# mims-harvard/G-Meta

Measured on AMD Instinct MI355X. Metric: meta-tasks/sec (inner-loop fwd+bwd) at task_num=32, higher is better.
Workload: dtype f32

## Files before the change

g-meta_amd/_lib.py:

```python
import ctypes as C
import os

HERE = os.path.dirname(os.path.abspath(__file__))
LIB_PATH = os.environ.get('GMETA_HIP_LIB') or os.path.join(HERE, 'libgmeta_hip.so')

GM_MAX_GCN = 4
(F_SUB_OFF, F_SET_SUB_OFF, F_PARENT, F_GRAPH, F_INDPTR, F_INDICES, F_INDPTR_T, F_INDICES_T, F_CENTRE, F_NORM,
 F_FEAT_ROW, F_NORM_SRC, F_NORM_CENTRE, F_EDGE_W, F_EDGE_W_T, F_HOP, F_NORM_E1, F_EDGE_CENTRE_T, F_OBS_CENTRE, F_OBS_E1) = range(20)
LINK_SYMMETRIC = 2
LINK_MASK_TARGET = 4
NEG_MODES = {'uniform': 0, 'two_hop': 1}
PAIR_MASK_TARGET = 1
PROP_SELF_LOOPS = 1
PROP_OPS = {'hadamard': 0, 'abs_diff': 1}
DIST_UNREACHED = 255


class Seed(C.Structure):
    _fields_ = [('graph', C.c_int32), ('i', C.c_int32), ('j', C.c_int32)]


class Model(C.Structure):
    _fields_ = [('n_gcn', C.c_int32), ('dims', C.c_int32 * (GM_MAX_GCN + 1)), ('n_out', C.c_int32), ('link_pred', C.c_int32)]


class HParams(C.Structure):
    _fields_ = [('update_lr', C.c_float), ('update_step', C.c_int32), ('k_spt', C.c_int32), ('need_meta_grad', C.c_int32),
                ('hoist_z1', C.c_int32), ('serialize', C.c_int32), ('sparse_bwd', C.c_int32), ('cone', C.c_int32)]


vp, i32, i64, u64 = C.c_void_p, C.c_int32, C.c_int64, C.c_uint64
PROTOTYPES = {
    'gm_last_error': (C.c_char_p, []),
    'gm_version': (C.c_int, []),
    'gm_store_create': (C.c_int, [i32, vp, vp, vp, vp, i32, vp]),
    'gm_store_create_weighted': (C.c_int, [i32, vp, vp, vp, vp, vp, i32, vp]),
    'gm_store_weighted': (i32, [vp]),
    'gm_batch_weighted': (i32, [vp]),
    'gm_store_destroy': (None, [vp]),
    'gm_store_negative_pairs': (i32, [vp, i32, i64, u64, i32, vp, i64, vp, vp, vp]),
    'gm_store_has_edges': (i32, [vp, i32, vp, i64, vp, vp]),
    'gm_store_pair_scores': (i32, [vp, i32, vp, i64, i32, vp, vp]),
    'gm_store_pair_walks': (i32, [vp, i32, vp, i64, i32, vp, vp]),
    'gm_store_rooted_pagerank': (i32, [vp, i32, vp, i64, C.c_float, i32, vp, vp]),
    'gm_store_pair_pagerank': (i32, [vp, i32, vp, i64, i32, C.c_float, i32, vp, vp]),
    'gm_store_pagerank_candidates': (i32, [vp, i32, vp, i64, i32, C.c_float, i32, vp, vp, vp, vp]),
    'gm_store_node_distances': (i32, [vp, i32, vp, i64, i32, vp, vp]),
    'gm_store_pair_distance': (i32, [vp, i32, vp, i64, i32, i32, vp, vp]),
    'gm_store_pair_distance_profile': (i32, [vp, i32, vp, i64, i32, i32, vp, vp]),
    'gm_store_sketch_build': (i32, [vp, i32, i32, i32, i32, u64, vp, vp]),
    'gm_sketch_dims': (i32, [vp, vp, vp, vp, vp, vp]),
    'gm_sketch_registers': (i32, [vp, i32, vp, i64, vp, vp, vp]),
    'gm_sketch_pair_counts': (i32, [vp, vp, i64, vp, vp, vp]),
    'gm_sketch_destroy': (None, [vp]),
    'gm_store_propagate_build': (i32, [vp, i32, i32, i32, vp, vp]),
    'gm_prop_dims': (i32, [vp, vp, vp, vp, vp, vp]),
    'gm_prop_rows': (i32, [vp, i32, vp, i64, vp, vp]),
    'gm_prop_pair_features': (i32, [vp, vp, i64, i32, vp, vp]),
    'gm_prop_destroy': (None, [vp]),
    'gm_store_neighbour_degrees': (i32, [vp, i32, vp, vp]),
    'gm_store_pair_candidates': (i32, [vp, i32, vp, i64, i32, i32, vp, vp, vp, vp]),
    'gm_extract': (C.c_int, [vp, vp, i32, vp, i32, i32, i32, u64, i32, vp, vp]),
    'gm_extract_pair': (C.c_int, [vp, vp, i32, vp, i32, vp, i32, vp, i32, i32, i32, u64, i32, vp, vp, vp]),
    'gm_batch_from_nodes': (C.c_int, [vp, vp, i32, vp, i32, vp, vp, i32, vp, vp]),
    'gm_set_hop_labels': (None, [i32]),
    'gm_get_hop_labels': (i32, []),
    'gm_batch_hop_labels': (i32, [vp]),
    'gm_batch_mask_target': (i32, [vp]),
    'gm_batch_concat': (C.c_int, [vp, i32, vp, vp]),
    'gm_batch_destroy': (None, [vp]),
    'gm_batch_prepare_cone': (C.c_int, [vp, i32, vp]),
    'gm_batch_prepare_cone_pair': (C.c_int, [vp, vp, i32, vp]),
    'gm_batch_cone_dims': (C.c_int, [vp, i32, vp, vp, vp]),
    'gm_batch_cone_read': (C.c_int, [vp, i32, i32, i32, vp, i64]),
    'gm_batch_dims': (C.c_int, [vp, vp, vp, vp, vp, vp]),
    'gm_batch_read': (C.c_int, [vp, i32, vp, i64]),
    'gm_batch_device_ptr': (C.c_int, [vp, i32, vp]),
    'gm_batch_source_rows': (C.c_int, [vp, vp]),
    'gm_batch_e1_source_rows': (C.c_int, [vp, vp]),
    'gm_gather_features': (C.c_int, [vp, vp, vp]),
    'gm_aggregate': (C.c_int, [vp, i32, i32, vp, i32, vp, vp, vp, vp]),
    'gm_aggregate_bytes': (i64, [vp, i32]),
    'gm_model_param_count': (i64, [vp]),
    'gm_gcn_ws_bytes': (i64, [vp, vp]),
    'gm_gcn_forward': (C.c_int, [vp, vp, vp, i64, vp, vp, vp, vp, i64, vp]),
    'gm_gcn_backward': (C.c_int, [vp, vp, vp, i64, vp, vp, vp, vp, i64, vp, i64, vp]),
    'gm_dense_update': (C.c_int, [vp, vp, i32, vp, i64, i32, vp, i32, vp]),
    'gm_dense_gemm': (C.c_int, [vp, vp, i64, i32, vp, i64, i32, i32, vp, i64, vp, vp, vp, i64, i32, vp, vp, vp, vp, vp, i32, vp, vp]),
    'gm_dense_fused_gemm': (C.c_int, [vp, i32, vp, i64, i32, vp, i64, vp, i64, vp, i64, i32, vp, i64, vp, vp, vp, i64, i32, vp, vp, vp, i32, vp, vp]),
    'gm_dense_wgrad_fused': (C.c_int, [vp, i32, vp, i64, i32, vp, i64, vp, i64, i32, vp, vp, vp, i64, vp, i64, i32, vp]),
    'gm_dense_aggregate': (C.c_int, [vp, i32, i32, vp, i64, i32, i32, vp, vp, i32, vp, i64, i32, vp, vp, vp, i32, vp, i64, i32, i32, i32, i32, i32, vp, vp, vp]),
    'gm_dense_agg_info': (C.c_int, [vp, i32, vp]),
    'gm_dense_fuse_counts': (C.c_int, [vp, vp]),
    'gm_dense_agg_table': (C.c_int, [vp, i32, i32, vp, i64, vp]),
    'gm_dense_dz_centre': (C.c_int, [vp, vp, i32, vp, i64, i32, vp, vp]),
    'gm_dense_wgrad_centre': (C.c_int, [vp, vp, i32, vp, i32, vp, i64, vp, i64, vp]),
    'gm_dense_agg_centre_t': (C.c_int, [vp, vp, i32, vp, vp, i32, vp]),
    'gm_dense_wgrad_e1': (C.c_int, [vp, vp, i32, vp, i32, vp, i64, vp, i64, vp]),
    'gm_dense_wgrad': (C.c_int, [vp, vp, i64, i32, vp, i64, i32, vp, vp, i64, vp, i64, vp, i64, i32, vp, vp, i64, C.c_float, vp, vp, vp, vp]),
    'gm_proto_loss_spt': (C.c_int, [vp, vp, i32, vp, i32, vp, vp, vp, vp, vp]),
    'gm_proto_loss_qry': (C.c_int, [vp, vp, i32, vp, vp, i32, vp, vp, vp, vp, vp]),
    'gm_dense_head_loss': (C.c_int, [vp, vp, i32, i32, i32, i32, vp, i64, i64, i64, vp, vp, i32, i32, vp, i32, vp, vp, vp, vp, vp, vp, vp, vp, i32, vp, i64, vp, vp,
                                     vp, vp, i64, C.c_float, vp, i32, vp, vp]),
    'gm_set_ragged_classes': (None, [i32]),
    'gm_get_ragged_classes': (i32, []),
    'gm_set_readout': (None, [i32]),
    'gm_get_readout': (i32, []),
    'gm_meta_ws_bytes': (i64, [vp, vp, vp, vp]),
    'gm_meta_out_floats': (i64, [vp, vp, vp]),
    'gm_meta_step': (C.c_int, [vp, vp, vp, vp, vp, vp, vp, vp, i64, vp, i64, vp]),
    'gm_adapt_ws_bytes': (i64, [vp, vp, vp]),
    'gm_meta_adapt': (C.c_int, [vp, vp, vp, vp, vp, vp, i64, vp, i32, vp, i64, vp]),
    'gm_predict_ws_bytes': (i64, [vp, vp, vp]),
    'gm_proto_predict': (C.c_int, [vp, vp, vp, vp, i64, vp, vp, i32, vp, vp, vp, vp, i64, vp]),
    'gm_meta_finish': (C.c_int, [vp, i64, i32, vp, vp, vp]),
    'gm_meta_finish_adam': (C.c_int, [vp, i64, i32, vp, vp, vp, vp, vp, i32, C.c_float, C.c_float, C.c_float, C.c_float, vp, vp, vp]),
    'gm_set_gemm_mode': (None, [i32]),
    'gm_get_gemm_mode': (i32, []),
    'gm_get_split_pieces': (i32, []),
    'gm_set_split_pieces': (None, [i32]),
    'gm_set_tuning': (C.c_int, [C.c_char_p, i32]),
    'gm_get_tuning': (i32, [C.c_char_p]),
    'gm_tuning_epoch': (i32, []),
    'gm_set_fuse_agg': (None, [i32]),
    'gm_get_fuse_agg': (i32, []),
    'gm_profile_enable': (None, [i32]),
    'gm_profile_aggregate': (C.c_int, [vp, vp, vp]),
    'gm_profile_read': (C.c_int, [i32, vp, vp, vp]),
    'gm_profile_read_launches': (C.c_int, [i32, vp, vp, i32]),
}
PROBE_PROTOTYPES = {
    'gm_debug_stamp': (C.c_int, [vp, vp]),
    'gm_stream_debug': (C.c_int, [i32, vp, i32]),
    'gm_head_loss_debug': (C.c_int, [i32, vp]),
}

_lib = None


def lib():
    global _lib
    if _lib is None:
        if not os.path.exists(LIB_PATH):
            raise RuntimeError('gmeta_amd: %s is missing -- run `python -c "import __graft_entry__ as g; g.build()"` '
                               '(hipcc --offload-arch=gfx950).  There is no CPU fallback.' % LIB_PATH)
        l = C.CDLL(LIB_PATH)
        for name, (res, args) in PROTOTYPES.items():
            fn = getattr(l, name)
            fn.restype, fn.argtypes = res, args
        for name, (res, args) in PROBE_PROTOTYPES.items():
            if hasattr(l, name):
                fn = getattr(l, name)
                fn.restype, fn.argtypes = res, args
        _lib = l
    return _lib


def check(rc, what=''):
    if rc != 0:
        msg = lib().gm_last_error().decode('utf-8', 'replace')
        exc = ValueError if rc == -1 else RuntimeError
        raise exc('%s failed (code %d): %s' % (what or 'libgmeta_hip', rc, msg))


def require_gpu():
    import torch
    if not torch.cuda.is_available():
        raise RuntimeError('gmeta_amd needs an AMD GPU (gfx950); torch.cuda.is_available() is False and there is no CPU fallback')


def stream_ptr():
    import torch
    return C.c_void_p(torch.cuda.current_stream().cuda_stream)


def ptr(t):
    if t is None:
        return C.c_void_p(0)
    if hasattr(t, 'data_ptr'):
        return C.c_void_p(t.data_ptr())
    return C.c_void_p(t.ctypes.data)


READOUT_CENTRE, READOUT_MEAN = 0, 1
READOUTS = {'centre': READOUT_CENTRE, 'mean': READOUT_MEAN}


def config_readout(config):
    ent = [(k, p) for k, (n, p) in enumerate(config) if n == 'Readout']
    if not ent:
        return 'centre'
    if len(ent) > 1:
        raise ValueError("config holds %d 'Readout' entries; at most one" % len(ent))
    k, p = ent[0]
    if not isinstance(p, (list, tuple)) or len(p) != 1 or p[0] not in READOUTS:
        raise ValueError("config entry ('Readout', %r): expected ['centre'] or ['mean']" % (p,))
    if any(n == 'LinkPred' for n, _ in config) and config[-1][0] != 'LinkPred':
        raise ValueError("the ('Readout', ...) entry must come before the trailing ('LinkPred', [True]) entry")
    return p[0]


class readout_switch:

    def __init__(self, readout):
        self.mode = READOUTS[readout] if isinstance(readout, str) else int(readout)

    def __enter__(self):
        l = lib()
        self.was = int(l.gm_get_readout())
        if self.was != self.mode:
            l.gm_set_readout(self.mode)
        return self

    def __exit__(self, *exc):
        if self.was != self.mode:
            lib().gm_set_readout(self.was)
        return False


def make_model(config):
    unknown = sorted({str(n) for n, _ in config if n not in ('GraphConv', 'Linear', 'LinkPred', 'Readout', 'Attention')})
    if unknown:
        raise ValueError('unknown config entries: %s' % ', '.join(unknown))
    config_readout(config)
    gcn = [p for n, p in config if n == 'GraphConv']
    lin = [p for n, p in config if n == 'Linear']
    if any(n == 'Attention' for n, _ in config):
        raise NotImplementedError("the 'Attention' branch of learner.py:98-131 is dead code in the reference (uses an undefined name)")
    if not gcn or len(lin) != 1 or len(gcn) > GM_MAX_GCN:
        raise ValueError('config must hold 1..%d GraphConv entries and one Linear entry' % GM_MAX_GCN)
# ... 12 lines not shown
```

g-meta_amd/csrc/agg.hip:

```cpp
#include <algorithm>
#include <stdlib.h>
#include <mutex>
#include "gm_internal.h"
#include "agg_hub.h"

#define AGG_BLOCK 256

struct AggK {
    const int32_t* indptr; const int32_t* indices; const float* x; const int32_t* x_row; int64_t ldx;
    const float* s_in; const float* s_out; const float* mask_h; const float* bias; int64_t bias_stride;
    const int32_t* set_row_off; int n_sets; int relu; float* out; int64_t rows; int width; int nblocks;
    const uint8_t* mask_b; uint8_t* relu_bits;
    const int32_t* heavy; int n_heavy, heavy_deg;
    const int32_t* sched; int sched_len;
    int nt;
    int win;
    const int32_t* hub; float* hub_scratch; int hub_part, hub_ld;
    const float* e_w; const int32_t* x_idx;
    int skip_lo, skip_hi;
    const int32_t* rowlist; int64_t n_list;
    int keep_signed;
};
__host__ __device__ __forceinline__ int agg_xcd_first(const int nb, const int x) {
    const int q = nb / GM_NXCD, r = nb % GM_NXCD;
    return x < r ? x * (q + 1) : r * (q + 1) + (x - r) * q;
}
__device__ __forceinline__ int agg_logical_block(const int nb, const int b) { return agg_xcd_first(nb, b % GM_NXCD) + b / GM_NXCD; }

__device__ __forceinline__ float agg_out_scale(const AggK& a, const float raw, bool& keep) {
    keep = !(a.keep_signed && (__float_as_uint(raw) >> 31));
    return a.keep_signed ? fabsf(raw) : raw;
}
__device__ __forceinline__ bool agg_unobservable(const AggK& a, const float raw) {
    return a.keep_signed && !a.relu_bits && (__float_as_uint(raw) >> 31);
}
__device__ __forceinline__ int agg_bias_set(const AggK& a, const int64_t row) {
    if (!a.bias || !a.bias_stride) return 0;
    int lo = 0, hi = a.n_sets;
    while (hi - lo > 1) { const int mid = (lo + hi) >> 1; if (a.set_row_off[mid] <= row) lo = mid; else hi = mid; }
    return lo;
}

__device__ __forceinline__ void agg_edge(const AggK& a, const int e, int& u, float& w) {
    if (a.e_w && (a.x_idx || !a.x_row)) {
        w = a.e_w[e]; u = a.x_idx ? a.x_idx[e] : a.indices[e];
    } else {
        u = a.indices[e]; w = a.s_in ? a.s_in[u] : 1.f;
        if (a.x_idx) u = a.x_idx[e]; else if (a.x_row) u = a.x_row[u];
    }
}
template <int VEC> struct VecT;
template <> struct VecT<4> { using T = float4; };
template <> struct VecT<1> { using T = float; };

__device__ __forceinline__ void vfma(float4& a, const float4& v, float s) { a.x += v.x * s; a.y += v.y * s; a.z += v.z * s; a.w += v.w * s; }
__device__ __forceinline__ void vfma(float& a, const float& v, float s) { a += v * s; }
__device__ __forceinline__ void vzero(float4& a) { a = make_float4(0.f, 0.f, 0.f, 0.f); }
__device__ __forceinline__ void vzero(float& a) { a = 0.f; }
__device__ __forceinline__ float vget(const float4& a, int k) { return k == 0 ? a.x : k == 1 ? a.y : k == 2 ? a.z : a.w; }
__device__ __forceinline__ float vget(const float& a, int) { return a; }
__device__ __forceinline__ void vset(float4& a, int k, float v) { if (k == 0) a.x = v; else if (k == 1) a.y = v; else if (k == 2) a.z = v; else a.w = v; }
__device__ __forceinline__ void vset(float& a, int, float v) { a = v; }

template <int VEC, int LPR>
__global__ __launch_bounds__(AGG_BLOCK) void k_agg(AggK a) {
    using V = typename VecT<VEC>::T;
    constexpr int RPW = GM_WAVE / LPR;
    constexpr int RPB = RPW * (AGG_BLOCK / GM_WAVE);
    const int lb = agg_logical_block(a.nblocks, blockIdx.x);
    const int lane = threadIdx.x & 63, wave = threadIdx.x >> 6;
    const int sub = lane / LPR, l = lane % LPR;
    const int64_t row = (int64_t)lb * RPB + wave * RPW + sub;
    if (row >= a.rows) return;
    const int e0 = a.indptr[row], e1 = a.indptr[row + 1];
    bool keep;
    const float raw = a.s_out ? a.s_out[row] : 1.f;
    if (agg_unobservable(a, raw)) return;
    const float so = agg_out_scale(a, raw, keep);
    const int set = agg_bias_set(a, row);
    for (int c0 = l * VEC; c0 < a.width; c0 += LPR * VEC) {
        V acc0, acc1; vzero(acc0); vzero(acc1);
        int e = e0;
        for (; e + 4 <= e1; e += 4) {
            int u0, u1, u2, u3; float w0, w1, w2, w3;
            agg_edge(a, e, u0, w0); agg_edge(a, e + 1, u1, w1); agg_edge(a, e + 2, u2, w2); agg_edge(a, e + 3, u3, w3);
            const V v0 = *reinterpret_cast<const V*>(a.x + (int64_t)u0 * a.ldx + c0);
            const V v1 = *reinterpret_cast<const V*>(a.x + (int64_t)u1 * a.ldx + c0);
            const V v2 = *reinterpret_cast<const V*>(a.x + (int64_t)u2 * a.ldx + c0);
            const V v3 = *reinterpret_cast<const V*>(a.x + (int64_t)u3 * a.ldx + c0);
            vfma(acc0, v0, w0); vfma(acc1, v1, w1); vfma(acc0, v2, w2); vfma(acc1, v3, w3);
        }
        for (; e < e1; ++e) {
            int u; float w;
            agg_edge(a, e, u, w);
            vfma(acc0, *reinterpret_cast<const V*>(a.x + (int64_t)u * a.ldx + c0), w);
        }
        V res;
#pragma unroll
        for (int k = 0; k < VEC; ++k) {
            float v = (vget(acc0, k) + vget(acc1, k)) * so;
            if (a.bias) v += a.bias[(int64_t)set * a.bias_stride + c0 + k];
            if (a.relu) v = v < 0.f ? 0.f : v;
            if (a.mask_b) v = ((a.mask_b[(row * a.width + c0) >> 2] >> k) & 1u) ? v : 0.f;
            else if (a.mask_h) v = a.mask_h[row * a.width + c0 + k] > 0.f ? v : 0.f;
// ... 56 lines not shown
            __builtin_nontemporal_store(vv, reinterpret_cast<f4v*>(dst));
        } else *dst = v;
    }
}

#define AGG_HEAVY_BLOCK 1024
template <int LPR, int NCH, int NTHREADS>
__device__ __forceinline__ void agg_heavy_row(const AggK& a, const int g, float* part) {
    constexpr int NG = NTHREADS / LPR;
    constexpr int PS = 16;
    const int tid = threadIdx.x, gi = tid / LPR, l = tid % LPR, lane = tid & 63;
    const int gbase = (lane / LPR) * LPR;
    int h = g, p = 0, P = 1;
    if (a.hub) { h = a.hub[a.n_heavy + 1 + g]; p = g - a.hub[h]; P = a.hub[h + 1] - a.hub[h]; }
    const int row = a.heavy[h];
    const float so = a.s_out ? a.s_out[row] : 1.f;
    if (agg_unobservable(a, so)) return;
    int e0 = a.indptr[row], e1 = a.indptr[row + 1];
    if (P > 1) { e0 += p * a.hub_part; if (p < P - 1) e1 = e0 + a.hub_part; }
    const float* xl = a.x + l * 4;
    float4 acc[NCH];
#pragma unroll
    for (int c = 0; c < NCH; ++c) acc[c] = make_float4(0.f, 0.f, 0.f, 0.f);
    for (int eb = e0 + gi * PS; eb < e1; eb += NG * PS) agg_gather_batch<LPR, NCH, PS, 8>(a, xl, eb, e1, l, gbase, acc);
#pragma unroll
    for (int c = 0; c < NCH; ++c) *reinterpret_cast<float4*>(&part[(gi * NCH + c) * LPR * 4 + l * 4]) = acc[c];
    __syncthreads();
    float4 s4[NCH];
    if (gi == 0) {
#pragma unroll
        for (int c = 0; c < NCH; ++c) {
            s4[c] = make_float4(0.f, 0.f, 0.f, 0.f);
            for (int k = 0; k < NG; ++k) { const float4 t = *reinterpret_cast<const float4*>(&part[(k * NCH + c) * LPR * 4 + l * 4]); s4[c].x += t.x; s4[c].y += t.y; s4[c].z += t.z; s4[c].w += t.w; }
        }
    }
    if (P > 1) {
        if (gi == 0) {
#pragma unroll
            for (int c = 0; c < NCH; ++c) agg_hub_publish(a.hub_scratch + (int64_t)g * a.hub_ld + l * 4 + c * LPR * 4, s4[c]);
        }
        agg_hub_drain();
        __syncthreads();
        int* ctr = const_cast<int*>(a.hub) + a.n_heavy + 1 + a.hub[a.n_heavy] + h;
        int* flag = reinterpret_cast<int*>(part);
        if (tid == 0) *flag = agg_hub_arrive(ctr, P);
        __syncthreads();
        if (!*flag || gi != 0) return;
        const float* sc = a.hub_scratch + (int64_t)a.hub[h] * a.hub_ld + l * 4;
#pragma unroll
        for (int c = 0; c < NCH; ++c) {
            s4[c] = make_float4(0.f, 0.f, 0.f, 0.f);
            for (int k = 0; k < P; ++k) {
                const float4 t = *reinterpret_cast<const float4*>(sc + (int64_t)k * a.hub_ld + c * LPR * 4);
                s4[c].x += t.x; s4[c].y += t.y; s4[c].z += t.z; s4[c].w += t.w;
            }
        }
    }
    if (gi == 0) agg_store_row<LPR, NCH>(a, row, so, l, s4, false);
}
template <int LPR, int NCH>
__global__ __launch_bounds__(AGG_HEAVY_BLOCK) void k_agg_heavy(AggK a) {
    __shared__ __attribute__((aligned(16))) float part[(AGG_HEAVY_BLOCK / LPR) * LPR * 4 * NCH];
    agg_heavy_row<LPR, NCH, AGG_HEAVY_BLOCK>(a, blockIdx.x, part);
}

template <int LPR, int NCH>
__global__ __launch_bounds__(AGG_BLOCK) void k_agg_win(AggK a) {
    constexpr int G = GM_WAVE / LPR;
    constexpr int UNR = 2;
    int lb = agg_logical_block(a.nblocks, blockIdx.x);
    if (a.sched) {
        const int e = a.sched[(blockIdx.x % GM_NXCD) * a.sched_len + blockIdx.x / GM_NXCD];
        if (e == -1) return;
        if (e < -1) {
            __shared__ __attribute__((aligned(16))) float part[AGG_BLOCK * 4 * NCH];
            agg_heavy_row<LPR, NCH, AGG_BLOCK>(a, -e - 2, part);
            return;
        }
        lb = e;
    }
    const int lane = threadIdx.x & 63, wave = threadIdx.x >> 6;
    const int g = lane / LPR, l = lane % LPR;
    const int64_t R0 = ((int64_t)lb * (AGG_BLOCK / GM_WAVE) + wave) * a.win;
    const int64_t nrows_w = a.rowlist ? a.n_list : a.rows;
    if (R0 >= nrows_w) return;
    const bool mine = lane < a.win && R0 + lane < nrows_w;
    const int64_t myrow = a.rowlist ? (mine ? (int64_t)a.rowlist[R0 + lane] : 0) : R0 + lane;
    const int myrow32 = (int)myrow;
    int p0 = 0, dg = 0, u0 = 0, u1 = 0; float w0 = 0.f, w1 = 0.f, so = 1.f;
    if (mine) {
        p0 = a.indptr[myrow]; dg = a.indptr[myrow + 1] - p0;
        if (a.s_out) so = a.s_out[myrow];
        if (dg >= a.skip_lo && dg <= a.skip_hi) dg = -2;
        if (agg_unobservable(a, so)) dg = -2;
        if (dg >= 1) agg_edge(a, p0, u0, w0);
        if (dg >= 2) agg_edge(a, p0 + 1, u1, w1);
    }
    const int nwin = (int)min((int64_t)a.win, nrows_w - R0);
    const float* xl = a.x + l * 4;
    const unsigned long long live = __ballot(mine && dg >= 0);
    for (int t0 = 0; t0 < nwin; t0 += G * UNR) {
        if (!((live >> t0) & ((1ull << (G * UNR)) - 1))) continue;
        float4 acc[UNR][NCH];
        int rdg[UNR], rp0[UNR], rrow[UNR]; float rso[UNR];
#pragma unroll
        for (int k = 0; k < UNR; ++k) {
            const int rr = t0 + k * G + g;
            const int src = rr < GM_WAVE ? rr : 0;
            rdg[k] = rr < nwin ? __shfl(dg, src, 64) : -1;
            rrow[k] = __shfl(myrow32, src, 64);
            if (a.n_heavy && rdg[k] > a.heavy_deg) rdg[k] = -1;
            rp0[k] = __shfl(p0, src, 64); rso[k] = __shfl(so, src, 64);
            const int a0 = __shfl(u0, src, 64), a1 = __shfl(u1, src, 64);
            const float f0 = __shfl(w0, src, 64), f1 = __shfl(w1, src, 64);
#pragma unroll
            for (int c = 0; c < NCH; ++c) acc[k][c] = make_float4(0.f, 0.f, 0.f, 0.f);
            if (rdg[k] >= 1) {
#pragma unroll
                for (int c = 0; c < NCH; ++c) vfma(acc[k][c], *reinterpret_cast<const float4*>(xl + (int64_t)a0 * a.ldx + c * LPR * 4), f0);
            }
            if (rdg[k] >= 2) {
#pragma unroll
                for (int c = 0; c < NCH; ++c) vfma(acc[k][c], *reinterpret_cast<const float4*>(xl + (int64_t)a1 * a.ldx + c * LPR * 4), f1);
            }
        }
#pragma unroll
        for (int k = 0; k < UNR; ++k) {
            if (rdg[k] < 0) continue;
            const int rr_ = t0 + k * G + g;
            const int64_t row = a.rowlist ? (int64_t)rrow[k] : R0 + rr_;
            const int eend = rp0[k] + rdg[k];
            for (int eb = rp0[k] + 2; eb < eend; eb += LPR) agg_gather_batch<LPR, NCH, LPR, 4>(a, xl, eb, eend, l, g * LPR, acc[k]);
            agg_store_row<LPR, NCH>(a, row, rso[k], l, acc[k], a.nt);
        }
    }
}

int gm_agg_window(int64_t rows, int64_t edges) {
    const bool dense = edges > 8 * rows;
    const int min_waves = dense ? 16384 : 32768;
    const int min_win = dense ? 4 : 2;
    int win = 64;
    while (win > min_win && rows / win < min_waves) win >>= 1;
    return win;
}

int gm_agg_schedule_flat(gm_batch* b, int64_t rows, int win, const int32_t* pos, int n_heavy, const std::vector<int32_t>& tab, int32_t** d_sched, int32_t* len_out,
                         hipStream_t s, gm_stager* sg) {
    const bool split = !tab.empty();
    const int RPB = win * (AGG_BLOCK / GM_WAVE);
    const int nwb = std::max(1, (int)((rows + RPB - 1) / RPB));
    auto x_start = [&](int x) { return agg_xcd_first(nwb, x); };
    auto n_entries = [&](int k) { return split ? tab[k + 1] - tab[k] : 1; };
    int extra[GM_NXCD] = {}; int first[GM_NXCD + 1];
    {
        int hk = 0;
        for (int x = 0; x < GM_NXCD; ++x) {
            const int end = x_start(x + 1);
            first[x] = hk;
            while (hk < n_heavy && pos[hk] / RPB < end) {
                GM_REQUIRE(hk == 0 || pos[hk] >= pos[hk - 1], GM_EINVAL, "aggregate schedule: hub-row list is not ascending");
                extra[x] += n_entries(hk); ++hk;
            }
        }
        first[GM_NXCD] = hk;
        GM_REQUIRE(hk == n_heavy, GM_EINVAL, "aggregate schedule: hub-row list is not ascending / out of range");
    }
    size_t len = 0;
    for (int x = 0; x < GM_NXCD; ++x) len = std::max(len, (size_t)(x_start(x + 1) - x_start(x) + extra[x]));
    std::vector<int32_t> flat(GM_NXCD * len);
    for (int x = 0; x < GM_NXCD; ++x) {
        int32_t* o = flat.data() + x * len; int32_t* const o_end = o + len;
        int wb = x_start(x); const int end = x_start(x + 1);
        for (int hk = first[x]; hk < first[x + 1]; ++hk) {
            const int hb = pos[hk] / RPB;
            while (wb <= hb) *o++ = wb++;
            if (split) for (int g = tab[hk]; g < tab[hk + 1]; ++g) *o++ = -g - 2;
            else *o++ = -hk - 2;
        }
        while (wb < end) *o++ = wb++;
        while (o < o_end) *o++ = -1;
    }
    GM_TRY(gm_balloc(b, d_sched, flat.size(), s));
    GM_TRY(sg->upload(*d_sched, flat));
    *len_out = (int32_t)len;
    return GM_OK;
}

int gm_agg_schedule(gm_batch* b, int64_t rows, int win, const int32_t* heavy_host, const int32_t* heavy_deg_host, int n_heavy, gm_agg_sched* out, hipStream_t s, gm_stager* sg) {
    *out = gm_agg_sched{};
    if (n_heavy <= 0 || rows <= 0) return GM_OK;
    int hub_part = 0;
    std::vector<int32_t> tab;
    if (heavy_deg_host) {
        int maxdeg = 0;
        for (int k = 0; k < n_heavy; ++k) maxdeg = std::max(maxdeg, heavy_deg_host[k]);
        hub_part = std::max(128, ((maxdeg + 31) / 32 + 15) / 16 * 16);
        tab.assign(n_heavy + 1, 0);
        for (int k = 0; k < n_heavy; ++k) tab[k + 1] = tab[k] + std::max(1, (heavy_deg_host[k] + hub_part / 2) / hub_part);
        const int parts = tab[n_heavy];
        if (parts == n_heavy) { hub_part = 0; tab.clear(); }
        else {
            tab.resize(n_heavy + 1 + parts + n_heavy, 0);
            for (int k = 0; k < n_heavy; ++k) for (int g = tab[k]; g < tab[k + 1]; ++g) tab[n_heavy + 1 + g] = k;
        }
    }
    GM_TRY(gm_agg_schedule_flat(b, rows, win, heavy_host, n_heavy, tab, &out->d_sched, &out->len, s, sg));
    if (hub_part) {
        GM_TRY(gm_balloc(b, &out->d_hub, tab.size(), s));
        GM_TRY(sg->upload(out->d_hub, tab));
        GM_TRY(gm_balloc(b, &out->d_hub_scratch, (size_t)tab[n_heavy] * GM_AGG_HUB_LD, s));
        out->hub_part = hub_part; out->hub_words = (int32_t)tab.size(); out->parts = tab[n_heavy];
    }
    out->tab = tab;
    return GM_OK;
}

template <int LPR, int NCH>
static void launch_win(const AggK& a0, hipStream_t s, int* launched) {
    AggK a = a0;
    a.win = (a.sched || a.rowlist) ? a0.win : gm_agg_window(a.rows, 0);
    const int RPB = a.win * (AGG_BLOCK / GM_WAVE);
    a.nblocks = (int)(((a.rowlist ? a.n_list : a.rows) + RPB - 1) / RPB);
    int grid = a.nblocks;
    if (a.sched) grid = GM_NXCD * a.sched_len;
    else if (a.n_heavy > 0) hipLaunchKernelGGL((k_agg_heavy<LPR, NCH>), dim3(a.n_heavy), dim3(AGG_HEAVY_BLOCK), 0, s, a);
    hipLaunchKernelGGL((k_agg_win<LPR, NCH>), dim3(grid), dim3(AGG_BLOCK), 0, s, a);
    if (launched) *launched = GM_AGG_ID_WIN(LPR, NCH) + (a.sched ? GM_AGG_ID_WIN_SCHED + (a.hub ? GM_AGG_ID_WIN_SPLIT : 0) : a.n_heavy > 0 ? GM_AGG_ID_WIN_HEAVY : 0) +
                                (a.rowlist ? GM_AGG_ID_WIN_LIST : 0);
}

template <int VEC, int LPR>
static void launch_one(const AggK& a0, hipStream_t s, int* launched) {
    AggK a = a0;
    constexpr int RPB = (GM_WAVE / LPR) * (AGG_BLOCK / GM_WAVE);
    a.nblocks = (int)((a.rows + RPB - 1) / RPB);
    hipLaunchKernelGGL((k_agg<VEC, LPR>), dim3(a.nblocks), dim3(AGG_BLOCK), 0, s, a);
    if (launched) *launched = GM_AGG_ID_ONE(VEC, LPR);
}
template <int VEC>
static void launch_generic(const AggK& a, const int lanes, hipStream_t s, int* launched) {
    if (lanes > 32) launch_one<VEC, 64>(a, s, launched);
    else if (lanes > 16) launch_one<VEC, 32>(a, s, launched);
    else if (lanes > 8) launch_one<VEC, 16>(a, s, launched);
    else if (lanes > 4) launch_one<VEC, 8>(a, s, launched);
    else if (lanes > 2) launch_one<VEC, 4>(a, s, launched);
    else launch_one<VEC, 2>(a, s, launched);
}

static int agg_nt(int64_t rows, int width) { return rows * (int64_t)width * 4 >= ((int64_t)128 << 20) ? 1 : 0; }

int gm_launch_aggregate(const gm_agg_args& g, hipStream_t s) {
    if (g.rows <= 0) return GM_OK;
    AggK a{};
    a.indptr = g.indptr; a.indices = g.indices; a.x = g.x; a.x_row = g.x_row; a.ldx = g.ldx;
    a.s_in = g.s_in; a.s_out = g.s_out; a.mask_h = g.mask_h; a.bias = g.bias; a.bias_stride = g.bias_stride;
    a.set_row_off = g.set_row_off; a.n_sets = g.n_sets; a.relu = g.relu; a.out = g.out; a.rows = g.rows; a.width = g.width;
    a.mask_b = g.mask_b; a.relu_bits = g.relu_bits;
    a.heavy = g.heavy; a.n_heavy = g.n_heavy; a.heavy_deg = g.heavy_deg;
    a.sched = g.sched; a.sched_len = g.sched_len;
    a.nt = agg_nt(g.rows, g.width);
    a.win = g.rowlist ? g.list_win : g.sched ? g.sched_win : 64;
    a.hub = g.sched ? g.hub : nullptr; a.hub_scratch = g.sched ? g.hub_scratch : nullptr; a.hub_part = g.hub_part; a.hub_ld = GM_AGG_HUB_LD;
    a.e_w = g.e_w; a.x_idx = g.x_idx;
    a.skip_lo = g.skip_on ? g.skip_lo : 1; a.skip_hi = g.skip_on ? g.skip_hi : 0;
    a.rowlist = g.rowlist; a.n_list = g.n_list;
    a.keep_signed = (g.keep_signed && g.s_out) ? 1 : 0;
    const bool vec4 = (g.width % 4 == 0) && (g.ldx % 4 == 0) && (((uintptr_t)g.x & 15) == 0) && (((uintptr_t)g.out & 15) == 0);
    const bool bias_ok = !g.bias || ((((uintptr_t)g.bias & 15) == 0) && (g.bias_stride % 4 == 0));
    const bool mask_ok = !g.mask_h || (((uintptr_t)g.mask_h & 15) == 0);
    GM_REQUIRE(!(g.mask_b || g.relu_bits) || vec4, GM_EINVAL, "aggregate: packed relu masks need width %% 4 == 0 and 16-byte aligned operands");
    const bool win = vec4 && bias_ok && mask_ok && (g.width == 64 || g.width == 128 || g.width == 256 || g.width == 512);
    GM_REQUIRE(!g.rowlist || win, GM_EINVAL, "aggregate: a row list needs the window kernel");
    if (!win) { a.heavy = nullptr; a.n_heavy = 0; a.sched = nullptr; a.hub = nullptr; }
    if (win && gm_knob().agg_stream && gm_stream_ok(g)) return gm_launch_stream(g, a.nt, s);
    if (win) {
        if (g.width == 64) launch_win<16, 1>(a, s, g.launched);
        else if (g.width == 128) launch_win<32, 1>(a, s, g.launched);
        else if (g.width == 256) launch_win<64, 1>(a, s, g.launched);
        else launch_win<64, 2>(a, s, g.launched);
    } else if (vec4) launch_generic<4>(a, g.width / 4, s, g.launched);
    else launch_generic<1>(a, g.width, s, g.launched);
    GM_HIP(hipGetLastError());
    return GM_OK;
}

int gm_agg_stream_args(gm_agg_args& a, const gm_batch* b, int o, bool gather, hipStream_t s) {
    if (!gm_knob().agg_stream || a.s_out || a.bias || a.mask_h || a.mask_b || a.relu || a.relu_bits || a.rowlist || a.skip_on) return GM_OK;
    gm_batch::stream_pending& sp = b->spend[o];
    {
        static std::mutex mu;
        std::lock_guard<std::mutex> lk(mu);
        if (sp.pending) {
            gm_batch* mb = const_cast<gm_batch*>(b);
            gm_stager sg(s);
            GM_TRY(gm_stream_tables(mb, o, sp.hubs.data(), sp.deg.data(), (int)sp.hubs.size(), sp.n_parts, sp.has_tab ? &sp.tab : nullptr, s, &sg));
            sp.pending = false;
            sp.hubs = std::vector<int32_t>(); sp.deg = std::vector<int32_t>(); sp.tab = std::vector<int32_t>();
            gm_batch_mark_use(b, s);
        }
    }
    if (!b->d_sptr[o] || !b->d_sseg[o] || (gather && (o != 0 || !b->d_su_feat))) return GM_OK;
    a.stream = b; a.stream_o = o; a.stream_feat = gather ? 1 : 0;
    a.stream_xrows = gather ? b->feat_rows : b->rows;
    return GM_OK;
}

extern "C" int64_t gm_aggregate_bytes(const gm_batch_t* b, int32_t width) {
    if (!b) return -1;
    return 4 * (b->rows + 1) + 4 * b->edges + 4 * b->rows + 8 * b->rows * (int64_t)width;
}

extern "C" int gm_aggregate(const gm_batch_t* b, int32_t transposed, int32_t gather, const float* x, int32_t width,
                            const float* s_in, const float* s_out, float* out, void* stream) {
    GM_REQUIRE(b && out && width >= 1, GM_EINVAL, "aggregate: bad arguments");
    GM_REQUIRE(gather || x, GM_EINVAL, "aggregate: x is NULL and gather == 0");
    GM_REQUIRE(!gather || width == b->feat_dim, GM_EINVAL, "aggregate: gather needs width == feat_dim");
    gm_agg_args a{};
    a.indptr = transposed ? b->d_indptr_t : b->d_indptr;
    a.indices = transposed ? b->d_indices_t : b->d_indices;
    a.x = gather ? b->feat : x;
    a.x_row = gather ? b->d_feat_row : nullptr;
    if (gather && !transposed) a.x_idx = b->d_efeat;
    if (s_in && s_in == b->d_norm) a.e_w = b->d_enorm[transposed ? 1 : 0];
    if (b->weighted) {
        GM_REQUIRE(!s_in || s_in == b->d_norm, GM_EINVAL, "aggregate: on a weighted batch s_in must be NULL or the batch's own GM_F_NORM (the per-source gather has no edge-weight slot)");
        GM_REQUIRE(!(gather && transposed), GM_EINVAL, "aggregate: gather with transposed is not available on a weighted batch (no per-edge feature rows for the by-source CSR)");
        if (!s_in) a.e_w = b->d_ew[transposed ? 1 : 0];
    }
    a.ldx = gather ? b->feat_ld : width; a.s_in = s_in; a.s_out = s_out; a.out = out; a.rows = b->rows; a.width = width;
    a.heavy = b->d_heavy[transposed ? 1 : 0]; a.n_heavy = b->n_heavy[transposed ? 1 : 0]; a.heavy_deg = b->heavy_deg;
    a.sched = b->d_sched[transposed ? 1 : 0]; a.sched_len = b->sched_len[transposed ? 1 : 0]; a.sched_win = b->sched_win; GM_TRY(gm_agg_hub(a, b, transposed ? 1 : 0, (hipStream_t)stream));
    if (a.e_w && a.e_w == b->d_enorm[transposed ? 1 : 0]) GM_TRY(gm_agg_stream_args(a, b, transposed ? 1 : 0, gather != 0, (hipStream_t)stream));
    gm_prof_agg_begin((hipStream_t)stream, gm_aggregate_bytes(b, width));
    int rc = gm_launch_aggregate(a, (hipStream_t)stream);
    gm_prof_agg_end((hipStream_t)stream);
    gm_batch_mark_use(b, (hipStream_t)stream);
    return rc;
}
```

g-meta_amd/csrc/common.hip:

```cpp
#include <stdarg.h>
#include <stdlib.h>
#include <atomic>
#include <chrono>
#include <map>
#include <mutex>
#include <set>
#include <utility>
#include "gm_internal.h"

static thread_local char g_err[512] = "";

void gm_set_error(const char* fmt, ...) {
    va_list ap;
    va_start(ap, fmt);
    vsnprintf(g_err, sizeof(g_err), fmt, ap);
    va_end(ap);
}

extern "C" const char* gm_last_error(void) { return g_err; }
extern "C" int gm_version(void) { return 100; }

static void pool_keep_memory() {
    static thread_local int done_for = -1;
    int dev = 0;
// ... 230 lines not shown
    ProfCat& c = g_prof[cat];
    if (c.used + 2 > c.ev.size()) {
        hipEvent_t a, b;
        if (hipEventCreate(&a) != hipSuccess || hipEventCreate(&b) != hipSuccess) return;
        c.ev.push_back(a); c.ev.push_back(b);
    }
    (void)hipEventRecord(c.ev[c.used], s);
    c.work += work; c.launches += 1; c.open = true;
    if (c.works.size() < c.used / 2 + 1) c.works.resize(c.used / 2 + 1);
    c.works[c.used / 2] = work;
}
bool gm_prof_enabled() { return g_prof_on != 0; }
void gm_prof_reset_cat(int cat) { ProfCat& c = g_prof[cat]; c.used = 0; c.work = 0; c.launches = 0; c.open = false; }
void gm_prof_note(int cat, int64_t work) { if (g_prof_on) g_prof[cat].work += work; }
void gm_prof_end(int cat, hipStream_t s) {
    ProfCat& c = g_prof[cat];
    if (!g_prof_on || !c.open) return;
    (void)hipEventRecord(c.ev[c.used + 1], s);
    c.used += 2; c.open = false;
}

extern "C" int gm_profile_read(int32_t category, double* total_ms, int64_t* launches, int64_t* work) {
    GM_REQUIRE(category >= 0 && category < GM_PROF_CATS, GM_EINVAL, "profile_read: unknown category %d", category);
    ProfCat& c = g_prof[category];
    double tot = 0;
    for (size_t k = 0; k + 1 < c.used + 1 && k < c.used; k += 2) {
        GM_HIP(hipEventSynchronize(c.ev[k + 1]));
        float ms = 0;
        GM_HIP(hipEventElapsedTime(&ms, c.ev[k], c.ev[k + 1]));
        tot += ms;
    }
    if (total_ms) *total_ms = tot;
    if (launches) *launches = c.launches;
    if (work) *work = c.work;
    return GM_OK;
}
extern "C" int gm_profile_read_launches(int32_t category, double* ms, int64_t* work, int32_t cap) {
    GM_REQUIRE(category >= 0 && category < GM_PROF_CATS && ms && work && cap >= 0, GM_EINVAL, "profile_read_launches: bad arguments");
    ProfCat& c = g_prof[category];
    int n = 0;
    for (size_t k = 0; k + 1 < c.used + 1 && k < c.used && n < cap; k += 2, ++n) {
        GM_HIP(hipEventSynchronize(c.ev[k + 1]));
        float t = 0;
        GM_HIP(hipEventElapsedTime(&t, c.ev[k], c.ev[k + 1]));
        ms[n] = t; work[n] = k / 2 < c.works.size() ? c.works[k / 2] : 0;
    }
    return n;
}
extern "C" int gm_profile_aggregate(double* total_ms, int64_t* launches, int64_t* algorithmic_bytes) {
    return gm_profile_read(GM_PROF_AGG, total_ms, launches, algorithmic_bytes);
}

#ifdef GM_PROBES
__global__ void k_debug_stamp(unsigned long long* out) { *out = wall_clock64(); }
extern "C" int gm_debug_stamp(void* out, void* stream) {
    GM_REQUIRE(out, GM_EINVAL, "debug_stamp: NULL argument");
    hipLaunchKernelGGL(k_debug_stamp, dim3(1), dim3(1), 0, (hipStream_t)stream, (unsigned long long*)out);
    GM_HIP(hipGetLastError());
    return GM_OK;
}
#endif

static gm_knobs g_knobs;
static std::once_flag g_knobs_once;
const gm_knobs& gm_knob() {
    gm_knobs& k = g_knobs;
    std::call_once(g_knobs_once, [] {
        gm_knobs& k = g_knobs;
        auto env = [](const char* name, int dflt) { const char* e = getenv(name); return e ? atoi(e) : dflt; };
        k.timing = env("GM_TIMING", 0);
        const char* gm = getenv("GM_GEMM_MODE");
        k.gemm_mode = (gm && (!strcmp(gm, "split") || !strcmp(gm, "1"))) ? 1 : (gm && (!strcmp(gm, "f32") || !strcmp(gm, "0"))) ? 0 : -1;
        k.gemm_split_min_tiles = env("GM_GEMM_SPLIT_MIN_TILES", -1);
        k.centre_store = env("GM_CENTRE_STORE", 2);
        k.dead_rows = env("GM_DEAD_ROWS", 4);
        k.fuse_agg = env("GM_FUSE_AGG", 1);
        k.fuse_diff = env("GM_FUSE_DIFF", 2);
        k.extract_pref16 = env("GM_EXTRACT_PREF16", 1);
        k.head_stage = env("GM_HEAD_STAGE", 1);
        k.head_threads = env("GM_HEAD_THREADS", 0);
        k.query_streams = env("GM_QUERY_STREAMS", 0);
        k.agg_mid_list = env("GM_AGG_MID_LIST", 1);
        k.agg_mid_win = env("GM_AGG_MID_WIN", 0);
        k.split_pieces = env("GM_SPLIT_PIECES", 3);
        k.split16_min_rows = env("GM_SPLIT16_MIN_ROWS", 65536);
        k.wgrad_split_min_chunks = env("GM_WGRAD_SPLIT_MIN_CHUNKS", -1);
        k.agg_stream = env("GM_AGG_STREAM", 1);
        k.agg_stream_min_rows = env("GM_AGG_STREAM_MIN_ROWS", 100000);
        k.neg_round = env("GM_NEG_ROUND", 0);
        k.pair_lanes = env("GM_PAIR_LANES", 0);
        k.cand_round = env("GM_CAND_ROUND", 0);
        k.cand_bitmap = env("GM_CAND_BITMAP", 0);
        k.walk_chunk = env("GM_WALK_CHUNK", 0);
        k.walk_lanes = env("GM_WALK_LANES", 0);
        k.ppr_chunk = env("GM_PPR_CHUNK", 0);
        k.ppr_cols = env("GM_PPR_COLS", 0);
        k.dist_chunk = env("GM_DIST_CHUNK", 0);
        k.dist_cols = env("GM_DIST_COLS", 0);
        k.dist_plane_kib = env("GM_DIST_PLANE_KIB", 0);
        k.sketch_chunk = env("GM_SKETCH_CHUNK", 0);
        k.sketch_mib = env("GM_SKETCH_MIB", 0);
        k.prop_chunk = env("GM_PROP_CHUNK", 0);
        k.prop_mib = env("GM_PROP_MIB", 0);
    });
    return k;
}

static std::atomic<int> g_tuning_epoch{0};
extern "C" int32_t gm_tuning_epoch(void) { return g_tuning_epoch.load(std::memory_order_relaxed); }
static int gm_knobs::* gm_find_knob(const char* name) {
    (void)gm_knob();
    static const struct { const char* name; int gm_knobs::*field; } tab[] = {
        {"GM_GEMM_SPLIT_MIN_TILES", &gm_knobs::gemm_split_min_tiles}, {"GM_CENTRE_STORE", &gm_knobs::centre_store}, {"GM_DEAD_ROWS", &gm_knobs::dead_rows},
        {"GM_HEAD_STAGE", &gm_knobs::head_stage}, {"GM_HEAD_THREADS", &gm_knobs::head_threads}, {"GM_QUERY_STREAMS", &gm_knobs::query_streams}, {"GM_AGG_MID_LIST", &gm_knobs::agg_mid_list}, {"GM_AGG_MID_WIN", &gm_knobs::agg_mid_win}, {"GM_AGG_STREAM", &gm_knobs::agg_stream}, {"GM_AGG_STREAM_MIN_ROWS", &gm_knobs::agg_stream_min_rows},
        {"GM_SPLIT16_MIN_ROWS", &gm_knobs::split16_min_rows}, {"GM_WGRAD_SPLIT_MIN_CHUNKS", &gm_knobs::wgrad_split_min_chunks}, {"GM_TIMING", &gm_knobs::timing},
        {"GM_FUSE_DIFF", &gm_knobs::fuse_diff}, {"GM_EXTRACT_PREF16", &gm_knobs::extract_pref16},
        {"neg_round", &gm_knobs::neg_round}, {"GM_NEG_ROUND", &gm_knobs::neg_round},
        {"pair_lanes", &gm_knobs::pair_lanes}, {"GM_PAIR_LANES", &gm_knobs::pair_lanes},
        {"cand_round", &gm_knobs::cand_round}, {"GM_CAND_ROUND", &gm_knobs::cand_round},
        {"cand_bitmap", &gm_knobs::cand_bitmap}, {"GM_CAND_BITMAP", &gm_knobs::cand_bitmap},
        {"walk_chunk", &gm_knobs::walk_chunk}, {"GM_WALK_CHUNK", &gm_knobs::walk_chunk},
        {"walk_lanes", &gm_knobs::walk_lanes}, {"GM_WALK_LANES", &gm_knobs::walk_lanes},
        {"ppr_chunk", &gm_knobs::ppr_chunk}, {"GM_PPR_CHUNK", &gm_knobs::ppr_chunk},
        {"ppr_cols", &gm_knobs::ppr_cols}, {"GM_PPR_COLS", &gm_knobs::ppr_cols},
        {"dist_chunk", &gm_knobs::dist_chunk}, {"GM_DIST_CHUNK", &gm_knobs::dist_chunk},
        {"dist_cols", &gm_knobs::dist_cols}, {"GM_DIST_COLS", &gm_knobs::dist_cols},
        {"dist_plane_kib", &gm_knobs::dist_plane_kib}, {"GM_DIST_PLANE_KIB", &gm_knobs::dist_plane_kib},
        {"sketch_chunk", &gm_knobs::sketch_chunk}, {"GM_SKETCH_CHUNK", &gm_knobs::sketch_chunk},
        {"sketch_mib", &gm_knobs::sketch_mib}, {"GM_SKETCH_MIB", &gm_knobs::sketch_mib},
        {"prop_chunk", &gm_knobs::prop_chunk}, {"GM_PROP_CHUNK", &gm_knobs::prop_chunk},
        {"prop_mib", &gm_knobs::prop_mib}, {"GM_PROP_MIB", &gm_knobs::prop_mib},
    };
    for (const auto& e : tab)
        if (!strcmp(name, e.name)) return e.field;
    return nullptr;
}
extern "C" int gm_set_tuning(const char* name, int32_t value) {
    GM_REQUIRE(name, GM_EINVAL, "set_tuning: NULL name");
    int gm_knobs::* f = gm_find_knob(name);
    GM_REQUIRE(f, GM_EINVAL, "set_tuning: unknown or start-up-only knob %s", name);
    g_knobs.*f = value; g_tuning_epoch.fetch_add(1, std::memory_order_relaxed);
    return GM_OK;
}
extern "C" int32_t gm_get_tuning(const char* name) {
    int gm_knobs::* f = name ? gm_find_knob(name) : nullptr;
    return f ? g_knobs.*f : 0;
}

int gm_heavy_deg() { return 64; }
int gm_heavy_deg_for(int64_t rows, int64_t edges) {
    return edges <= 8 * rows ? 32 : 64;
}

static std::mutex g_dev_mu;

int gm_num_cus() {
    static std::map<int, int> cus;
    int dev = 0;
    if (hipGetDevice(&dev) != hipSuccess) { (void)hipGetLastError(); return 256; }
    std::lock_guard<std::mutex> lk(g_dev_mu);
    auto it = cus.find(dev);
    if (it != cus.end()) return it->second;
    int n = 0;
    if (hipDeviceGetAttribute(&n, hipDeviceAttributeMultiprocessorCount, dev) != hipSuccess || n <= 0) { (void)hipGetLastError(); n = 256; }
    cus[dev] = n;
    return n;
}

int gm_func_full_lds(const void* fn) {
    static std::set<std::pair<int, const void*>> done;
    int dev = 0;
    GM_HIP(hipGetDevice(&dev));
    std::lock_guard<std::mutex> lk(g_dev_mu);
    if (done.count({dev, fn})) return GM_OK;
    GM_HIP(hipFuncSetAttribute(fn, hipFuncAttributeMaxDynamicSharedMemorySize, 160 * 1024));
    done.insert({dev, fn});
    return GM_OK;
}
```

g-meta_amd/csrc/dense_exports.hip:

```cpp
#include <algorithm>
#include "gm_internal.h"

static int set_row_amax(const gm_batch* b, const float* x, int64_t ldx, int cols, unsigned* slots, hipStream_t st) {
    int rc = GM_OK;
    for (int t0 = 0; rc == GM_OK && t0 < b->sets; t0 += 8) {
        const int segs = std::min(8, b->sets - t0);
        int64_t xo[8], xn[8];
        for (int i = 0; i < segs; ++i) {
            const int64_t r0 = b->h_set_row_off[t0 + i], nr = b->h_set_row_off[t0 + i + 1] - r0;
            xo[i] = r0 * ldx; xn[i] = nr > 0 ? (nr - 1) * ldx + cols : 0;
        }
        rc = gm_amax_segs(x, xo, xn, segs, slots + (int64_t)t0 * GM_BOUND_PAD, GM_BOUND_PAD, st);
    }
    return rc;
}

extern "C" int gm_dense_update(const gm_batch_t* b, const float* x, int32_t K, const float* W, int64_t w_stride, int32_t N, float* out, int32_t mode,
                               void* stream) {
    GM_REQUIRE(b && x && W && out && K >= 1 && N >= 1, GM_EINVAL, "dense_update: bad arguments");
    hipStream_t st = (hipStream_t)stream;
    gm_gemm_args g{};
    g.A = x; g.lda = K; g.B = W; g.b_stride = w_stride; g.C = out; g.ldc = N; g.K = K; g.N = N;
    g.tiles = b->d_tiles; g.n_tiles = b->n_tiles; g.rows = b->rows;
    uint16_t* planes = nullptr; unsigned* slots = nullptr;
// ... 220 lines not shown
    GM_REQUIRE(table == 1 || (gx && ldgx >= K), GM_EINVAL, "dense_wgrad_fused: table 0 needs gx and ldgx >= K");
    GM_REQUIRE(table == 0 || (b->feat && (K == b->feat_dim || K == b->feat_ld)), GM_EINVAL, "dense_wgrad_fused: table 1 needs K == feat_dim (%d)", b->feat_dim);
    const int sets = b->sets;
    const int64_t KN = (int64_t)K * N;
    GM_REQUIRE(sets == 1 || (dw_stride >= KN && db_stride >= N), GM_EINVAL, "dense_wgrad_fused: per-set outputs overlap");
    hipStream_t st = (hipStream_t)stream;
    gm_wgrad_args w{};
    w.A = A; w.lda = lda; w.K = K; w.G = g; w.ldg = ldg; w.N = N; w.a_scale = s; w.g_keep = g_keep;
    w.chunks = b->d_chunks; w.n_chunks = b->n_chunks; w.set_chunk_off = b->d_set_chunk_off; w.sets = sets; w.rows = b->rows;
    w.dW = dW; w.dw_stride = dw_stride; w.db = db; w.db_stride = db_stride;
    w.fuse2 = table == 1 ? b->d_fuse2_feat : b->d_fuse2;
    w.gx = table == 1 ? b->feat : gx; w.ldgx = table == 1 ? b->feat_ld : ldgx;
    w.pick = mode == 0 ? GM_WGRAD_PICK_EXACT : GM_WGRAD_PICK_SPLIT;
    unsigned* slots = nullptr;
    int rc = gm_alloc(&w.partial, (size_t)std::max(1, b->n_chunks) * (size_t)(KN + N), st);
    if (rc == GM_OK && mode == 2) {
        rc = gm_alloc(&slots, (size_t)(2 * sets + 1) * GM_BOUND_PAD, st);
        if (rc == GM_OK && hipMemsetAsync(slots, 0, sizeof(unsigned) * (2 * sets + 1) * GM_BOUND_PAD, st) != hipSuccess) { gm_set_error("dense_wgrad_fused: memset failed"); rc = GM_EHIP; }
        w.np = 2;
        w.a_bound = gm_no_bound(); w.a_bound.amax = slots; w.a_bound.stride = GM_BOUND_PAD;
        w.g_bound = gm_no_bound(); w.g_bound.amax = slots + (int64_t)sets * GM_BOUND_PAD; w.g_bound.stride = GM_BOUND_PAD;
    }
    if (rc == GM_OK) rc = gm_launch_wgrad(w, st);
    if (w.partial) gm_dev_free(w.partial, st);
    if (slots) gm_dev_free(slots, st);
    gm_batch_mark_use(b, st);
    return rc;
}

extern "C" int gm_dense_aggregate(const gm_batch_t* b, int32_t transposed, int32_t x_src, const float* x, int64_t ldx, int32_t width, int32_t scale_src,
                                  const float* s_in, const float* s_out, int32_t keep_signed, const float* bias, int64_t bias_stride, int32_t relu,
                                  uint8_t* relu_bits, const float* mask_h, const uint8_t* mask_b, int32_t hubs, const int32_t* rowlist, int64_t n_list,
                                  int32_t list_win, int32_t list_sched, int32_t skip_lo, int32_t skip_hi, int32_t stream_ok, float* out, int32_t* launched,
                                  void* stream) {
    GM_REQUIRE(b && out && width >= 1 && x_src >= 0 && x_src <= 3 && scale_src >= 0 && scale_src <= 2 && hubs >= 0 && hubs <= 2, GM_EINVAL, "dense_aggregate: bad arguments");
    GM_REQUIRE(!(mask_h && mask_b), GM_EINVAL, "dense_aggregate: mask_h together with mask_b");
    GM_REQUIRE(!(rowlist && stream_ok), GM_EINVAL, "dense_aggregate: a row list together with the stream kernel");
    GM_REQUIRE(!stream_ok || hubs == 2, GM_EINVAL, "dense_aggregate: the stream kernel takes the batch's hub tables (hubs == 2)");
    const int o = transposed ? 1 : 0;
    const bool gather = x_src == 1 || x_src == 2;
    GM_REQUIRE(gather || (x && ldx >= width), GM_EINVAL, "dense_aggregate: a caller matrix needs x and ldx >= width");
    GM_REQUIRE(!gather || width == b->feat_dim, GM_EINVAL, "dense_aggregate: a gather needs width == feat_dim (%d)", b->feat_dim);
    GM_REQUIRE(x_src != 2 || (!transposed && b->d_efeat), GM_EINVAL, "dense_aggregate: the per-edge feature rows belong to the by-destination CSR");
    GM_REQUIRE(x_src != 3 || (transposed && b->d_ect), GM_EINVAL, "dense_aggregate: the centre-edge table belongs to the by-source CSR of a batch that carries one");
    GM_REQUIRE((scale_src == 1) == (s_in != nullptr), GM_EINVAL, "dense_aggregate: s_in goes with scale_src == 1 and only with it");
    GM_REQUIRE(scale_src != 2 || b->d_enorm[o], GM_EINVAL, "dense_aggregate: the batch has no per-edge norm table");
    GM_REQUIRE(!bias || !bias_stride || b->d_set_row_off, GM_EINVAL, "dense_aggregate: per-set bias without set row offsets");
    GM_REQUIRE(!keep_signed || s_out, GM_EINVAL, "dense_aggregate: keep_signed needs s_out");
    GM_REQUIRE(!relu_bits || relu, GM_EINVAL, "dense_aggregate: relu_bits are written with relu");
    hipStream_t st = (hipStream_t)stream;
    gm_agg_args a{};
    a.indptr = transposed ? b->d_indptr_t : b->d_indptr;
    a.indices = transposed ? b->d_indices_t : b->d_indices;
    a.rows = b->rows; a.width = width; a.out = out; a.launched = launched;
    if (gather) { a.x = b->feat; a.ldx = b->feat_ld; a.x_row = b->d_feat_row; if (x_src == 2) a.x_idx = b->d_efeat; }
    else { a.x = x; a.ldx = ldx; if (x_src == 3) a.x_idx = b->d_ect; }
    if (b->weighted) {
        GM_REQUIRE(scale_src != 1, GM_EINVAL, "dense_aggregate: on a weighted batch the source scale is none or the batch's own table (the per-source gather has no edge-weight slot)");
        GM_REQUIRE(x_src != 1, GM_EINVAL, "dense_aggregate: on a weighted batch the feature gather goes through the per-edge row table (x_src 2; the per-source gather has no edge-weight slot)");
        if (scale_src == 0) a.e_w = b->d_ew[o];
    }
    if (scale_src == 1) a.s_in = s_in;
    if (scale_src == 2) { a.s_in = b->d_norm; a.e_w = b->d_enorm[o]; }
    a.s_out = s_out; a.keep_signed = keep_signed ? 1 : 0;
    a.bias = bias; a.bias_stride = bias_stride; a.set_row_off = b->d_set_row_off; a.n_sets = b->sets;
    a.relu = relu ? 1 : 0; a.relu_bits = relu_bits; a.mask_h = mask_h; a.mask_b = mask_b;
    if (hubs) { a.heavy = b->d_heavy[o]; a.n_heavy = b->n_heavy[o]; a.heavy_deg = b->heavy_deg; }
    if (hubs == 2) { a.sched = b->d_sched[o]; a.sched_len = b->sched_len[o]; a.sched_win = b->sched_win; GM_TRY(gm_agg_hub(a, b, o, st)); }
    if (skip_lo <= skip_hi) { a.skip_on = 1; a.skip_lo = skip_lo; a.skip_hi = skip_hi; }
    if (rowlist) {
        GM_REQUIRE(n_list >= 1 && n_list <= b->rows && list_win >= 2 && list_win <= 64 && (list_win & (list_win - 1)) == 0, GM_EINVAL,
                   "dense_aggregate: a row list needs 1 .. rows entries and a window of 2, 4, .. 64 rows");
        std::vector<int32_t> h((size_t)n_list);
        GM_HIP(hipMemcpyAsync(h.data(), rowlist, sizeof(int32_t) * (size_t)n_list, hipMemcpyDeviceToHost, st));
        GM_HIP(hipStreamSynchronize(st));
        for (int64_t k = 0; k < n_list; ++k)
            GM_REQUIRE(h[k] >= 0 && h[k] < b->rows && (k == 0 || h[k] > h[k - 1]), GM_EINVAL, "dense_aggregate: the row list is not ascending / out of range at entry %lld", (long long)k);
        a.rowlist = rowlist; a.n_list = n_list; a.list_win = list_win;
        if (list_sched) {
            GM_REQUIRE(hubs == 2 && !transposed && b->d_sched_mid && n_list == b->n_mid && list_win == b->mid_win, GM_EINVAL,
                       "dense_aggregate: the list schedule goes with the batch's own list (%d rows, windows of %d) and its hub tables", b->n_mid, b->mid_win);
            a.sched = b->d_sched_mid; a.sched_len = b->sched_len_mid; a.sched_win = b->mid_win;
        } else { a.sched = nullptr; a.sched_len = 0; }
    } else GM_REQUIRE(!list_sched, GM_EINVAL, "dense_aggregate: a list schedule without a row list");
    if (stream_ok && a.e_w && a.e_w == b->d_enorm[o]) GM_TRY(gm_agg_stream_args(a, b, o, gather, st));
    const int rc = gm_launch_aggregate(a, st);
    gm_batch_mark_use(b, st);
    return rc;
}

extern "C" int gm_dense_agg_info(const gm_batch_t* b, int32_t transposed, int64_t* info) {
    GM_REQUIRE(b && info, GM_EINVAL, "dense_agg_info: bad arguments");
    const int o = transposed ? 1 : 0;
    const int64_t v[16] = {b->heavy_deg, b->n_heavy[o], b->sched_win, b->hub_part[o], b->hub_parts[o], b->d_sched[o] ? 1 : 0, b->d_mid ? b->n_mid : 0, b->mid_win,
                           b->d_sched_mid ? 1 : 0, b->d_sseg[o] ? b->stream_nseg[o] : 0, b->stream_nwg[o], b->stream_hubwg[o], b->weighted ? 1 : 0, b->feat_dim, b->feat_ld, 0};
    std::copy(v, v + 16, info);
    return GM_OK;
}
extern "C" int gm_dense_fuse_counts(const gm_batch_t* b, int64_t* counts) {
    GM_REQUIRE(b && counts, GM_EINVAL, "dense_fuse_counts: bad arguments");
    counts[0] = b->unfused_rows; counts[1] = b->unfused_edges;
    return GM_OK;
}
extern "C" int gm_dense_agg_table(const gm_batch_t* b, int32_t which, int32_t transposed, void* dst, int64_t n, void* stream) {
    GM_REQUIRE(b && dst && n >= 0 && which >= 0 && which <= 9, GM_EINVAL, "dense_agg_table: bad arguments");
    const int o = transposed ? 1 : 0;
    const void* src = which == 0 ? (const void*)b->d_enorm[o] : which == 1 ? (const void*)b->d_efeat : which == 2 ? (const void*)b->d_mid : which == 3 ? (const void*)b->d_heavy[o]
                    : which == 4 ? (const void*)b->d_fuse2 : which == 5 ? (const void*)b->d_fuse2_feat : which == 6 ? (const void*)b->d_dq_tab
                    : which == 7 ? (const void*)b->d_fwd_tab[0] : which == 8 ? (const void*)b->d_fwd_tab[1] : (const void*)b->d_fwd_tab_feat;
    const int64_t have = which <= 1 ? b->edges : which == 2 ? b->n_mid : which == 3 ? b->n_heavy[o] : b->rows;
    GM_REQUIRE(src && n <= have, GM_EINVAL, "dense_agg_table: table %d holds %lld entries", which, (long long)(src ? have : 0));
    if (n) GM_HIP(hipMemcpyAsync(dst, src, (which >= 4 ? 16 : 4) * (size_t)n, hipMemcpyDeviceToDevice, (hipStream_t)stream));
    gm_batch_mark_use(b, (hipStream_t)stream);
    return GM_OK;
}
```

g-meta_amd/csrc/extract.hip:

```cpp
#include <algorithm>
#include <initializer_list>
#include <stdlib.h>
#include <string.h>
#include <memory>
#include <mutex>
#include <type_traits>
#include "gm_internal.h"
#include "gm_devutil.h"

#define EX_BLOCK 512
#define EX_WAVES (EX_BLOCK / GM_WAVE)

__device__ __forceinline__ int lane_id() { return __builtin_amdgcn_mbcnt_hi(~0u, __builtin_amdgcn_mbcnt_lo(~0u, 0u)); }
__device__ __forceinline__ int wave_sum(int v) {
#pragma unroll
    for (int o = 32; o > 0; o >>= 1) v += __shfl_xor(v, o, 64);
    return v;
}
template <bool G> __device__ __forceinline__ bool bit_test(const uint32_t* bm, int v) { return (wld<G>(&bm[v >> 5]) >> (v & 31)) & 1u; }
__device__ __forceinline__ void bit_set(uint32_t* bm, int v) { atomicOr(&bm[v >> 5], 1u << (v & 31)); }
template <bool G, typename PT> __device__ __forceinline__ int pref_ld(const PT* p) {
    if constexpr (sizeof(PT) == 4) return (int)wld<G>(reinterpret_cast<const uint32_t*>(p)); else return (int)*p;
}
template <bool G, typename PT> __device__ __forceinline__ int bit_rank(const uint32_t* bm, const PT* pref, int v) {
// ... 504 lines not shown
template <typename... WArgs>
__global__ void k_row_tables(const int32_t* indptr, const int32_t* indices, const int32_t* indptr_t, int64_t rows, const float* norm, const int32_t* feat_row,
                             int4* f2, int4* f2_feat, unsigned long long* counts, int32_t* heavy0, int32_t* heavy1, int32_t* hcnt, int cap, int thr, float* norm_c,
                             int2* first0, int2* first1, int n_first, float* norm_src, int4* dq_tab, WArgs... w_args) {
    constexpr bool WT = sizeof...(WArgs) != 0;
    unsigned long long nr = 0, ne = 0, ns = 0;
    for (int64_t r = blockIdx.x * (int64_t)blockDim.x + threadIdx.x; r < rows; r += (int64_t)gridDim.x * blockDim.x) {
        const int p = indptr[r], d = indptr[r + 1] - p, dt = indptr_t[r + 1] - indptr_t[r];
        {
            const unsigned long long m0 = __ballot(d > thr), m1 = __ballot(dt > thr), below = (1ull << (threadIdx.x & 63)) - 1ull;
            if (m0) {
                const int lead = __ffsll((long long)m0) - 1;
                int base = ((int)(threadIdx.x & 63) == lead) ? atomicAdd(hcnt, __popcll(m0)) : 0;
                base = __shfl(base, lead, 64);
                if (d > thr) { const int k = base + __popcll(m0 & below); if (k < cap) { heavy0[k] = (int32_t)r; heavy0[cap + k] = d; } if (k < n_first) first0[k] = make_int2((int)r, d); }
            }
            if (m1) {
                const int lead = __ffsll((long long)m1) - 1;
                int base = ((int)(threadIdx.x & 63) == lead) ? atomicAdd(hcnt + 1, __popcll(m1)) : 0;
                base = __shfl(base, lead, 64);
                if (dt > thr) { const int k = base + __popcll(m1 & below); if (k < cap) { heavy1[k] = (int32_t)r; heavy1[cap + k] = dt; } if (k < n_first) first1[k] = make_int2((int)r, dt); }
            }
        }
        const float nrm = norm[r];
        norm_c[r] = __uint_as_float(__float_as_uint(nrm) | 0x80000000u);
        norm_src[r] = dt > 0 ? nrm : __uint_as_float(__float_as_uint(nrm) | 0x80000000u);
        if (dt > 0) ++ns;
        dq_tab[r] = make_int4(GM_FUSE_ZERO, GM_FUSE_ZERO, 0, 0);
        const int self = (int)r | GM_FUSE_SELF;
        int4 t = make_int4(self, self, __float_as_int(1.f), 0), tf = t;
        if (d == 0) { t = make_int4(GM_FUSE_ZERO, GM_FUSE_ZERO, __float_as_int(1.f), 0); tf = t; }
        else if (d <= GM_FUSE_MAXDEG) {
            const int u0 = indices[p], u1 = d >= 2 ? indices[p + 1] : u0;
            int w0, w1;
            if constexpr (WT) { const float* ew = (w_args, ...).ew; w0 = __float_as_int(ew[p] * norm[u0]); w1 = d >= 2 ? __float_as_int(ew[p + 1] * norm[u1]) : 0; }
            else { w0 = __float_as_int(norm[u0]); w1 = d >= 2 ? __float_as_int(norm[u1]) : 0; }
            t = make_int4(u0, u1, w0, w1); tf = make_int4(feat_row[u0], feat_row[u1], w0, w1);
        }
        if (d > GM_FUSE_MAXDEG) { ++nr; ne += (unsigned long long)d; }
        f2[r] = t; f2_feat[r] = tf;
    }
    __shared__ unsigned long long part[3][4];
#pragma unroll
    for (int off = 32; off >= 1; off >>= 1) { nr += __shfl_down(nr, off, 64); ne += __shfl_down(ne, off, 64); ns += __shfl_down(ns, off, 64); }
    if ((threadIdx.x & 63) == 0) { part[0][threadIdx.x >> 6] = nr; part[1][threadIdx.x >> 6] = ne; part[2][threadIdx.x >> 6] = ns; }
    __syncthreads();
    if (threadIdx.x == 0) {
        counts[3 * blockIdx.x] = part[0][0] + part[0][1] + part[0][2] + part[0][3];
        counts[3 * blockIdx.x + 1] = part[1][0] + part[1][1] + part[1][2] + part[1][3];
        counts[3 * blockIdx.x + 2] = part[2][0] + part[2][1] + part[2][2] + part[2][3];
    }
}
__global__ void k_mark_sources(const int32_t* indptr, const int32_t* indices, int64_t rows, int maxdeg, uint32_t* bits) {
    for (int64_t r = blockIdx.x * (int64_t)blockDim.x + threadIdx.x; r < rows; r += (int64_t)gridDim.x * blockDim.x) {
        const int p = indptr[r], d = indptr[r + 1] - p;
        if (d > maxdeg) for (int e = p; e < p + d; ++e) { const int u = indices[e]; atomicOr(&bits[u >> 5], 1u << (u & 31)); }
    }
}
__global__ void k_count_bits(const uint32_t* bits, int64_t words, unsigned long long* out) {
    unsigned long long c = 0;
    for (int64_t w = blockIdx.x * (int64_t)blockDim.x + threadIdx.x; w < words; w += (int64_t)gridDim.x * blockDim.x) c += __popc(bits[w]);
#pragma unroll
    for (int off = 32; off >= 1; off >>= 1) c += __shfl_down(c, off, 64);
    if ((threadIdx.x & 63) == 0 && c) atomicAdd(out, c);
}
int64_t gm_batch_unfused_sources(const gm_batch* b, hipStream_t s) {
    if (b->unfused_src >= 0) return b->unfused_src;
    const int64_t fallback = std::min<int64_t>(b->unfused_edges, b->rows);
    if (b->rows <= 0 || b->unfused_edges <= 0) return b->unfused_src = 0;
    const int64_t words = (b->rows + 31) / 32;
    uint32_t* bits = nullptr; unsigned long long* cnt = nullptr; unsigned long long h = 0;
    if (gm_alloc(&bits, (size_t)words, s) != GM_OK || gm_alloc(&cnt, 1, s) != GM_OK) { gm_dev_free(bits, s); return fallback; }
    bool ok = hipMemsetAsync(bits, 0, 4 * (size_t)words, s) == hipSuccess && hipMemsetAsync(cnt, 0, 8, s) == hipSuccess;
    if (ok) {
        hipLaunchKernelGGL(k_mark_sources, dim3((int)std::min<int64_t>(2048, (b->rows + 255) / 256)), dim3(256), 0, s, b->d_indptr, b->d_indices, (int64_t)b->rows, GM_FUSE_MAXDEG, bits);
        hipLaunchKernelGGL(k_count_bits, dim3((int)std::min<int64_t>(512, (words + 255) / 256)), dim3(256), 0, s, bits, words, cnt);
        ok = hipMemcpyAsync(&h, cnt, 8, hipMemcpyDeviceToHost, s) == hipSuccess && hipStreamSynchronize(s) == hipSuccess;
    }
    if (!ok) (void)hipGetLastError();
    gm_dev_free(bits, s); gm_dev_free(cnt, s);
    return ok ? (b->unfused_src = (int64_t)h) : fallback;
}
#define MID_BLOCK 1024
__device__ __forceinline__ bool mid_row(const int32_t* indptr, int64_t r, int64_t rows, int lo, int hi) {
    if (r >= rows) return false;
    const int d = indptr[r + 1] - indptr[r];
    return d >= lo && d <= hi;
}
__global__ __launch_bounds__(MID_BLOCK) void k_mid_count(const int32_t* indptr, int64_t rows, int lo, int hi, int32_t* bcnt) {
    __shared__ int wsum[MID_BLOCK / 64];
    const int64_t r = (int64_t)blockIdx.x * MID_BLOCK + threadIdx.x;
    const unsigned long long m = __ballot(mid_row(indptr, r, rows, lo, hi));
    if ((threadIdx.x & 63) == 0) wsum[threadIdx.x >> 6] = __popcll(m);
    __syncthreads();
    if (threadIdx.x == 0) { int t = 0; for (int k = 0; k < MID_BLOCK / 64; ++k) t += wsum[k]; bcnt[blockIdx.x] = t; }
}
__global__ __launch_bounds__(1024) void k_mid_scan(int32_t* bcnt, int nb) {
    __shared__ int part[1024];
    const int per = (nb + 1023) / 1024, a = threadIdx.x * per, b = min(nb, a + per);
    int t = 0;
    for (int k = a; k < b; ++k) t += bcnt[k];
    part[threadIdx.x] = t;
    __syncthreads();
    if (threadIdx.x == 0) { int run = 0; for (int k = 0; k < 1024; ++k) { const int v = part[k]; part[k] = run; run += v; } }
    __syncthreads();
    int run = part[threadIdx.x];
    for (int k = a; k < b; ++k) { const int v = bcnt[k]; bcnt[k] = run; run += v; }
}
__global__ __launch_bounds__(MID_BLOCK) void k_mid_scatter(const int32_t* indptr, int64_t rows, int lo, int hi, const int32_t* boff, int32_t* list, int cap) {
    __shared__ int wsum[MID_BLOCK / 64];
    const int64_t r = (int64_t)blockIdx.x * MID_BLOCK + threadIdx.x;
    const bool f = mid_row(indptr, r, rows, lo, hi);
    const unsigned long long m = __ballot(f);
    const int lane = threadIdx.x & 63, wv = threadIdx.x >> 6;
    if (lane == 0) wsum[wv] = __popcll(m);
    __syncthreads();
    int base = boff[blockIdx.x];
    for (int k = 0; k < wv; ++k) base += wsum[k];
    const int at = base + __popcll(m & ((1ull << lane) - 1ull));
    if (f && at < cap) list[at] = (int32_t)r;
}
__global__ void k_centre_rows(const int32_t* sub_off, const int32_t* centre, int nc, int n_c, const int32_t* indptr, const float* norm,
                              int32_t* crow, float* cnorm, int32_t* cdeg, float* norm_c, int32_t* centre_copy, int4* dq_tab) {
    const int k = blockIdx.x * blockDim.x + threadIdx.x;
    if (k >= n_c) return;
    const int row = sub_off[k / nc] + centre[k];
    centre_copy[k] = centre[k];
    crow[k] = row; cnorm[k] = norm[row]; cdeg[k] = indptr[row + 1] - indptr[row];
    if (norm_c) norm_c[row] = __uint_as_float(__float_as_uint(norm[row]) & 0x7fffffffu);
    if (dq_tab) dq_tab[row] = make_int4(row | GM_FUSE_SELF, GM_FUSE_ZERO, __float_as_int(1.f), 0);
}
struct CentreW { const float* ew; float* e_coef; };
template <typename... WArgs>
__global__ void k_centre_edges(const int32_t* crow, const int32_t* eoff, int n_c, const int32_t* indptr, const int32_t* indices,
                               const float* norm, int32_t* e_row, int32_t* e_par, float* e_norm, WArgs... w_args) {
    const int k = blockIdx.x;
    if (k >= n_c) return;
    const int p0 = indptr[crow[k]], n = eoff[k + 1] - eoff[k], o = eoff[k];
    for (int j = threadIdx.x; j < n; j += blockDim.x) {
        const int u = indices[p0 + j]; e_row[o + j] = u; e_par[o + j] = k; e_norm[o + j] = norm[u];
        if constexpr (sizeof...(WArgs) != 0) { const CentreW& cw = (w_args, ...); cw.e_coef[o + j] = cw.ew[p0 + j] * norm[u]; }
    }
}
__global__ void k_e1_tables(const int32_t* indices_t, int64_t edges, const float* norm, const float* norm_c, int64_t rows, int32_t* ect, float* norm_e1, int32_t* n_rows) {
    const int64_t n = edges > rows ? edges : rows;
    if (blockIdx.x == 0 && threadIdx.x == 0) *n_rows = 0;
    for (int64_t k = blockIdx.x * (int64_t)blockDim.x + threadIdx.x; k < n; k += (int64_t)gridDim.x * blockDim.x) {
        if (k < rows) norm_e1[k] = __uint_as_float(__float_as_uint(norm[k]) | 0x80000000u);
        if (k < edges) { const int v = indices_t[k]; ect[k] = (__float_as_uint(norm_c[v]) >> 31) ? (int32_t)(rows + (k & (GM_ZERO_ROWS - 1))) : v; }
    }
}
__global__ void k_e1_rows(const int32_t* e_row, int n_e1, float* norm_e1, int32_t* n_rows) {
    const int k = blockIdx.x * blockDim.x + threadIdx.x;
    if (k >= n_e1) return;
    const unsigned old = atomicAnd(reinterpret_cast<unsigned*>(norm_e1) + e_row[k], 0x7fffffffu);
    if (old >> 31) atomicAdd(n_rows, 1);
}
int64_t gm_batch_e1_rows(const gm_batch* b, hipStream_t s) {
    if (b->n_e1_rows >= 0) return b->n_e1_rows;
    const int64_t fallback = std::min<int64_t>(b->n_e1, b->rows);
    if (!b->d_n_e1_rows) return fallback;
    int32_t h = 0;
    if (hipMemcpyAsync(&h, b->d_n_e1_rows, 4, hipMemcpyDeviceToHost, s) != hipSuccess || hipStreamSynchronize(s) != hipSuccess) { (void)hipGetLastError(); return fallback; }
    return b->n_e1_rows = h;
}
__global__ void k_e1_kept_edges(const int32_t* indptr_t, const float* norm_e1, int64_t rows, unsigned long long* out) {
    unsigned long long c = 0;
    for (int64_t r = blockIdx.x * (int64_t)blockDim.x + threadIdx.x; r < rows; r += (int64_t)gridDim.x * blockDim.x)
        if (!(__float_as_uint(norm_e1[r]) >> 31)) c += (unsigned long long)(indptr_t[r + 1] - indptr_t[r]);
#pragma unroll
    for (int off = 32; off >= 1; off >>= 1) c += __shfl_down(c, off, 64);
    if ((threadIdx.x & 63) == 0 && c) atomicAdd(out, c);
}
int64_t gm_batch_e1_edges(const gm_batch* b, hipStream_t s) {
    if (b->n_e1_edges >= 0) return b->n_e1_edges;
    const int64_t fallback = b->edges;
    if (!b->d_norm_e1 || !b->d_indptr_t || b->rows <= 0) return fallback;
    unsigned long long* cnt = nullptr; unsigned long long h = 0;
    if (gm_alloc(&cnt, 1, s) != GM_OK) return fallback;
    bool ok = hipMemsetAsync(cnt, 0, 8, s) == hipSuccess;
    if (ok) {
        hipLaunchKernelGGL(k_e1_kept_edges, dim3((int)std::min<int64_t>(512, (b->rows + 255) / 256)), dim3(256), 0, s, b->d_indptr_t, b->d_norm_e1, (int64_t)b->rows, cnt);
        ok = hipMemcpyAsync(&h, cnt, 8, hipMemcpyDeviceToHost, s) == hipSuccess && hipStreamSynchronize(s) == hipSuccess;
    }
    if (!ok) (void)hipGetLastError();
    gm_dev_free(cnt, s);
    return ok ? (b->n_e1_edges = (int64_t)h) : fallback;
}
__global__ void k_fwd_tables(const int4* f2, const int4* f2_feat, const float* norm_c, const float* norm_e1, int64_t rows, int4* tab_c, int4* tab_e1, int4* tab_e1_feat,
                             float* obs_c, float* obs_e1) {
    auto pick = [](const bool on, const int4 t) { return make_int4(on ? t.x : GM_FUSE_ZERO, on ? t.y : GM_FUSE_ZERO, on ? t.z : 0, on ? t.w : 0); };
    for (int64_t r = blockIdx.x * (int64_t)blockDim.x + threadIdx.x; r < rows; r += (int64_t)gridDim.x * blockDim.x) {
        const bool c = !(__float_as_uint(norm_c[r]) >> 31), e = !(__float_as_uint(norm_e1[r]) >> 31);
        const int4 t = f2[r], tf = f2_feat[r];
        tab_c[r] = pick(c, t); tab_e1[r] = pick(e, t); tab_e1_feat[r] = pick(e, tf);
// ... 177 lines not shown
};
struct TabPart { int32_t** d; const std::vector<int32_t>* v; };
static int upload_tables(gm_batch* b, gm_stager& sg, hipStream_t s, std::initializer_list<TabPart> parts) {
    auto pad = [](size_t n) { return (std::max<size_t>(n, 1) + 63) / 64 * 64; };
    size_t tot = 0;
    for (const TabPart& p : parts) tot += pad(p.v->size());
    int32_t* base = nullptr;
    GM_TRY(gm_balloc(b, &base, tot, s));
    std::vector<int32_t> h(tot, 0);
    size_t o = 0;
    for (const TabPart& p : parts) { std::copy(p.v->begin(), p.v->end(), h.begin() + o); *p.d = base + o; o += pad(p.v->size()); }
    return sg.upload(base, h);
}
static std::vector<int32_t> set_spans(const std::vector<int32_t>& off, int step, std::vector<int32_t>* set_first = nullptr) {
    std::vector<int32_t> v;
    if (set_first) set_first->assign(1, 0);
    for (int t = 0; t + 1 < (int)off.size(); ++t) {
        for (int r = off[t]; r < off[t + 1]; r += step) { v.push_back(t); v.push_back(r); v.push_back(std::min(step, off[t + 1] - r)); }
        if (set_first) set_first->push_back((int32_t)(v.size() / 3));
    }
    return v;
}
static int finalize_launch(gm_batch* b, hipStream_t s, gm_stager& sg, FinalizeCtx& fc) {
    gm_phase_timer tm("finalize-launch");
    std::vector<int32_t> sub_set(b->subs), set_chunk_off;
    for (int t = 0; t < b->sets; ++t)
        for (int k = b->h_set_sub_off[t]; k < b->h_set_sub_off[t + 1]; ++k) sub_set[k] = t;
    const std::vector<int32_t> tiles = set_spans(b->h_set_row_off, GM_GEMM_BM), chunks = set_spans(b->h_set_row_off, gm_wgrad_chunk_rows(b->h_set_row_off), &set_chunk_off);
    b->n_tiles = (int32_t)(tiles.size() / 3); b->n_chunks = (int32_t)(chunks.size() / 3);
    GM_TRY(upload_tables(b, sg, s, {{&b->d_sub_set, &sub_set}, {&b->d_tiles, &tiles}, {&b->d_chunks, &chunks}, {&b->d_set_chunk_off, &set_chunk_off}}));
    tm.lap("tables");
    if (b->hop_D > 0) GM_TRY(label_batch(b, s)); else b->d_store_row = b->d_feat_row;
    b->heavy_deg = gm_heavy_deg_for(b->rows, b->edges);
    const int cap = fc.cap = (int)(b->edges / b->heavy_deg + 1);
    const int nc = b->centres; b->n_c = b->subs * nc;
    FinalScratch& lay = fc.lay;
    lay.plan(b->rows, b->n_c, cap);
    GM_TRY(gm_alloc(&fc.scratch, lay.ints, s));
    fc.s = s;
    int32_t* const scr = fc.scratch;
    GM_HIP(hipMemsetAsync(scr, 0, 32, s));
    for (int o = 0; o < 2; ++o) GM_TRY(gm_balloc(b, &b->d_heavy[o], 2 * (size_t)cap, s));
    if (b->edges > 0) {
        GM_TRY(gm_balloc(b, &b->d_enorm[0], (size_t)b->edges, s)); GM_TRY(gm_balloc(b, &b->d_enorm[1], (size_t)b->edges, s)); GM_TRY(gm_balloc(b, &b->d_efeat, (size_t)b->edges, s));
        auto edge_tables = [&](auto kern, auto... w) {
            hipLaunchKernelGGL(kern, dim3(grid_for(b->edges, 4096)), dim3(256), 0, s, b->d_indices, b->d_indices_t, (int64_t)b->edges, b->d_norm, b->d_feat_row, b->d_enorm[0], b->d_enorm[1], b->d_efeat, w...);
        };
        if (b->weighted) edge_tables(k_edge_tables<EdgeW>, EdgeW{b->d_ew[0], b->d_ew[1]}); else edge_tables(k_edge_tables<>);
    }
    GM_TRY(gm_balloc(b, &b->d_norm_c, b->rows, s)); GM_TRY(gm_balloc(b, &b->d_norm_src, b->rows, s));
    if (b->rows > 0) {
        int4 *f0 = nullptr, *ff = nullptr, *fd = nullptr;
        GM_TRY(gm_balloc(b, &f0, (size_t)b->rows, s)); GM_TRY(gm_balloc(b, &ff, (size_t)b->rows, s)); GM_TRY(gm_balloc(b, &fd, (size_t)b->rows, s));
        b->d_fuse2 = f0; b->d_fuse2_feat = ff; b->d_dq_tab = fd;
        auto row_tables = [&](auto kern, auto... w) {
            hipLaunchKernelGGL(kern, dim3(lay.rt_blocks), dim3(256), 0, s, b->d_indptr, b->d_indices, b->d_indptr_t, (int64_t)b->rows, b->d_norm, b->d_feat_row, f0, ff,
                               (unsigned long long*)(scr + lay.o_part), b->d_heavy[0], b->d_heavy[1], scr + lay.o_cnt, cap, b->heavy_deg, b->d_norm_c, (int2*)lay.pairs(scr, 0),
                               (int2*)lay.pairs(scr, 1), lay.first, b->d_norm_src, fd, w...);
        };
        if (b->weighted) row_tables(k_row_tables<RowW>, RowW{b->d_ew[0]}); else row_tables(k_row_tables<>);
    }
    GM_TRY(gm_balloc(b, &b->d_crow, b->n_c, s)); GM_TRY(gm_balloc(b, &b->d_cnorm, b->n_c, s));
    hipLaunchKernelGGL(k_centre_rows, dim3((b->n_c + 255) / 256), dim3(256), 0, s, b->d_sub_off, b->d_centre, nc, b->n_c, b->d_indptr, b->d_norm, b->d_crow, b->d_cnorm, scr + lay.o_cdeg, b->d_norm_c, scr + lay.o_centre, (int4*)b->d_dq_tab);
    GM_HIP(hipGetLastError());
    fc.h_scr = sg.download((const int32_t*)scr, lay.ints);
    GM_REQUIRE(fc.h_scr, GM_ENOMEM, "finalize: pinned staging failed");
    tm.lap("launches");
    return GM_OK;
}
static int finalize_finish(gm_batch* b, hipStream_t s, gm_stager& sg, FinalizeCtx& fc) {
    gm_phase_timer tm("finalize-finish");
    const FinalScratch& lay = fc.lay;
    const int cap = fc.cap, first = lay.first, nc = b->centres;
    const int32_t* h_cnt = fc.h_scr + lay.o_cnt; const int32_t* h_cdeg = fc.h_scr + lay.o_cdeg; const int32_t* h_centre = fc.h_scr + lay.o_centre;
    gm_dev_free(fc.scratch, s); fc.scratch = nullptr;
    if (b->rows > 0) {
        const unsigned long long* h_counts = (const unsigned long long*)(fc.h_scr + lay.o_part);
        unsigned long long nr = 0, ne = 0, ns = 0;
        for (int k = 0; k < lay.rt_blocks; ++k) { nr += h_counts[3 * k]; ne += h_counts[3 * k + 1]; ns += h_counts[3 * k + 2]; }
        b->unfused_rows = (int64_t)nr; b->unfused_edges = (int64_t)ne; b->n_src = (int64_t)ns;
    }
    b->h_centre.assign(h_centre, h_centre + b->n_c);
    b->sched_win = gm_agg_window(b->rows, b->edges);
    std::vector<int32_t> heavy0, tab0;
    for (int o = 0; o < 2; ++o) {
        b->n_heavy[o] = std::min(h_cnt[o], cap);
        if (b->n_heavy[o] > 0) {
            const size_t nh = b->n_heavy[o];
            std::vector<int32_t> h(nh), hd(nh);
            if ((int)nh <= first) { const int32_t* pr = lay.pairs(fc.h_scr, o); for (size_t k = 0; k < nh; ++k) { h[k] = pr[2 * k]; hd[k] = pr[2 * k + 1]; } }
            else {
                const int32_t* a = sg.download(b->d_heavy[o], nh); const int32_t* d = sg.download(b->d_heavy[o] + cap, nh);
                GM_REQUIRE(a && d, GM_ENOMEM, "finalize: pinned staging failed");
                GM_HIP(hipStreamSynchronize(s));
                std::copy(a, a + nh, h.begin()); std::copy(d, d + nh, hd.begin());
            }
            sort_rows_with_degrees(h, hd, b->rows);
            if (nh > 1) GM_TRY(sg.upload(b->d_heavy[o], h));
            tm.lap("hub-sort");
            gm_agg_sched sc;
            GM_TRY(gm_agg_schedule(b, b->rows, b->sched_win, h.data(), hd.data(), b->n_heavy[o], &sc, s, &sg));
            tm.lap("schedule");
            if (o == 0) { heavy0 = h; tab0 = sc.tab; }
            {
                gm_batch::stream_pending& sp = b->spend[o];
                sp.pending = true; sp.has_tab = sc.d_hub != nullptr; sp.n_parts = sc.d_hub ? sc.parts : (int)nh;
                sp.hubs = h; sp.deg = hd; if (sp.has_tab) sp.tab = sc.tab;
            }
            b->d_sched[o] = sc.d_sched; b->sched_len[o] = sc.len; b->d_hub[o] = sc.d_hub; b->d_hub_scratch[o] = sc.d_hub_scratch; b->hub_part[o] = sc.hub_part; b->hub_words[o] = sc.hub_words; b->hub_parts[o] = sc.parts;
        } else b->spend[o].pending = true;
    }
    if (b->d_fuse2 && gm_knob().agg_mid_list) {
        const int64_t n_mid = b->unfused_rows - (int64_t)b->n_heavy[0];
        if (n_mid > 0 && n_mid < b->rows && h_cnt[0] <= cap) {
            const int nb = (int)((b->rows + MID_BLOCK - 1) / MID_BLOCK);
            int32_t* d_bcnt = nullptr;
            GM_TRY(gm_alloc(&d_bcnt, (size_t)nb, s));
            GM_TRY(gm_balloc(b, &b->d_mid, (size_t)n_mid, s));
            hipLaunchKernelGGL(k_mid_count, dim3(nb), dim3(MID_BLOCK), 0, s, b->d_indptr, (int64_t)b->rows, GM_FUSE_MAXDEG + 1, b->heavy_deg, d_bcnt);
            hipLaunchKernelGGL(k_mid_scan, dim3(1), dim3(1024), 0, s, d_bcnt, nb);
            hipLaunchKernelGGL(k_mid_scatter, dim3(nb), dim3(MID_BLOCK), 0, s, b->d_indptr, (int64_t)b->rows, GM_FUSE_MAXDEG + 1, b->heavy_deg, d_bcnt, b->d_mid, (int)n_mid);
            GM_HIP(hipGetLastError());
            gm_dev_free(d_bcnt, s);
            b->n_mid = (int32_t)n_mid;
            int win = 64;
            while (win > 2 && n_mid / win < 16384) win >>= 1;
            if (gm_knob().agg_mid_win > 0) win = gm_knob().agg_mid_win;
            b->mid_win = win;
            if (b->n_heavy[0] > 0 && b->d_sched[0]) {
                std::vector<int32_t> pos(heavy0.size());
                for (size_t k = 0; k < heavy0.size(); ++k) pos[k] = (int32_t)std::min<int64_t>(n_mid - 1, (int64_t)heavy0[k] * n_mid / b->rows);
                GM_TRY(gm_agg_schedule_flat(b, n_mid, win, pos.data(), (int)heavy0.size(), tab0, &b->d_sched_mid, &b->sched_len_mid, s, &sg));
            }
        }
    }
    tm.lap("mid-list");
    std::vector<int32_t> eoff(b->n_c + 1, 0);
    for (int k = 0; k < b->n_c; ++k) eoff[k + 1] = eoff[k] + h_cdeg[k];
    b->n_e1 = eoff[b->n_c];
    int32_t* d_eoff = nullptr;
    GM_TRY(gm_alloc(&d_eoff, eoff.size(), s));
    GM_TRY(sg.upload(d_eoff, eoff));
    GM_TRY(gm_balloc(b, &b->d_e1_row, b->n_e1, s)); GM_TRY(gm_balloc(b, &b->d_e1_par, b->n_e1, s)); GM_TRY(gm_balloc(b, &b->d_e1_norm, b->n_e1, s));
    if (b->weighted) GM_TRY(gm_balloc(b, &b->d_e1_coef, b->n_e1, s));
    auto centre_edges = [&](auto kern, auto... w) {
        hipLaunchKernelGGL(kern, dim3(b->n_c), dim3(64), 0, s, b->d_crow, d_eoff, b->n_c, b->d_indptr, b->d_indices, b->d_norm, b->d_e1_row, b->d_e1_par, b->d_e1_norm, w...);
    };
    if (b->weighted) centre_edges(k_centre_edges<CentreW>, CentreW{b->d_ew[0], b->d_e1_coef}); else centre_edges(k_centre_edges<>);
    GM_HIP(hipGetLastError());
    if (b->rows > 0 && b->d_norm_c) {
        GM_TRY(gm_balloc(b, &b->d_ect, (size_t)b->edges, s)); GM_TRY(gm_balloc(b, &b->d_norm_e1, (size_t)b->rows, s)); GM_TRY(gm_balloc(b, &b->d_n_e1_rows, 1, s));
        hipLaunchKernelGGL(k_e1_tables, dim3(grid_for(std::max<int64_t>(b->edges, b->rows), 4096)), dim3(256), 0, s, b->d_indices_t, (int64_t)b->edges, b->d_norm, b->d_norm_c, (int64_t)b->rows, b->d_ect, b->d_norm_e1, b->d_n_e1_rows);
        if (b->n_e1 > 0) hipLaunchKernelGGL(k_e1_rows, dim3((b->n_e1 + 255) / 256), dim3(256), 0, s, b->d_e1_row, b->n_e1, b->d_norm_e1, b->d_n_e1_rows);
        GM_HIP(hipGetLastError());
        if (b->d_fuse2 && b->d_fuse2_feat) {
            int4 *tc = nullptr, *te = nullptr, *tf = nullptr;
            GM_TRY(gm_balloc(b, &tc, (size_t)b->rows, s)); GM_TRY(gm_balloc(b, &te, (size_t)b->rows, s)); GM_TRY(gm_balloc(b, &tf, (size_t)b->rows, s));
            GM_TRY(gm_balloc(b, &b->d_obs[0], (size_t)b->rows, s)); GM_TRY(gm_balloc(b, &b->d_obs[1], (size_t)b->rows, s));
            hipLaunchKernelGGL(k_fwd_tables, dim3(grid_for(b->rows, 4096)), dim3(256), 0, s, (const int4*)b->d_fuse2, (const int4*)b->d_fuse2_feat, b->d_norm_c, b->d_norm_e1, (int64_t)b->rows,
                               tc, te, tf, b->d_obs[0], b->d_obs[1]);
            GM_HIP(hipGetLastError());
            b->d_fwd_tab[0] = tc; b->d_fwd_tab[1] = te; b->d_fwd_tab_feat = tf;
        }
    }
    std::vector<int32_t> ccoff, ecoff, c_set_off(b->sets + 1), e_set_off(b->sets + 1);
    for (int t = 0; t <= b->sets; ++t) { c_set_off[t] = b->h_set_sub_off[t] * nc; e_set_off[t] = eoff[b->h_set_sub_off[t] * nc]; }
    const std::vector<int32_t> ct = set_spans(c_set_off, GM_GEMM_BM), cc = set_spans(c_set_off, gm_wgrad_chunk_rows(c_set_off), &ccoff), ec = set_spans(e_set_off, gm_wgrad_chunk_rows(e_set_off), &ecoff);
    b->n_c_tiles = (int32_t)(ct.size() / 3); b->n_c_chunks = (int32_t)(cc.size() / 3); b->n_e1_chunks = (int32_t)(ec.size() / 3);
    GM_TRY(upload_tables(b, sg, s, {{&b->d_c_tiles, &ct}, {&b->d_c_chunks, &cc}, {&b->d_c_set_chunk_off, &ccoff}, {&b->d_e1_chunks, &ec}, {&b->d_e1_set_chunk_off, &ecoff}}));
    gm_dev_free(d_eoff, s);
    return GM_OK;
}
static int gm_batch_finalize(gm_batch* const* bs, int n, hipStream_t s, gm_stager& sg, gm_phase_timer* tm = nullptr) {
    FinalizeCtx fc[2];
    for (int p = 0; p < n; ++p) GM_TRY(finalize_launch(bs[p], s, sg, fc[p]));
    GM_HIP(hipStreamSynchronize(s));
    if (tm) tm->lap("finalize-wait");
    for (int p = 0; p < n; ++p) GM_TRY(finalize_finish(bs[p], s, sg, fc[p]));
    return GM_OK;
}

static int batch_alloc(gm_batch* b, hipStream_t s) {
    GM_TRY(gm_balloc(b, &b->d_sub_off, b->subs + 1, s)); GM_TRY(gm_balloc(b, &b->d_set_sub_off, b->sets + 1, s));
    GM_TRY(gm_balloc(b, &b->d_set_row_off, b->sets + 1, s)); GM_TRY(gm_balloc(b, &b->d_graph, b->subs, s));
    GM_TRY(gm_balloc(b, &b->d_parent, b->rows, s)); GM_TRY(gm_balloc(b, &b->d_feat_row, b->rows, s));
    GM_TRY(gm_balloc(b, &b->d_indptr, b->rows + 1, s)); GM_TRY(gm_balloc(b, &b->d_indices, b->edges, s));
    GM_TRY(gm_balloc(b, &b->d_indptr_t, b->rows + 1, s)); GM_TRY(gm_balloc(b, &b->d_indices_t, b->edges, s));
    GM_TRY(gm_balloc(b, &b->d_centre, (size_t)b->subs * b->centres, s)); GM_TRY(gm_balloc(b, &b->d_norm, b->rows, s));
    if (b->weighted) { GM_TRY(gm_balloc(b, &b->d_ew[0], b->edges, s)); GM_TRY(gm_balloc(b, &b->d_ew[1], b->edges, s)); }
    return GM_OK;
}

static int upload_small(gm_batch* b, gm_stager& sg) {
    GM_TRY(sg.upload(b->d_sub_off, b->h_sub_off)); GM_TRY(sg.upload(b->d_set_sub_off, b->h_set_sub_off));
    GM_TRY(sg.upload(b->d_set_row_off, b->h_set_row_off)); GM_TRY(sg.upload(b->d_graph, b->h_graph));
    return GM_OK;
}
struct BatchDrop { void operator()(gm_batch* b) const { gm_batch_destroy(b); } };
typedef std::unique_ptr<gm_batch, BatchDrop> BatchPtr;

struct ExPart { const int32_t* set_offsets; int32_t n_sets; int32_t n_seeds; };
struct ExPlan { bool gpath, p16, needx, sym; int Wmax; size_t Wp; int64_t cap; size_t lds_a, lds_b; };
static ExPlan ex_plan(const gm_store* store, int64_t cap, bool given, int link, int h) {
    ExPlan pl;
    pl.cap = cap; pl.sym = link == GM_LINK_SYMMETRIC;
    pl.Wmax = (int)((store->max_nodes + 31) >> 5);
    const size_t W = (size_t)pl.Wmax;
    pl.gpath = sizeof(uint32_t) * (2 * W + EX_BLOCK + 256 + 16) > 160 * 1024;
    pl.p16 = !pl.gpath && cap < 65536 && gm_knob().extract_pref16;
    pl.needx = !given && link != 1 && h >= 3;
    pl.Wp = pl.p16 ? (W + 1) / 2 : W;
    pl.lds_a = sizeof(uint32_t) * ((pl.gpath ? 0 : W + ((pl.p16 && !pl.needx) ? pl.Wp : W)) + EX_BLOCK + 256 + 16);
    pl.lds_b = sizeof(uint32_t) * ((pl.gpath ? 0 : W + pl.Wp) + EX_BLOCK + 16);
    return pl;
}
struct ExKernels { decltype(&k_nodes<false>) nodes; decltype(&k_fill<false>) fill; decltype(&k_fill<false, false, false, FillW>) fill_w; };
template <bool MASK> static ExKernels ex_kernels_of(const ExPlan& pl) {
    ExKernels k = {};
    if (!pl.gpath) {
        if (pl.sym) { if (!pl.p16) k.nodes = k_nodes<false, false, true, true, MASK>; else if (pl.needx) k.nodes = k_nodes<false, true, true, true, MASK>; else k.nodes = k_nodes<false, true, false, true, MASK>; }
        else if (!pl.p16) k.nodes = k_nodes<false, false, true, false, MASK>;
        else if constexpr (MASK) k.nodes = k_nodes<false, true, false, false, true>;
        else if (pl.needx) k.nodes = k_nodes<false, true, true>; else k.nodes = k_nodes<false, true, false>;
        if (!pl.p16) k.fill = k_fill<false, false, MASK>; else k.fill = k_fill<false, true, MASK>;
        if (!pl.p16) k.fill_w = k_fill<false, false, MASK, FillW>; else k.fill_w = k_fill<false, true, MASK, FillW>;
    } else {
        if (pl.sym) k.nodes = k_nodes<true, false, true, true, MASK>; else k.nodes = k_nodes<true, false, true, false, MASK>;
        k.fill_w = k_fill<true, false, MASK, FillW>; k.fill = k_fill<true, false, MASK>;
    }
    return k;
}
static ExKernels ex_kernels(const ExPlan& pl, bool mask) { return mask ? ex_kernels_of<true>(pl) : ex_kernels_of<false>(pl); }
struct ExBuild {
    const gm_store* store; const gm_seed_t* seeds; int n_parts; const ExPart* parts; int32_t n_seeds, split;
    int32_t h, sample_nodes, link; uint64_t rng_seed;
    bool mask = false;
    const int32_t* nodes_flat; const int64_t* nodes_off;
    hipStream_t st; ExPlan pl; ExKernels kern; ExStore S;
    gm_stager sg;
    BatchPtr bs[2];
    gm_seed_t* d_seeds = nullptr; int32_t *d_nodes = nullptr, *d_degi = nullptr, *d_dego = nullptr, *d_nsub = nullptr, *d_esub = nullptr;
    int32_t* d_given = nullptr; int64_t* d_given_off = nullptr; uint32_t* d_gbits = nullptr;
    int32_t* d_eoff = nullptr; const int32_t* d_order = nullptr;
    const int32_t* nsub = nullptr; const int32_t* esub = nullptr; FillOut fo[2] = {};
    explicit ExBuild(hipStream_t s) : st(s), sg(s) {}
    ~ExBuild() { for (void* p : {(void*)d_gbits, (void*)d_seeds, (void*)d_nodes, (void*)d_degi, (void*)d_dego, (void*)d_nsub, (void*)d_esub, (void*)d_given, (void*)d_given_off, (void*)d_eoff}) gm_dev_free(p, st); }
};
// ... 264 lines not shown
```

g-meta_amd/csrc/gm_internal.h:

```cpp
#pragma once
#include <hip/hip_runtime.h>
#include "gm_bound.h"
#include <stdint.h>
#include <stdio.h>
#include <mutex>
#include <stdlib.h>
#include <string.h>
#include <vector>
#include <algorithm>
#include "../../include/gmeta_hip.h"

#define GM_WAVE 64
#define GM_NXCD 8

void gm_set_error(const char* fmt, ...);

#define GM_HIP(call)                                                                              \
    do {                                                                                          \
        hipError_t e__ = (call);                                                                  \
        if (e__ != hipSuccess) {                                                                  \
            gm_set_error("%s failed: %s (%s:%d)", #call, hipGetErrorString(e__), __FILE__, __LINE__); \
            return GM_EHIP;                                                                       \
        }                                                                                         \
    } while (0)
// ... 51 lines not shown
    float* d_ew = nullptr; float* d_enorm = nullptr; float* d_ew_t = nullptr; float* d_enorm_t = nullptr; int32_t* d_efeat = nullptr;
    int32_t* d_heavy[2] = {nullptr, nullptr}; int32_t n_heavy[2] = {0, 0};
};
struct gm_cone {
    int L = 0; bool ok = false; int heavy_deg = 64;
    gm_cone_level lv[GM_MAX_GCN + 1];
    void* slab = nullptr;
};
struct gm_batch;
int gm_batch_cone(const gm_batch* b, int L, hipStream_t s, const gm_cone** out);
void gm_cone_free(gm_cone* c, hipStream_t s);

struct gm_batch {
    const gm_store* store = nullptr;
    int64_t rows = 0, edges = 0;
    int32_t subs = 0, sets = 0, centres = 1;
    std::vector<int32_t> h_sub_off, h_set_sub_off, h_set_row_off, h_graph;
    int32_t* d_sub_off = nullptr;
    int32_t* d_set_sub_off = nullptr;
    int32_t* d_set_row_off = nullptr;
    int32_t* d_graph = nullptr;
    int32_t* d_parent = nullptr;
    int32_t* d_feat_row = nullptr;
    const float* feat = nullptr; int64_t feat_ld = 0, feat_rows = 0; int32_t feat_dim = 0;
    int32_t hop_D = 0;
    int8_t* d_hop = nullptr;
    int32_t* d_store_row = nullptr;
    int32_t* d_indptr = nullptr;
    int32_t* d_indices = nullptr;
    int32_t* d_indptr_t = nullptr;
    int32_t* d_indices_t = nullptr;
    int32_t* d_centre = nullptr;
    std::vector<int32_t> h_centre;
    float* d_norm = nullptr;
    bool weighted = false;
    bool mask_target = false;
    float* d_ew[2] = {nullptr, nullptr};
    int32_t* d_sub_set = nullptr;
    int32_t* d_tiles = nullptr;
    int32_t n_tiles = 0;
    int32_t* d_chunks = nullptr;
    int32_t n_chunks = 0;
    int32_t* d_set_chunk_off = nullptr;
    int32_t* d_heavy[2] = {nullptr, nullptr};
    int32_t n_heavy[2] = {0, 0};
    int32_t heavy_deg = 64;
    int32_t* d_sched[2] = {nullptr, nullptr};
    int32_t sched_len[2] = {0, 0};
    int32_t sched_win = 0;
    int32_t* d_hub[2] = {nullptr, nullptr}; float* d_hub_scratch[2] = {nullptr, nullptr}; int32_t hub_part[2] = {0, 0};
    int32_t hub_words[2] = {0, 0}, hub_parts[2] = {0, 0};
    mutable int32_t* d_hub2[2] = {nullptr, nullptr}; mutable float* d_hub_scratch2[2] = {nullptr, nullptr};
    mutable hipStream_t hub_stream[4] = {nullptr, nullptr, nullptr, nullptr}; mutable bool hub_used[4] = {false, false, false, false}; mutable hipEvent_t hub_ev[4] = {nullptr, nullptr, nullptr, nullptr};
    float* d_enorm[2] = {nullptr, nullptr}; int32_t* d_efeat = nullptr;
    float* d_gain = nullptr;
    void* d_fuse2 = nullptr; void* d_fuse2_feat = nullptr;
    int64_t unfused_rows = 0, unfused_edges = 0;
    int32_t* d_mid = nullptr; int32_t n_mid = 0, mid_win = 0;
    int32_t* d_sptr[2] = {nullptr, nullptr}; int32_t* d_su[2] = {nullptr, nullptr}; int32_t* d_su_feat = nullptr; float* d_sw[2] = {nullptr, nullptr};
    int32_t* d_scum[2] = {nullptr, nullptr}; int2* d_sseg[2] = {nullptr, nullptr}; int32_t* d_sxord[2] = {nullptr, nullptr};
    int32_t stream_nseg[2] = {0, 0}, stream_nwg[2] = {0, 0}, stream_hubwg[2] = {0, 0}, stream_nparts[2] = {0, 0}, stream_enorm[2] = {0, 0};
    struct stream_pending { bool pending = false; bool has_tab = false; int n_parts = 0; std::vector<int32_t> hubs, deg, tab; };
    mutable stream_pending spend[2];
    int32_t* d_sched_mid = nullptr; int32_t sched_len_mid = 0;
    mutable int64_t unfused_src = -1;
    int32_t n_c = 0;
    int32_t* d_crow = nullptr;
    float* d_cnorm = nullptr;
    float* d_norm_c = nullptr;
    float* d_norm_src = nullptr;
    int64_t n_src = 0;
    void* d_dq_tab = nullptr;
    int32_t n_e1 = 0;
    int32_t* d_e1_row = nullptr;
    int32_t* d_e1_par = nullptr;
    int32_t* d_ect = nullptr;
    float* d_norm_e1 = nullptr;
    int32_t* d_n_e1_rows = nullptr;
    mutable int64_t n_e1_rows = -1;
    mutable int64_t n_e1_edges = -1;
    void* d_fwd_tab[2] = {nullptr, nullptr};
    void* d_fwd_tab_feat = nullptr;
    float* d_obs[2] = {nullptr, nullptr};
    mutable int64_t fwd_cnt[2][3] = {{-1, -1, -1}, {-1, -1, -1}};
    float* d_e1_norm = nullptr;
    float* d_e1_coef = nullptr;
    int32_t* d_c_tiles = nullptr; int32_t n_c_tiles = 0;
    int32_t* d_c_chunks = nullptr; int32_t* d_c_set_chunk_off = nullptr; int32_t n_c_chunks = 0;
    int32_t* d_e1_chunks = nullptr; int32_t* d_e1_set_chunk_off = nullptr; int32_t n_e1_chunks = 0;
    mutable int32_t* d_ro_chunks = nullptr; mutable int32_t* d_ro_multi = nullptr; mutable int32_t n_ro_chunks = 0, n_ro_multi = 0;
    mutable hipStream_t ro_stream = nullptr; mutable hipEvent_t ro_ev = nullptr;
    mutable gm_cone* cone[GM_MAX_GCN + 1] = {};
    hipStream_t stream = nullptr;
    struct slab { char* base; size_t cap, used; };
    std::vector<slab> slabs;
    std::mutex slab_mu;
    mutable hipEvent_t used_ev = nullptr;
};
int gm_batch_gains(const gm_batch* b, hipStream_t s);
int gm_balloc_bytes(gm_batch* b, void** p, size_t bytes, hipStream_t s);
template <class T> static inline int gm_balloc(gm_batch* b, T** p, size_t n, hipStream_t s) { return gm_balloc_bytes(b, (void**)p, (n ? n : 1) * sizeof(T), s); }
void gm_batch_mark_use(const gm_batch* b, hipStream_t st);
int gm_batch_wait_build(const gm_batch* b, hipStream_t s);
static inline int gm_hop_feat_dim(const gm_store* st, int centres, int D) { return st->feat_dim + centres * (D + 2); }

struct gm_knobs {
    int timing;
    int extract_pref16;
    int gemm_mode;
    int gemm_split_min_tiles;
    int centre_store, dead_rows;
    int fuse_agg, head_stage;
    int fuse_diff;
    int agg_mid_win;
    int agg_mid_list;
    int query_streams;
    int head_threads;
    int split16_min_rows;
    int split_pieces;
    int wgrad_split_min_chunks;
    int agg_stream;
    int agg_stream_min_rows;
    int neg_round;
    int pair_lanes;
    int cand_round;
    int walk_chunk;
    int walk_lanes;
    int ppr_chunk;
    int ppr_cols;
    int dist_chunk;
    int dist_cols;
    int dist_plane_kib;
    int cand_bitmap;
    int sketch_chunk;
    int sketch_mib;
    int prop_chunk;
    int prop_mib;
};
const gm_knobs& gm_knob();

int gm_nbr_index(const gm_store* s);
void gm_nbr_release(const gm_store* s);
int gm_pair_lanes(const gm_store* s, int32_t g, const char* what, int* lpp);
int gm_pair_scores_launch(const gm_store* s, int32_t g, int lpp, const int32_t* d_pairs, int64_t n, int mask, float* d_out, hipStream_t st);

#define GM_CAND_THREADS 256
#define GM_CAND_WAVES (GM_CAND_THREADS / GM_WAVE)
#define GM_CAND_MAX_K 1024

__device__ __forceinline__ unsigned long long gm_cand_key(uint32_t score_bits, int32_t w) {
    return ((unsigned long long)score_bits << 32) | (unsigned long long)(0xFFFFFFFFu - (uint32_t)w);
}

__device__ __forceinline__ int gm_cand_scan(int v, int* part, int* total) {
    const int lane = (int)threadIdx.x & (GM_WAVE - 1), wave = (int)threadIdx.x / GM_WAVE;
    int inc = v;
#pragma unroll
    for (int o = 1; o < GM_WAVE; o <<= 1) { const int t = __shfl_up(inc, o, GM_WAVE); if (lane >= o) inc += t; }
    __syncthreads();
    if (lane == GM_WAVE - 1) part[wave] = inc;
    __syncthreads();
    int base = 0, tot = 0;
#pragma unroll
    for (int w = 0; w < GM_CAND_WAVES; ++w) { const int p = part[w]; tot += p; if (w < wave) base += p; }
    *total = tot;
    return base + inc;
}

__device__ __forceinline__ void gm_cand_sort_write(unsigned long long* sk, int cnt, int k, int64_t o, int32_t* __restrict__ out_nodes, float* __restrict__ out_scores) {
    const int tid = (int)threadIdx.x;
    int S = 1;
    while (S < cnt) S <<= 1;
    for (int i = cnt + tid; i < S; i += GM_CAND_THREADS) sk[i] = 0ull;
    __syncthreads();
    for (int size = 2; size <= S; size <<= 1) {
        for (int stride = size >> 1; stride > 0; stride >>= 1) {
            for (int t = tid; t < (S >> 1); t += GM_CAND_THREADS) {
                const int i = ((t & ~(stride - 1)) << 1) | (t & (stride - 1)), j = i + stride;
                const unsigned long long x = sk[i], y = sk[j];
                const bool desc = (i & size) == 0;
                if (desc ? x < y : x > y) { sk[i] = y; sk[j] = x; }
            }
            __syncthreads();
        }
    }
    for (int j = tid; j < k; j += GM_CAND_THREADS) {
        const unsigned long long key = j < cnt ? sk[j] : 0ull;
        out_nodes[o + j] = j < cnt ? (int32_t)(0xFFFFFFFFu - (uint32_t)key) : -1;
        out_scores[o + j] = j < cnt ? __uint_as_float((uint32_t)(key >> 32)) : 0.f;
    }
}

static inline int gm_store_call_check(const char* what, const gm_store* s, int32_t g, const char* cnt_name = nullptr, int64_t n = 0, int32_t flags = 0) {
    GM_REQUIRE(s, GM_EINVAL, "%s: store is NULL", what);
    GM_REQUIRE(g >= 0 && g < s->n_graphs, GM_EINVAL, "%s: graph %d of a store with %d graph(s)", what, g, s->n_graphs);
    if (!cnt_name) return GM_OK;
    GM_REQUIRE(n >= 0 && n <= (int64_t)INT32_MAX, GM_EINVAL, "%s: %s = %lld", what, cnt_name, (long long)n);
// ... 42 lines not shown
        return h;
    }
};

struct gm_scratch {
    hipStream_t st;
    std::vector<void*> p;
    explicit gm_scratch(hipStream_t s) : st(s) {}
    ~gm_scratch() { for (void* q : p) gm_dev_free(q, st); }
    gm_scratch(const gm_scratch&) = delete;
    gm_scratch& operator=(const gm_scratch&) = delete;
    template <class T> int take(T** d, size_t n) {
        GM_TRY(gm_alloc(d, n, st));
        p.push_back((void*)*d);
        return GM_OK;
    }
    template <class T> int put(T** d, const std::vector<T>& v, gm_stager& sg) {
        GM_TRY(take(d, v.size()));
        return sg.upload(*d, v);
    }
};

struct gm_nbr_graph;
struct gm_pprc {
    int32_t k = 0, wgs_max = 0; hipStream_t st = nullptr;
    void* cols = nullptr;
    int32_t *hist = nullptr, *cnt = nullptr, *total = nullptr, *ties = nullptr;
    unsigned long long* surv = nullptr;
};
int gm_pprc_prepare(gm_pprc* w, gm_scratch& sc, int32_t Bmax, int32_t k, hipStream_t st);
int gm_pprc_round(const gm_pprc& w, const gm_nbr_graph& G, float* P, int32_t Br, const int32_t* d_src, const int32_t* d_row, const int32_t* d_col, int64_t c0, int64_t rows,
                  int32_t* d_out_nodes, float* d_out_scores, int32_t* d_out_total, gm_phase_timer* tm);

int gm_prof_transpose(hipStream_t st, const uint64_t* next, int32_t W, int64_t N, const int32_t* flag, uint64_t* plane);
int gm_prof_count(hipStream_t st, const uint64_t* T, int32_t D, int64_t B, int64_t N, const int32_t* cu, const int32_t* cv, const int64_t* dst, int64_t cnt, int32_t* out);

struct gm_layout {
    int n_gcn;
    int dims[GM_MAX_GCN + 1];
    int n_out, link, hc;
    int readout;
    int64_t w_off[GM_MAX_GCN], b_off[GM_MAX_GCN], wl_off, bl_off, P;
};
int gm_make_layout(const gm_model_t* m, gm_layout* L);
static inline int gm_check_feat_dim(const gm_batch* b, int dims0, const char* what) {
    if (dims0 == b->feat_dim || dims0 == b->feat_ld) return GM_OK;
    if (b->hop_D) gm_set_error("%s: dims[0]=%d but the batch has %d features (%d of the store + %d hop-label columns, gm_set_hop_labels(%d))", what, dims0, b->feat_dim,
                               b->store->feat_dim, b->feat_dim - b->store->feat_dim, b->hop_D);
    else gm_set_error("%s: dims[0]=%d but the store has %d features", what, dims0, b->feat_dim);
    return GM_EINVAL;
}
static inline int gm_pad_feat(int F) { return F <= 32 ? 32 : (F + 63) / 64 * 64; }

struct gm_agg_args {
    const int32_t* indptr;
    const int32_t* indices;
    const float* x;
    const int32_t* x_row;
    const float* e_w;
    const int32_t* x_idx;
    int skip_on, skip_lo, skip_hi;
    int64_t ldx;
    const float* s_in;
    const float* s_out;
    int keep_signed;
    const float* mask_h;
    const uint8_t* mask_b;
    uint8_t* relu_bits;
    const float* bias;
    int64_t bias_stride;
    const int32_t* set_row_off;
    int n_sets;
    int relu;
    float* out;
    int64_t rows;
    int width;
    const int32_t* heavy;
    int n_heavy;
    int heavy_deg;
    const int32_t* sched;
    int sched_len, sched_win;
    const int32_t* hub; float* hub_scratch; int hub_part;
    const int32_t* rowlist; int64_t n_list; int list_win;
    const gm_batch* stream; int stream_o; int stream_feat; int64_t stream_xrows;
    int* launched;
};
#define GM_AGG_ID_LPR(LPR) ((LPR) == 64 ? 6 : (LPR) == 32 ? 5 : (LPR) == 16 ? 4 : (LPR) == 8 ? 3 : (LPR) == 4 ? 2 : 1)
#define GM_AGG_ID_ONE(VEC, LPR) (100 + ((VEC) == 4 ? 10 : 0) + GM_AGG_ID_LPR(LPR))
#define GM_AGG_ID_WIN(LPR, NCH) (200 + 16 * ((NCH) == 2 ? 3 : GM_AGG_ID_LPR(LPR) - 4))
#define GM_AGG_ID_WIN_SCHED 1
#define GM_AGG_ID_WIN_SPLIT 2
#define GM_AGG_ID_WIN_HEAVY 4
#define GM_AGG_ID_WIN_LIST 8
#define GM_AGG_ID_STREAM(LPR, SPLIT) (300 + 2 * (GM_AGG_ID_LPR(LPR) - 4) + ((SPLIT) ? 1 : 0))
int gm_agg_stream_args(gm_agg_args& a, const gm_batch* b, int o, bool gather, hipStream_t s);
bool gm_stream_ok(const gm_agg_args& g);
bool gm_stream_batch_ok(const gm_batch* b, int o);
int gm_launch_stream(const gm_agg_args& g, int nt, hipStream_t s);
int gm_stream_tables(gm_batch* b, int o, const int32_t* hubs_host, const int32_t* deg_host, int n_hubs, int n_parts, const std::vector<int32_t>* part_tab, hipStream_t s,
                     gm_stager* sg);
#define GM_FUSE_SELF 0x40000000
#define GM_FUSE_ZERO 0x20000000
const float* gm_zero_row(hipStream_t s);
#ifndef GM_ZERO_ROWS
#define GM_ZERO_ROWS 1
#endif
#define GM_FUSE_MAXDEG 2
#define GM_AGG_HUB_LD 512
struct gm_agg_sched { int32_t* d_sched = nullptr; int32_t len = 0; int32_t* d_hub = nullptr; float* d_hub_scratch = nullptr; int32_t hub_part = 0; int32_t hub_words = 0, parts = 0;
                      std::vector<int32_t> tab; };
int gm_batch_hub_order(const gm_batch* b, int o, hipStream_t s, int set = 0);
int gm_batch_hub_alt(const gm_batch* b, hipStream_t s);
template <class A> inline int gm_agg_hub(A& a, const gm_batch* b, int o, hipStream_t s, int set = 0) {
    const bool alt = set == 1 && b->d_hub2[o];
    a.hub = alt ? b->d_hub2[o] : b->d_hub[o]; a.hub_scratch = alt ? b->d_hub_scratch2[o] : b->d_hub_scratch[o]; a.hub_part = b->hub_part[o];
    return a.hub ? gm_batch_hub_order(b, o, s, alt ? 1 : 0) : GM_OK;
}
int gm_agg_window(int64_t rows, int64_t edges);
struct gm_stager;
int gm_agg_schedule_flat(gm_batch* b, int64_t rows, int win, const int32_t* pos, int n_heavy, const std::vector<int32_t>& tab, int32_t** d_sched, int32_t* len, hipStream_t s, gm_stager* sg);
int gm_agg_schedule(gm_batch* b, int64_t rows, int win, const int32_t* heavy_host, const int32_t* heavy_deg_host, int n_heavy, gm_agg_sched* out, hipStream_t s, gm_stager* sg);
int gm_heavy_deg();
int gm_heavy_deg_for(int64_t rows, int64_t edges);
int gm_launch_aggregate(const gm_agg_args& a, hipStream_t s);

struct gm_gemm_args {
    const float* A; int64_t lda;
    const float* B; int64_t b_stride;
    int transB;
    float* C; int64_t ldc;
    int K, N;
    const float* row_scale;
    const float* row_scale_keep;
    int64_t n_keep;
    const float* bias; int64_t bias_stride;
    int relu;
    const float* mask_h;
    const uint8_t* mask_b;
    uint8_t* relu_bits;
    const uint16_t* Bsplit; int64_t bsplit_stride;
    const void* fuse2; const float* zside; int64_t ldz;
    int np; gm_bound a_bound, b_bound; unsigned* amax_out;
    float* zero_out;
    const int32_t* tiles;
    int n_tiles;
    int64_t rows;
    int* launched;
};
#define GM_GEMM_ID_GLDS4 1
#define GM_GEMM_ID_GLDS2 2
#define GM_GEMM_ID_GLDS1 3
#define GM_GEMM_ID_GLDS_SMALL 4
#define GM_GEMM_ID_NN(WC, VEC, TB) (10 + 4 * ((WC) == 4 ? 2 : (WC) == 2 ? 1 : 0) + 2 * (VEC) + (TB))
#define GM_GEMM_ID_SPLIT(GATHER, MI, WC, NP) (30 + 10 * (GATHER) + ((MI) == 2 ? 0 : (WC) == 4 ? 2 : 4) + ((NP) == 2))
#define GM_GEMM_BM 128
int gm_launch_gemm_nn(const gm_gemm_args& a, hipStream_t s);
int gm_gemm_mode();
bool gm_gemm_split_ok(int n_tiles, int K, int N);
int gm_split_weights(const float* params, int64_t pstride, int64_t w_off, int K, int N, int trans, int sets, uint16_t* out, hipStream_t s, int np = 3,
                     gm_bound bound = gm_no_bound());
int gm_amax(const float* x, int64_t stride, int64_t off, int64_t n, int sets, unsigned* out, int64_t out_stride, hipStream_t s);
int gm_amax_segs(const float* x, const int64_t* off, const int64_t* n, int segs, unsigned* out, int64_t out_stride, hipStream_t s);
int gm_split_np();

struct gm_wgrad_hold { int n = 0; int sets[GM_MAX_GCN] = {}; alignas(16) unsigned char slot[GM_MAX_GCN][256] = {}; };
struct gm_wgrad_args {
    const float* A; int64_t lda; int K;
    const int32_t* a_row;
    const float* G; int64_t ldg; int N;
    const float* Gb; int64_t ldgb;
    const float* a_scale;
    const int32_t* chunks;
    int n_chunks;
    const int32_t* set_chunk_off;
    int sets;
    float* partial;
    float* dW; int64_t dw_stride;
    float* db; int64_t db_stride;
    const float* sgd_cur; int64_t sgd_cur_stride; float* sgd_next; int64_t sgd_next_stride; float sgd_lr;
    int64_t w_off, b_off;
    int np; gm_bound a_bound, g_bound; int pl_np; gm_bound pl_bound;
    uint16_t* pl_fwd; uint16_t* pl_dz;
    float* wt_next;
    int64_t rows;
    const void* fuse2; const float* gx; int64_t ldgx;
    int64_t a_rows;
    const float* g_keep;
    gm_wgrad_hold* hold; int hold_this;
    int pick;
};
#define GM_WGRAD_PICK_EXACT 1
#define GM_WGRAD_PICK_SPLIT 2
#define GM_WGRAD_ROWS 1024
int gm_launch_wgrad(const gm_wgrad_args& a, hipStream_t s);
bool gm_wgrad_gather_ok(int n_chunks, int K, int N);

int gm_num_cus();
int gm_func_full_lds(const void* fn);
#define GM_WGRAD_EXTRA_ROUND_PCT 25
static inline int gm_wgrad_chunk_rows(const std::vector<int32_t>& set_off, int n_cu = gm_num_cus()) {
    const int sets = (int)set_off.size() - 1;
    int64_t total = 0; int mx = 1;
    for (int t = 0; t < sets; ++t) { const int n = set_off[t + 1] - set_off[t]; total += n; mx = n > mx ? n : mx; }
// ... 49 lines not shown
```

g-meta_amd/csrc/model.hip:

```cpp
#include <algorithm>
#include <atomic>
#include <map>
#include <stdlib.h>
#include "gm_internal.h"


__device__ __forceinline__ float wave_sumf(float v) {
#pragma unroll
    for (int o = 32; o > 0; o >>= 1) v += __shfl_xor(v, o, 64);
    return v;
}

struct HeadK {
    const float* H; int64_t ldh; int Hd;
    const int32_t* sub_off; const int32_t* centre; int nc; const int32_t* sub_set; const int32_t* set_sub_off;
    const float* params; int64_t pstride; int64_t wl_off, bl_off; int hc, C; int subs;
    int compact;
    unsigned* dq_amax;
    int subs_per_set;
};

__device__ __forceinline__ int64_t centre_row(const HeadK& k, int s, int which) {
    return k.compact ? (int64_t)s * k.nc + which : (int64_t)k.sub_off[s] + k.centre[s * k.nc + which];
}
// ... 488 lines not shown
        const int e = (int)(id / F), f = (int)(id - (int64_t)e * F);
        const float h = H1[(int64_t)e_row[e] * F + f];
        G1[id] = h > 0.f ? e_norm[e] * T2[(int64_t)e_par[e] * F + f] : 0.f;
    }
}

__global__ __launch_bounds__(256) void k_transpose_w(const float* params, int64_t pstride, int64_t w_off, int fi, int fo, float* WT) {
    __shared__ float tile[32][33];
    const int t = blockIdx.z, k0 = blockIdx.x * 32, n0 = blockIdx.y * 32;
    const float* W = params + (int64_t)t * pstride + w_off;
    float* O = WT + (int64_t)t * fi * fo;
    const int tx = threadIdx.x & 31, ty = threadIdx.x >> 5;
    for (int r = ty; r < 32; r += 8) { const int n = n0 + r, k = k0 + tx; tile[r][tx] = (n < fi && k < fo) ? W[(int64_t)n * fo + k] : 0.f; }
    __syncthreads();
    for (int r = ty; r < 32; r += 8) { const int k = k0 + r, n = n0 + tx; if (k < fo && n < fi) O[(int64_t)k * fi + n] = tile[tx][r]; }
}

__global__ void k_colsum_rows(const float* G, int64_t ldg, int N, const int32_t* set_off, float* db, int64_t db_stride, SgdK u, int64_t b_off) {
    const int set = blockIdx.x, r0 = set_off[set], r1 = set_off[set + 1];
    for (int n = threadIdx.x; n < N; n += blockDim.x) {
        float s = 0.f;
        for (int r = r0; r < r1; ++r) s += G[(int64_t)r * ldg + n];
        db[(int64_t)set * db_stride + n] = s;
        if (u.next) u.next[(int64_t)set * u.next_stride + b_off + n] = u.cur[(int64_t)set * u.cur_stride + b_off + n] - u.lr * s;
    }
}

__global__ void k_finalize(const float* gq, const float* gp, int64_t stride, int64_t P, int T, const float* lq, const float* aq, int K1, float* out,
                           int64_t cut, int64_t shift, const unsigned* viol) {
    const int64_t tot = P + 2 * K1 + 1 + (int64_t)T * K1;
    const unsigned vw = viol ? *viol : 0u;
    for (int64_t id = blockIdx.x * (int64_t)blockDim.x + threadIdx.x; id <= tot; id += (int64_t)gridDim.x * blockDim.x) {
        float s = 0.f;
        if (id == tot) { out[id] = (float)vw; continue; }
        if (id < P) { const int64_t src = id < cut ? id : id + shift; if (gq) for (int t = 0; t < T; ++t) s += gq[t * stride + src] + gp[t * stride + src]; }
        else if (id < P + K1) { for (int t = 0; t < T; ++t) s += lq[t * K1 + (id - P)]; if (vw && id == P + K1 - 1) s = __uint_as_float(0x7fc00000u); }
        else if (id < P + 2 * K1) { for (int t = 0; t < T; ++t) s += aq[t * K1 + (id - P - K1)]; }
        else if (id == P + 2 * K1) s = (float)T;
        else s = aq[id - P - 2 * K1 - 1];
        out[id] = s;
    }
}

struct Carver {
    char* base; int64_t used = 0, cap;
    Carver(void* p, int64_t c) : base((char*)p), cap(c) {}
    template <class T> T* take(int64_t n) {
        const int64_t bytes = ((n > 0 ? n : 1) * (int64_t)sizeof(T) + 255) / 256 * 256;
        T* r = base ? (T*)(base + used) : nullptr;
        used += bytes;
        return r;
    }
    bool ok() const { return !base || used <= cap; }
};

#define GM_W_HEADROOM 1024.f
struct PlaneDir {
    const float* fw0 = nullptr; int64_t TP = 0; int K = 0;
    uint16_t* base = nullptr; int64_t per_k = 0;
    int64_t off[GM_MAX_GCN][2] = {};
    bool valid[64][GM_MAX_GCN][2] = {};
    int index_of(const float* params) const {
        if (!base || !fw0 || params < fw0) return 0;
        const int64_t d = params - fw0;
        if (d % TP) return 0;
        const int64_t k = d / TP + 1;
        return (k >= 1 && k <= K && k < 64) ? (int)k : 0;
    }
    uint16_t* slot(int k, int l, int o) const { return (k && off[l][o] >= 0) ? base + (int64_t)(k - 1) * per_k + off[l][o] : nullptr; }
    uint16_t* lookup(const float* params, int l, int o) const { const int k = index_of(params); return (k && off[l][o] >= 0 && valid[k][l][o]) ? slot(k, l, o) : nullptr; }
    unsigned* wam = nullptr; const float* theta = nullptr;
    unsigned* viol = nullptr;
    bool w_bound(const float* params, int l, gm_bound& bd) const {
        bd = gm_no_bound();
        if (!wam || !(index_of(params) || params == theta)) return false;
        bd.amax = wam + (int64_t)l * GM_BOUND_PAD; bd.stride = 0; bd.gain = nullptr; bd.hgain = GM_W_HEADROOM; bd.viol = viol;
        return true;
    }
};

enum PassKind { PASS_PLAIN = 0, PASS_FWD_ONLY = 1, PASS_DIFF = 2 };
enum RowSet { ROWS_ALL, ROWS_SRC, ROWS_E1, ROWS_CENTRE };
enum DqFill { DQ_MEMSET, DQ_ZEROED, DQ_CENTRE };
struct LayerPlan { bool split, fuse; RowSet formed, stored; bool relu_bits; };
struct PassPlan { PassKind kind; LayerPlan layer[GM_MAX_GCN]; DqFill dq; bool t_centre, dq_e1; };

struct GcnCtx {
    const gm_batch* b; gm_layout L;
    PlaneDir* pd;
    bool is_support = false;
    PassPlan plan = {};
    bool t_zero = false;
    float* Z[GM_MAX_GCN]; float* H[GM_MAX_GCN]; float* X0; float* bufA; float* bufB; float* partial;
    float* partial_l[GM_MAX_GCN];
    gm_wgrad_hold hold;
    uint16_t* Wsplit;
    float* WTl[GM_MAX_GCN];
    const float* wt_of[GM_MAX_GCN]; int64_t wt_stride[GM_MAX_GCN];
    uint8_t* M[GM_MAX_GCN];
    float* cG2; float* cT2; float* cG1; float* partial_c;
    float* Pool; float* Gpool; float* ro_part;
    const float* x0_user; const int32_t* centre; int z1_valid;
    int zw[GM_MAX_GCN];
    const gm_cone* cone;
    SgdK sgd;
    int hub_set = 0;
    int np = 3; unsigned* am = nullptr; int am_passes = 0, am_pass = -1;
    const unsigned* feat_bound = nullptr;
    bool hv[GM_MAX_GCN] = {}, tv[GM_MAX_GCN] = {}; bool dqv = false;
    unsigned* am_slot(int i) const { return am + ((int64_t)am_pass * (2 * L.n_gcn + 1) + i) * b->sets * GM_BOUND_PAD; }
    unsigned* amH(int l) const { return am_slot(l); }
    unsigned* amT(int l) const { return am_slot(L.n_gcn + l); }
    unsigned* amdQ() const { return am_slot(2 * L.n_gcn); }
};
static bool in_bound(const GcnCtx& c, int l, gm_bound& bd) {
    bd = gm_no_bound();
    if (c.np != 2 || c.am_pass < 0 || !c.b->d_gain) return false;
    if (l == 0) {
        if (c.x0_user || !c.feat_bound) return false;
        bd.amax = c.feat_bound; bd.stride = 1;
    } else {
        if (!c.hv[l - 1]) return false;
        bd.amax = c.amH(l - 1); bd.stride = GM_BOUND_PAD;
    }
    bd.gain = c.b->d_gain; bd.hgain = 1.f;
    return true;
}
static bool dq_bound(const GcnCtx& c, int l, gm_bound& bd) {
    bd = gm_no_bound();
    if (c.np != 2 || c.am_pass < 0 || !c.b->d_gain) return false;
    if (l == c.L.n_gcn - 1) { if (!c.dqv) return false; bd.amax = c.amdQ(); bd.gain = nullptr; }
    else { if (!c.tv[l + 1]) return false; bd.amax = c.amT(l + 1); bd.gain = c.b->d_gain + 1; }
    bd.stride = GM_BOUND_PAD; bd.hgain = 1.f;
    return true;
}
static int weight_planes(GcnCtx& c, const float* params, int64_t pstride, int l, int o, hipStream_t st, gm_gemm_args& g) {
    const int fi = c.L.dims[l], fo = c.L.dims[l + 1];
    const bool want16 = o ? dq_bound(c, l, g.a_bound) : in_bound(c, l, g.a_bound);
    uint16_t* have = (c.pd && pstride) ? c.pd->lookup(params, l, o) : nullptr;
    g.b_bound = gm_no_bound(); g.np = 3; g.bsplit_stride = pstride ? (int64_t)3 * fi * fo : 0;
    if (have && c.np == 2) {
        if (want16 && c.pd->w_bound(params, l, g.b_bound)) g.np = 2; else have = nullptr;
    }
    if (!have) {
        if (want16 && c.pd && c.pd->w_bound(params, l, g.b_bound)) g.np = 2; else g.b_bound = gm_no_bound();
        GM_TRY(gm_split_weights(params, pstride, c.L.w_off[l], o ? fo : fi, o ? fi : fo, o, pstride ? c.b->sets : 1, c.Wsplit, st, g.np, g.b_bound));
        have = c.Wsplit;
    }
    g.Bsplit = have;
    if (g.np == 2) { g.amax_out = o ? c.amT(l) : c.amH(l); (o ? c.tv : c.hv)[l] = true; }
    return GM_OK;
}

static bool mean_readout(const GcnCtx& c) { return c.L.readout == GM_READOUT_MEAN; }
static int64_t readout_chunk_count(const gm_batch* b);
static int readout_tables(const gm_batch* b, hipStream_t s);
static int readout_fwd(const GcnCtx& c, hipStream_t st);
static int readout_bwd(const GcnCtx& c, hipStream_t st);

static void wgrad_sgd(gm_wgrad_args& w, const GcnCtx& c, int l) {
    w.sgd_cur = c.sgd.cur; w.sgd_cur_stride = c.sgd.cur_stride; w.sgd_next = c.sgd.next; w.sgd_next_stride = c.sgd.next_stride; w.sgd_lr = c.sgd.lr;
    w.w_off = c.L.w_off[l]; w.b_off = c.L.b_off[l];
}

static void gcn_carve(GcnCtx& c, Carver& cv) {
    const gm_layout& L = c.L; const int64_t rows = c.b->rows;
    int maxd = 0; int64_t maxkn = 0;
    if (c.cone) {
// ... 106 lines not shown

static int partial_agg_bytes(const gm_batch* b, RowSet formed, int fi, bool gather, hipStream_t st, int64_t* bytes, int64_t* strict) {
    const bool all = formed == ROWS_ALL;
    int64_t w[3] = {std::min<int64_t>(b->unfused_rows, row_view(b, formed, gather).n), b->unfused_edges, std::min<int64_t>(b->unfused_edges, b->rows)};
    if (gm_prof_enabled() && all) w[2] = gm_batch_unfused_sources(b, st);
    if (gm_prof_enabled() && !all) GM_TRY(gm_batch_fwd_counts(b, row_view(b, formed, gather).obs, st, w));
    const int64_t pb0 = 4 * (b->rows + 1) + (all ? 4 : 8) * b->unfused_rows + 4 * w[1] + 4 * w[0] * (int64_t)fi;
    *bytes = pb0 + 4 * w[2] * (int64_t)fi;
    *strict = pb0 + 4 * (gather ? std::min<int64_t>(w[2], b->feat_rows) : w[2]) * (int64_t)fi;
    gm_prof_note(GM_PROF_AGG_BOUND, pb0 + 4 * std::min<int64_t>(w[1], b->rows) * (int64_t)fi - *bytes);
    return GM_OK;
}
static int64_t t_centre_agg_bytes(const gm_batch* b, RowSet out, int fi, bool maskbits, hipStream_t st) {
    const int64_t n_out = rows_kept(b, out, st), e_out = (out == ROWS_E1 && gm_prof_enabled()) ? gm_batch_e1_edges(b, st) : b->edges;
    return 4 * (b->rows + 1) + 4 * b->rows + 4 * e_out + (maskbits ? n_out * (int64_t)fi / 4 : 0) + 4 * ((int64_t)b->n_c + n_out) * (int64_t)fi;
}

static bool dz_split_ok(const GcnCtx& c, int l) { return c.Wsplit && gm_gemm_split_ok(c.b->n_tiles, c.L.dims[l + 1], c.L.dims[l]); }
static bool dz_centre_ok(const GcnCtx& c, int l) { return dz_split_ok(c, l) && c.L.dims[l + 1] >= 64 && c.L.dims[l + 1] <= 4096 && c.b->d_dq_tab; }
static float* t_zero_rows(const GcnCtx& c) {
    const gm_layout& L = c.L; const int Lg = L.n_gcn;
    if (c.cone || Lg < 2 || !c.bufB || L.dims[Lg - 1] > L.dims[Lg]) return nullptr;
    for (int l = 0; l < Lg - 1; ++l) if (std::min(L.dims[l], L.dims[l + 1]) > L.dims[Lg - 1]) return nullptr;
    return c.bufB + c.b->rows * (int64_t)L.dims[Lg - 1];
}
static int dead_row_level(const GcnCtx& c) { return (gm_knob().centre_store == 0 || c.centre) ? 0 : gm_knob().dead_rows; }
static int t_zero_fill(GcnCtx& c, hipStream_t st) {
    float* z = t_zero_rows(c);
    c.t_zero = z && dead_row_level(c) >= 2 && dz_centre_ok(c, c.L.n_gcn - 1) && c.b->d_ect && c.b->d_norm_e1;
    if (c.t_zero) GM_HIP(hipMemsetAsync(z, 0, sizeof(float) * GM_ZERO_ROWS * c.L.dims[c.L.n_gcn - 1], st));
    return GM_OK;
}

int gm_gather_rows(const gm_batch* b, const int32_t* feat_row, int64_t n, int F, float* out, hipStream_t st);
static int cone_forward(GcnCtx& c, const float* params, int64_t pstride, float* logits, hipStream_t st, int reuse_z1, int skip_head);
static int cone_backward(GcnCtx& c, const float* params, int64_t pstride, const float* dlogits, float* dparams, int64_t dstride, hipStream_t st, int skip_head);

static std::atomic<int> g_fuse_agg_override{-1};
extern "C" void gm_set_fuse_agg(int32_t on) { g_fuse_agg_override.store(on < 0 ? -1 : (on ? 1 : 0), std::memory_order_relaxed); }
extern "C" int32_t gm_get_fuse_agg(void) { const int o = g_fuse_agg_override.load(std::memory_order_relaxed); return o >= 0 ? o : gm_knob().fuse_agg; }

static int plan_check(const GcnCtx& c, const PassPlan& p) {
    for (int l = 0; l < c.L.n_gcn; ++l) {
        GM_REQUIRE(p.layer[l].formed == ROWS_ALL || p.layer[l].fuse, GM_EINVAL, "plan: layer %d is formed on a row set but not fused: nothing reads it through the set's table", l);
        GM_REQUIRE(p.layer[l].formed != ROWS_CENTRE || (l == c.L.n_gcn - 1 && p.layer[l].stored == ROWS_CENTRE && (l > 0 || c.x0_user)), GM_EINVAL, "plan: layer %d is formed on the centre rows, but is not a last layer that stores them alone and reads no feature table", l);
    }
    GM_REQUIRE(!(p.kind == PASS_DIFF && p.layer[c.L.n_gcn - 1].formed == ROWS_CENTRE) || p.dq == DQ_CENTRE, GM_EINVAL, "plan: a restricted differentiated pass must leave dQ to its centre rows");
    GM_REQUIRE(!p.dq_e1 || p.t_centre, GM_EINVAL, "plan: dQ_{L-1} on the sources of the centres' in-edges needs T_L on its centre rows");
    return GM_OK;
}
static int plan_check(const GcnCtx& c, const PassPlan& p);
static int plan_pass(const GcnCtx& c, const float* params, int64_t pstride, PassKind kind, int reuse_z1, PassPlan* plan) {
    const gm_layout& L = c.L; const gm_batch* b = c.b;
    const int Lg = L.n_gcn, last = Lg - 1, level = dead_row_level(c), centre_store = gm_knob().centre_store;
    const bool mean = mean_readout(c);
    auto agg_first = [&](int l) { return L.dims[l] <= L.dims[l + 1]; };
    auto wgrad_tabled = [&](int l) { return gm_wgrad_gather_ok(b->n_chunks, L.dims[l], L.dims[l + 1]); };
    PassPlan p{}; p.kind = kind; p.dq = DQ_MEMSET;
    for (int l = 0; l < Lg; ++l) {
        LayerPlan& lp = p.layer[l]; const int fi = L.dims[l];
        lp.relu_bits = !agg_first(l) || kind != PASS_FWD_ONLY;
        if (!agg_first(l)) continue;
        lp.split = c.Wsplit && gm_gemm_split_ok(b->n_tiles, fi, L.dims[l + 1]) && ((uintptr_t)(params + L.b_off[l]) & 15) == 0 && pstride % 4 == 0;
        const bool gather = (l == 0 && !c.x0_user);
        const bool keeps_stream = gm_knob().fuse_diff == 2 && c.is_support && gm_knob().agg_stream && gm_stream_batch_ok(b, 0);
        const bool diff_ok = kind == PASS_DIFF && gm_knob().fuse_diff && !keeps_stream && c.np != 2 && !c.cone && wgrad_tabled(l);
        lp.fuse = (kind == PASS_FWD_ONLY || diff_ok) && gm_get_fuse_agg() && lp.split && !(l == 0 && reuse_z1) && fi >= 64 && fi % 4 == 0 && b->d_fuse2 && b->d_enorm[0] &&
                  (!gather || (b->feat_ld % 4 == 0 && b->feat_ld >= fi)) &&
                  2 * b->unfused_rows <= b->rows;
        if (l == last) { if (!mean && !c.centre && b->d_norm_c && (centre_store >= 2 || (centre_store == 1 && kind == PASS_FWD_ONLY))) lp.stored = ROWS_CENTRE; }
        else if (level >= 1 && lp.split && (kind == PASS_FWD_ONLY || (kind == PASS_DIFF && c.M[l])) && L.dims[l + 1] <= L.dims[l + 2] && b->d_norm_src) lp.stored = ROWS_SRC;
    }
    if (kind == PASS_DIFF && agg_first(last) && !mean)
        p.dq = (level >= 1 && p.layer[last].split && c.np != 2 && b->d_norm_c && (last == 0 || dz_centre_ok(c, last)) && wgrad_tabled(last)) ? DQ_CENTRE : DQ_ZEROED;
    p.t_centre = p.dq == DQ_CENTRE && c.t_zero && level >= 2;
    p.dq_e1 = p.t_centre && Lg == 2 && agg_first(0) && c.np != 2 && wgrad_tabled(0);
    const bool last_ok = !mean && c.np != 2 && b->d_norm_c && b->d_norm_e1 && b->d_fwd_tab[0] && b->d_obs[0] && agg_first(last) && p.layer[last].fuse;
    const bool below_ok = Lg >= 2 && agg_first(Lg - 2) && b->d_fwd_tab[1] && b->d_fwd_tab_feat && b->d_obs[1];
    const bool fwd3 = kind == PASS_FWD_ONLY && level >= 3 && centre_store >= 1 && last_ok && (Lg >= 2 || c.x0_user);
    const bool diff4 = kind == PASS_DIFF && level >= 4 && centre_store >= 2 && p.t_centre && !reuse_z1 && Lg >= 2 && last_ok;
    if (fwd3 || diff4) p.layer[last].formed = ROWS_CENTRE;
    if (below_ok && ((fwd3 && p.layer[Lg - 2].split) || (diff4 && p.dq_e1 && p.layer[0].fuse && c.M[0]))) {
        p.layer[Lg - 2].stored = ROWS_E1; if (p.layer[Lg - 2].fuse) p.layer[Lg - 2].formed = ROWS_E1; }
    *plan = p; return plan_check(c, p);
}

static int gcn_forward(GcnCtx& c, const float* params, int64_t pstride, float* logits, hipStream_t st, int reuse_z1, int skip_head = 0, PassKind kind = PASS_PLAIN) {
    if (c.cone) return cone_forward(c, params, pstride, logits, st, reuse_z1, skip_head);
    const gm_layout& L = c.L; const gm_batch* b = c.b;
    if (!c.x0_user) GM_TRY(gm_check_feat_dim(b, L.dims[0], "forward"));
    GM_REQUIRE((L.link != 0) == (b->centres == 2), GM_EINVAL, "forward: link_pred model needs a 2-centre batch and vice versa");
    const float* xin = c.x0_user;
    GM_TRY(plan_pass(c, params, pstride, kind, reuse_z1, &c.plan));
    const PassPlan& plan = c.plan; const bool mean = mean_readout(c);
    if (mean) GM_TRY(readout_tables(b, st));
    if (c.np == 2) {
        ++c.am_pass;
        GM_REQUIRE(c.am_pass < c.am_passes, GM_EINVAL, "forward: more passes than bound slots (%d)", c.am_passes);
        for (int l = 0; l < GM_MAX_GCN; ++l) c.hv[l] = c.tv[l] = false;
        c.dqv = false;
    }
    for (int l = 0; l < L.n_gcn; ++l) {
        const int fi = L.dims[l], fo = L.dims[l + 1];
        const bool gather = (l == 0 && !c.x0_user);
        const LayerPlan& lp = plan.layer[l]; uint8_t* relu_bits = lp.relu_bits ? c.M[l] : nullptr;
        if (fi > fo) {
            const float* A = xin; int64_t lda = fi;
            if (gather) { GM_TRY(gm_gather_rows(b, b->d_feat_row, b->rows, fi, c.X0, st)); A = c.X0; }
            gm_gemm_args g{}; g.A = A; g.lda = lda; g.B = params + L.w_off[l]; g.b_stride = pstride; g.C = c.Z[l]; g.ldc = fo; g.K = fi; g.N = fo;
            g.row_scale = b->d_norm; g.tiles = b->d_tiles; g.n_tiles = b->n_tiles; g.rows = b->rows;
            GM_TRY(gm_launch_gemm_nn(g, st));
            gm_agg_args a; GM_TRY(batch_agg(c, 0, st, a));
            a.x = c.Z[l]; a.ldx = fo; a.s_out = b->d_norm;
            a.bias = params + L.b_off[l]; a.bias_stride = pstride; a.set_row_off = b->d_set_row_off; a.n_sets = b->sets; a.relu = 1;
            a.out = c.H[l]; a.width = fo; a.relu_bits = relu_bits;
            GM_TRY(launch_agg(a, gm_aggregate_bytes(b, fo), gm_aggregate_bytes(b, fo), st));
        } else {
            const float* x = gather ? b->feat : xin; const int64_t ldx = gather ? b->feat_ld : fi;
            if (!(l == 0 && reuse_z1 && c.z1_valid)) {
                gm_agg_args a; GM_TRY(batch_agg(c, 0, st, a));
                a.s_in = b->d_norm; a.e_w = b->d_enorm[0]; a.out = c.Z[l]; a.width = fi;
                a.x = x; a.ldx = ldx; if (gather) { a.x_row = b->d_feat_row; a.x_idx = b->d_efeat; }
                if (lp.fuse) {
                    a.skip_on = 1; a.skip_lo = 0; a.skip_hi = GM_FUSE_MAXDEG;
                    if (b->d_mid && c.hub_set == 0 && gm_knob().agg_mid_list && (b->n_heavy[0] == 0 || b->d_sched_mid)) {
                        a.rowlist = b->d_mid; a.n_list = b->n_mid; a.list_win = b->mid_win;
                        if (b->n_heavy[0] > 0) { a.sched = b->d_sched_mid; a.sched_len = b->sched_len_mid; a.sched_win = b->mid_win; }
                        else { a.sched = nullptr; a.sched_len = 0; }
                    }
                    if (lp.formed != ROWS_ALL) { a.s_out = row_view(b, lp.formed, gather).sign; a.keep_signed = 1; }
                    int64_t pb, pbs;
                    GM_TRY(partial_agg_bytes(b, lp.formed, fi, gather, st, &pb, &pbs));
                    GM_TRY(launch_agg(a, pb, pbs, st));
                } else {
                    if (a.e_w) GM_TRY(gm_agg_stream_args(a, b, 0, gather, st));
                    int64_t strict = gm_aggregate_bytes(b, fi);
                    if (gather) strict += 4 * b->rows - 4 * b->rows * (int64_t)fi + std::min<int64_t>(4 * b->rows * (int64_t)fi, 4 * b->feat_rows * (int64_t)fi);
                    GM_TRY(launch_agg(a, gm_aggregate_bytes(b, fi), strict, st));
                    if (l == 0) c.z1_valid = 1;
                }
            }
            gm_gemm_args g{}; g.A = c.Z[l]; g.lda = fi; g.B = params + L.w_off[l]; g.b_stride = pstride; g.C = c.H[l]; g.ldc = fo; g.K = fi; g.N = fo;
            g.row_scale = b->d_norm; g.bias = params + L.b_off[l]; g.bias_stride = pstride; g.relu = 1; g.tiles = b->d_tiles; g.n_tiles = b->n_tiles; g.rows = b->rows;
            g.relu_bits = relu_bits;
            if (lp.stored != ROWS_ALL) { g.row_scale_keep = row_view(b, lp.stored, false).keep; g.n_keep = rows_kept(b, lp.stored, st); }
            if (lp.split) {
                GM_TRY(weight_planes(c, params, pstride, l, 0, st, g));
                GM_REQUIRE(!(l == L.n_gcn - 1 && plan.dq == DQ_CENTRE) || g.np == 3, GM_EINVAL, "forward: dQ is left to its centre rows, which needs the three-piece kernels");
            }
            if (l == L.n_gcn - 1 && plan.dq == DQ_ZEROED) g.zero_out = c.bufA;
            if (lp.fuse) { g.A = x; g.lda = ldx; g.zside = c.Z[l]; g.ldz = fi; g.fuse2 = row_view(b, lp.formed, gather).tab; }
            GM_TRY(gm_launch_gemm_nn(g, st));
        }
        xin = c.H[l];
    }
    if (mean) GM_TRY(readout_fwd(c, st));
    return skip_head ? GM_OK : launch_head_fwd(c, params, pstride, logits, st);
}

static int gcn_backward_sparse(GcnCtx& c, const float* params, int64_t pstride, const float* dlogits, float* dparams, int64_t dstride, hipStream_t st, int skip_head);
static bool sparse_bwd_ok(const gm_layout& L);

static int gcn_backward(GcnCtx& c, const float* params, int64_t pstride, const float* dlogits, float* dparams, int64_t dstride, hipStream_t st, int sparse = 0,
                        int skip_head = 0) {
    if (c.cone) return cone_backward(c, params, pstride, dlogits, dparams, dstride, st, skip_head);
    if (sparse && sparse_bwd_ok(c.L)) return gcn_backward_sparse(c, params, pstride, dlogits, dparams, dstride, st, skip_head);
    const gm_layout& L = c.L; const gm_batch* b = c.b; const int Lg = L.n_gcn;
    float* dQ = c.bufA; float* T = c.bufB;
    c.hold.n = 0;
    const PassPlan& plan = c.plan;
    const bool dq_centre = skip_head && plan.dq == DQ_CENTRE;
    const bool t_centre = dq_centre && plan.t_centre, dq_e1 = t_centre && plan.dq_e1;
    const bool dq_filled = !skip_head && !mean_readout(c);
    if (!skip_head && mean_readout(c)) {
        GM_TRY(launch_head_bwd(c, params, pstride, dlogits, dparams, dstride, nullptr, c.Gpool, st));
        GM_TRY(readout_bwd(c, st));
    } else if (!skip_head) {
        GM_HIP(hipMemsetAsync(dQ, 0, sizeof(float) * b->rows * L.dims[Lg], st));
        GM_TRY(launch_head_bwd(c, params, pstride, dlogits, dparams, dstride, dQ, nullptr, st));
    }
    for (int l = Lg - 1; l >= 0; --l) {
        const int fi = L.dims[l], fo = L.dims[l + 1];
        const float* Xprev = l > 0 ? c.H[l - 1] : (c.x0_user ? c.x0_user : c.X0);
        const float* maskprev = l > 0 ? c.H[l - 1] : nullptr;
        const uint8_t* maskbits = l > 0 ? c.M[l - 1] : nullptr;
        if (maskbits) maskprev = nullptr;
        gm_wgrad_args w{}; w.chunks = b->d_chunks; w.n_chunks = b->n_chunks; w.set_chunk_off = b->d_set_chunk_off; w.sets = b->sets; w.rows = b->rows;
        w.partial = c.partial; w.dW = dparams + L.w_off[l]; w.dw_stride = dstride; w.db = dparams + L.b_off[l]; w.db_stride = dstride;
        w.a_scale = b->d_norm; w.K = fi; w.N = fo;
        wgrad_sgd(w, c, l);
        w.hold = &c.hold; w.hold_this = l > 0 ? 1 : 0;
        if (l > 0) w.partial = c.partial_l[l];
        if (fi > fo) {
            gm_agg_args a; GM_TRY(batch_agg(c, 1, st, a));
            a.x = dQ; a.ldx = fo; a.s_in = b->d_norm; a.e_w = b->d_enorm[1]; a.out = T; a.width = fo;
            GM_TRY(launch_agg(a, gm_aggregate_bytes(b, fo), gm_aggregate_bytes(b, fo), st));
            w.A = Xprev; w.lda = fi; w.G = T; w.ldg = fo; w.Gb = dQ; w.ldgb = fo;
            GM_TRY(gm_launch_wgrad(w, st));
            if (l > 0) {
                gm_gemm_args g{}; g.A = T; g.lda = fo; g.B = params + L.w_off[l]; g.b_stride = pstride; g.transB = 1; g.C = dQ; g.ldc = fi; g.K = fo; g.N = fi;
                g.row_scale = b->d_norm; g.mask_h = maskprev; g.mask_b = maskbits; g.tiles = b->d_tiles; g.n_tiles = b->n_tiles; g.rows = b->rows;
                GM_TRY(gm_launch_gemm_nn(g, st));
            }
        } else {
            w.A = c.Z[l]; w.lda = fi; w.G = dQ; w.ldg = fo;
            const RowSet g_rows = (dq_centre && l == Lg - 1) ? ROWS_CENTRE : (dq_e1 && l == Lg - 2) ? ROWS_E1 : ROWS_ALL;
            w.g_keep = row_view(b, g_rows, false).keep;
            const RowSet z_rows = plan.layer[l].formed;
            if (plan.layer[l].fuse) {
                const bool gather = l == 0 && !c.x0_user;
                w.fuse2 = row_view(b, z_rows, gather).tab;
                w.gx = gather ? b->feat : (l > 0 ? c.H[l - 1] : c.x0_user); w.ldgx = gather ? b->feat_ld : fi;
            }
            if (z_rows != ROWS_ALL) {
                GM_REQUIRE(w.g_keep || dq_filled, GM_EINVAL, "backward: layer %d was formed on its observable rows only, but its weight gradient got neither flagged rows of G (g_keep) nor a dQ this call zero-filled", l);
                if (gm_prof_enabled()) w.a_rows = rows_kept(b, z_rows, st);
            }
            if (l > 0) {
                gm_gemm_args g{}; g.A = dQ; g.lda = fo; g.C = T; g.ldc = fi; g.K = fo; g.N = fi;
                g.row_scale = b->d_norm; g.tiles = b->d_tiles; g.n_tiles = b->n_tiles; g.rows = b->rows;
                const bool use_split = dz_split_ok(c, l);
                const bool use_wt = !use_split && c.WTl[l] && fi % 64 == 0 && fo % 16 == 0;
                if (use_split) {
                    GM_TRY(weight_planes(c, params, pstride, l, 1, st, g));
                    g.B = params + L.w_off[l]; g.b_stride = pstride; g.transB = 1;
                    if (dq_centre && l == Lg - 1) { g.fuse2 = b->d_dq_tab; g.zside = dQ; g.ldz = fo; }
                    if (t_centre && l == Lg - 1) { g.row_scale_keep = row_view(b, ROWS_CENTRE, false).keep; g.n_keep = rows_kept(b, ROWS_CENTRE, st); }
                } else if (use_wt) {
                    if (!(c.wt_of[l] == params && c.wt_stride[l] == pstride)) {
                        const int nt = pstride ? b->sets : 1;
                        hipLaunchKernelGGL(k_transpose_w, dim3((fo + 31) / 32, (fi + 31) / 32, nt), dim3(256), 0, st, params, pstride, L.w_off[l], fi, fo, c.WTl[l]);
                        GM_HIP(hipGetLastError());
                        c.wt_of[l] = params; c.wt_stride[l] = pstride;
                    }
                    g.B = c.WTl[l]; g.b_stride = pstride ? (int64_t)fi * fo : 0; g.transB = 0;
                } else { g.B = params + L.w_off[l]; g.b_stride = pstride; g.transB = 1; }
                GM_TRY(gm_launch_gemm_nn(g, st));
                if (use_wt && c.sgd.next) { w.wt_next = c.WTl[l]; }
            }
            int kn = 0;
            if (c.pd && c.sgd.next && (kn = c.pd->index_of(c.sgd.next)) != 0) { w.pl_fwd = c.pd->slot(kn, l, 0); w.pl_dz = c.pd->slot(kn, l, 1); }
            if (c.np == 2) {
                gm_bound ab, gb;
                if (in_bound(c, l, ab) && dq_bound(c, l, gb)) { w.np = 2; w.a_bound = ab; w.g_bound = gb; }
                if (kn) {
                    if (c.pd->w_bound(c.sgd.next, l, w.pl_bound)) w.pl_np = 2; else { w.pl_fwd = nullptr; w.pl_dz = nullptr; }
                }
            }
            GM_TRY(gm_launch_wgrad(w, st));
            if (kn) { c.pd->valid[kn][l][0] = w.pl_fwd != nullptr; c.pd->valid[kn][l][1] = w.pl_dz != nullptr; }
            if (w.wt_next) { c.wt_of[l] = c.sgd.next; c.wt_stride[l] = c.sgd.next_stride; }
            if (l > 0) {
                gm_agg_args a; GM_TRY(batch_agg(c, 1, st, a));
                a.x = T; a.ldx = fi; a.s_out = b->d_norm; a.mask_h = maskprev; a.mask_b = maskbits;
                a.out = dQ; a.width = fi;
                int64_t by = gm_aggregate_bytes(b, fi);
                if (t_centre && l == Lg - 1) {
                    a.x_idx = b->d_ect;
                    const RowSet out = dq_e1 ? ROWS_E1 : ROWS_ALL;
                    if (dq_e1) { a.s_out = row_view(b, out, false).keep; a.keep_signed = 1; }
                    by = t_centre_agg_bytes(b, out, fi, maskbits != nullptr, st);
                }
                GM_TRY(launch_agg(a, by, by, st));
            }
        }
    }
    return GM_OK;
}

static bool sparse_bwd_ok(const gm_layout& L) {
    if (L.n_gcn > 2 || L.readout == GM_READOUT_MEAN) return false;
    for (int l = 0; l < L.n_gcn; ++l) if (L.dims[l] > L.dims[l + 1]) return false;
    return true;
}

static int gcn_backward_sparse(GcnCtx& c, const float* params, int64_t pstride, const float* dlogits, float* dparams, int64_t dstride, hipStream_t st, int skip_head) {
    const gm_layout& L = c.L; const gm_batch* b = c.b;
    const int Lg = L.n_gcn, fiL = L.dims[Lg - 1], foL = L.dims[Lg];
    if (!skip_head) GM_TRY(launch_head_bwd(c, params, pstride, dlogits, dparams, dstride, nullptr, c.cG2, st));
    gm_wgrad_args w{}; w.A = c.Z[Lg - 1]; w.lda = fiL; w.K = fiL; w.a_row = b->d_crow; w.a_scale = b->d_cnorm; w.G = c.cG2; w.ldg = foL; w.N = foL;
    w.rows = b->n_c; w.chunks = b->d_c_chunks; w.n_chunks = b->n_c_chunks; w.set_chunk_off = b->d_c_set_chunk_off; w.sets = b->sets; w.partial = c.partial_c;
    w.dW = dparams + L.w_off[Lg - 1]; w.dw_stride = dstride; w.db = dparams + L.b_off[Lg - 1]; w.db_stride = dstride;
    wgrad_sgd(w, c, Lg - 1);
    GM_TRY(gm_launch_wgrad(w, st));
    if (Lg == 1) return GM_OK;
    gm_gemm_args g{}; g.A = c.cG2; g.lda = foL; g.B = params + L.w_off[Lg - 1]; g.b_stride = pstride; g.transB = 1; g.C = c.cT2; g.ldc = fiL; g.K = foL; g.N = fiL;
    g.row_scale = b->d_cnorm; g.tiles = b->d_c_tiles; g.n_tiles = b->n_c_tiles; g.rows = b->n_c;
    GM_TRY(gm_launch_gemm_nn(g, st));
    if (b->n_e1 > 0) {
        const int64_t tot = (int64_t)b->n_e1 * fiL;
        hipLaunchKernelGGL(k_expand_edges, dim3((int)std::min<int64_t>(2048, (tot + 255) / 256)), dim3(256), 0, st, c.cT2, c.H[0], fiL, b->d_e1_row, b->d_e1_par,
                           b->weighted ? b->d_e1_coef : b->d_e1_norm, b->n_e1, c.cG1);
        GM_HIP(hipGetLastError());
    }
    const int f0 = L.dims[0];
    gm_wgrad_args w1{}; w1.A = c.Z[0]; w1.lda = f0; w1.K = f0; w1.a_row = b->d_e1_row; w1.a_scale = b->d_e1_norm; w1.G = c.cG1; w1.ldg = fiL; w1.N = fiL;
    w1.rows = b->n_e1; w1.chunks = b->d_e1_chunks; w1.n_chunks = b->n_e1_chunks; w1.set_chunk_off = b->d_e1_set_chunk_off; w1.sets = b->sets; w1.partial = c.partial_c;
    w1.dW = dparams + L.w_off[0]; w1.dw_stride = dstride; w1.db = dparams + L.b_off[0]; w1.db_stride = dstride;
    wgrad_sgd(w1, c, 0);
    GM_TRY(gm_launch_wgrad(w1, st));
    return GM_OK;
}



static int64_t cone_agg_bytes(int64_t n_dst, int64_t n_src, int64_t nnz, int width) {
    return 4 * (n_dst + 1) + 4 * nnz + 4 * n_dst + 4 * (n_src + n_dst) * (int64_t)width;
}
static int cone_launch_agg(const gm_agg_args& a, int64_t n_src, int64_t nnz, hipStream_t st) {
    const int64_t by = cone_agg_bytes(a.rows, n_src, nnz, a.width);
    return launch_agg(a, by, by, st);
}
static gm_agg_args cone_agg(const gm_cone* cn, const gm_cone_level& up, int transposed) {
    gm_agg_args a{};
    a.indptr = transposed ? up.d_indptr_t : up.d_indptr; a.indices = transposed ? up.d_indices_t : up.d_indices;
    a.heavy = up.d_heavy[transposed]; a.n_heavy = up.n_heavy[transposed]; a.heavy_deg = cn->heavy_deg;
    a.e_w = transposed ? up.d_ew_t : up.d_ew;
    return a;
}

static int cone_forward(GcnCtx& c, const float* params, int64_t pstride, float* logits, hipStream_t st, int reuse_z1, int skip_head) {
    const gm_layout& L = c.L; const gm_batch* b = c.b; const gm_cone* cn = c.cone;
    GM_TRY(gm_check_feat_dim(b, L.dims[0], "forward"));
    GM_REQUIRE((L.link != 0) == (b->centres == 2), GM_EINVAL, "forward: link_pred model needs a 2-centre batch and vice versa");
    GM_REQUIRE(!c.x0_user && !c.centre, GM_EINVAL, "forward: the cone schedule reads features and centres from the batch");
    const float* xin = nullptr;
    for (int l = 0; l < L.n_gcn; ++l) {
        const gm_cone_level& lo = cn->lv[l]; const gm_cone_level& up = cn->lv[l + 1];
        const int fi = L.dims[l], fo = L.dims[l + 1];
        if (fi > fo) {
            const float* A = xin;
            if (l == 0) { GM_TRY(gm_gather_rows(b, lo.d_feat_row, lo.n, fi, c.X0, st)); A = c.X0; }
            gm_gemm_args g{}; g.A = A; g.lda = fi; g.B = params + L.w_off[l]; g.b_stride = pstride; g.C = c.Z[l]; g.ldc = fo; g.K = fi; g.N = fo;
            g.row_scale = lo.d_norm; g.tiles = lo.d_tiles; g.n_tiles = lo.n_tiles; g.rows = lo.n;
            GM_TRY(gm_launch_gemm_nn(g, st));
            gm_agg_args a = cone_agg(cn, up, 0);
            a.x = c.Z[l]; a.ldx = fo; a.s_out = up.d_norm; a.bias = params + L.b_off[l]; a.bias_stride = pstride; a.set_row_off = up.d_set_off; a.n_sets = b->sets;
            a.relu = 1; a.out = c.H[l]; a.rows = up.n; a.width = fo;
            GM_TRY(cone_launch_agg(a, lo.n, up.nnz, st));
        } else {
            if (!(l == 0 && reuse_z1 && c.z1_valid)) {
                gm_agg_args a = cone_agg(cn, up, 0);
                a.s_in = lo.d_norm; a.e_w = up.d_enorm; a.out = c.Z[l]; a.rows = up.n; a.width = fi; a.ldx = fi;
                if (l == 0) { a.x = b->feat; a.x_row = lo.d_feat_row; a.x_idx = up.d_efeat; a.ldx = b->feat_ld; } else a.x = xin;
                GM_TRY(cone_launch_agg(a, lo.n, up.nnz, st));
                if (l == 0) c.z1_valid = 1;
// ... 1144 lines not shown
```

include/gmeta_hip.h:

```cpp
#ifndef GMETA_HIP_H
#define GMETA_HIP_H
#include <stdint.h>
#ifdef __cplusplus
extern "C" {
#endif

#define GM_OK 0
#define GM_EINVAL (-1)
#define GM_ENOMEM (-2)
#define GM_EHIP (-3)
#define GM_ERANGE (-4)
#define GM_MAX_GCN 4

typedef struct gm_store gm_store_t;
typedef struct gm_batch gm_batch_t;

typedef struct gm_seed { int32_t graph, i, j; } gm_seed_t;

typedef struct gm_model {
    int32_t n_gcn;
    int32_t dims[GM_MAX_GCN + 1];
    int32_t n_out;
    int32_t link_pred;
} gm_model_t;
// ... 69 lines not shown
#define GM_LINK_SYMMETRIC 2
#define GM_LINK_MASK_TARGET 4
int gm_extract(const gm_store_t* store, const gm_seed_t* seeds, int32_t n_seeds,
               const int32_t* set_offsets, int32_t n_sets, int32_t h, int32_t sample_nodes,
               uint64_t rng_seed, int32_t link_pred, void* stream, gm_batch_t** out);
int gm_extract_pair(const gm_store_t* store, const gm_seed_t* seeds_a, int32_t n_seeds_a, const int32_t* set_offsets_a, int32_t n_sets_a,
                    const gm_seed_t* seeds_b, int32_t n_seeds_b, const int32_t* set_offsets_b, int32_t n_sets_b,
                    int32_t h, int32_t sample_nodes, uint64_t rng_seed, int32_t link_pred, void* stream,
                    gm_batch_t** out_a, gm_batch_t** out_b);
int gm_batch_from_nodes(const gm_store_t* store, const gm_seed_t* seeds, int32_t n_seeds,
                        const int32_t* set_offsets, int32_t n_sets, const int32_t* nodes_flat,
                        const int64_t* nodes_off, int32_t link_pred, void* stream, gm_batch_t** out);
void gm_set_hop_labels(int32_t D);
int32_t gm_get_hop_labels(void);
int32_t gm_batch_hop_labels(const gm_batch_t* b);
int32_t gm_batch_mask_target(const gm_batch_t* b);
int gm_batch_concat(const gm_batch_t* const* parts, int32_t n_parts, void* stream, gm_batch_t** out);
int gm_batch_prepare_cone(const gm_batch_t* b, int32_t n_gcn, void* stream);
int gm_batch_prepare_cone_pair(const gm_batch_t* a, const gm_batch_t* b, int32_t n_gcn, void* stream);
int gm_batch_cone_dims(const gm_batch_t* b, int32_t n_gcn, int32_t* ok, int64_t* level_rows, int64_t* level_edges);
int gm_batch_cone_read(const gm_batch_t* b, int32_t n_gcn, int32_t level, int32_t what, void* host, int64_t host_bytes);
void gm_batch_destroy(gm_batch_t* b);

int gm_batch_dims(const gm_batch_t* b, int64_t* rows, int64_t* edges, int32_t* subs, int32_t* sets,
                  int32_t* centres);
enum gm_field {
    GM_F_SUB_OFF = 0,
    GM_F_SET_SUB_OFF,
    GM_F_PARENT,
    GM_F_GRAPH,
    GM_F_INDPTR,
    GM_F_INDICES,
    GM_F_INDPTR_T,
    GM_F_INDICES_T,
    GM_F_CENTRE,
    GM_F_NORM,
    GM_F_FEAT_ROW,
    GM_F_NORM_SRC,
    GM_F_NORM_CENTRE,
    GM_F_EDGE_W,
    GM_F_EDGE_W_T = 14,
    GM_F_HOP = 15,
    GM_F_NORM_E1 = 16,
    GM_F_EDGE_CENTRE_T = 17,
    GM_F_OBS_CENTRE = 18,
    GM_F_OBS_E1 = 19
};
int32_t gm_batch_weighted(const gm_batch_t* b);
int gm_batch_read(const gm_batch_t* b, int32_t field, void* host_dst, int64_t bytes);
int gm_batch_device_ptr(const gm_batch_t* b, int32_t field, void** dptr);
int gm_batch_source_rows(const gm_batch_t* b, int64_t* n_rows);
int gm_batch_e1_source_rows(const gm_batch_t* b, int64_t* n_rows);

int gm_gather_features(const gm_batch_t* b, float* x_out, void* stream);

int gm_aggregate(const gm_batch_t* b, int32_t transposed, int32_t gather, const float* x, int32_t width,
                 const float* s_in, const float* s_out, float* out, void* stream);
int64_t gm_aggregate_bytes(const gm_batch_t* b, int32_t width);

int64_t gm_model_param_count(const gm_model_t* m);
int64_t gm_gcn_ws_bytes(const gm_batch_t* b, const gm_model_t* m);
int gm_gcn_forward(const gm_batch_t* b, const gm_model_t* m, const float* params, int64_t param_stride,
                   const float* x0, const int32_t* centre_local, float* logits, void* ws, int64_t ws_bytes,
                   void* stream);
int gm_gcn_backward(const gm_batch_t* b, const gm_model_t* m, const float* params, int64_t param_stride,
                    const float* x0, const int32_t* centre_local, const float* dlogits, float* dparams,
                    int64_t dparam_stride, void* ws, int64_t ws_bytes, void* stream);

int gm_dense_update(const gm_batch_t* b, const float* x, int32_t K, const float* W, int64_t w_stride, int32_t N, float* out, int32_t mode,
                    void* stream);
int gm_dense_gemm(const gm_batch_t* b, const float* x, int64_t ldx, int32_t K, const float* W, int64_t w_stride, int32_t trans_w, int32_t N,
                  float* out, int64_t ldc, const float* s, const float* s_keep, const float* bias, int64_t bias_stride, int32_t relu,
                  uint8_t* relu_bits, const float* mask_h, const uint8_t* mask_b, float* zero_out, uint32_t* amax_out, int32_t mode,
                  int32_t* launched, void* stream);
int gm_dense_fused_gemm(const gm_batch_t* b, int32_t table, const float* x, int64_t ldx, int32_t K, const float* zside, int64_t ldz, const float* zfull,
                        int64_t ldzf, const float* W, int64_t w_stride, int32_t N, float* out, int64_t ldc, const float* s, const float* s_keep,
                        const float* bias, int64_t bias_stride, int32_t relu, uint8_t* relu_bits, float* zero_out, uint32_t* amax_out, int32_t mode,
                        int32_t* launched, void* stream);
int gm_dense_aggregate(const gm_batch_t* b, int32_t transposed, int32_t x_src, const float* x, int64_t ldx, int32_t width, int32_t scale_src,
                       const float* s_in, const float* s_out, int32_t keep_signed, const float* bias, int64_t bias_stride, int32_t relu,
                       uint8_t* relu_bits, const float* mask_h, const uint8_t* mask_b, int32_t hubs, const int32_t* rowlist, int64_t n_list,
                       int32_t list_win, int32_t list_sched, int32_t skip_lo, int32_t skip_hi, int32_t stream_ok, float* out, int32_t* launched,
                       void* stream);
int gm_dense_agg_info(const gm_batch_t* b, int32_t transposed, int64_t* info);
int gm_dense_fuse_counts(const gm_batch_t* b, int64_t* counts);
int gm_dense_agg_table(const gm_batch_t* b, int32_t which, int32_t transposed, void* dst, int64_t n, void* stream);
int gm_dense_dz_centre(const gm_batch_t* b, const float* dQ, int32_t K, const float* W, int64_t w_stride, int32_t N, float* T, void* stream);
int gm_dense_wgrad_centre(const gm_batch_t* b, const float* x, int32_t Kx, const float* dQ, int32_t N, float* dW, int64_t dw_stride, float* db,
                          int64_t db_stride, void* stream);
int gm_dense_agg_centre_t(const gm_batch_t* b, float* T, int32_t width, const uint8_t* mask_b, float* out, int32_t keep, void* stream);
int gm_dense_wgrad_e1(const gm_batch_t* b, const float* x, int32_t Kx, const float* dQ, int32_t N, float* dW, int64_t dw_stride, float* db,
                      int64_t db_stride, void* stream);
int gm_dense_wgrad(const gm_batch_t* b, const float* x, int64_t ldx, int32_t K, const float* g, int64_t ldg, int32_t N, const float* s,
                   const float* gb, int64_t ldgb, float* dW, int64_t dw_stride, float* db, int64_t db_stride, int32_t mode,
                   const float* cur, float* next, int64_t p_stride, float lr, float* wt, uint16_t* pl_fwd, uint16_t* pl_dz, void* stream);
int gm_dense_wgrad_fused(const gm_batch_t* b, int32_t table, const float* A, int64_t lda, int32_t K, const float* gx, int64_t ldgx, const float* g,
                         int64_t ldg, int32_t N, const float* s, const float* g_keep, float* dW, int64_t dw_stride, float* db, int64_t db_stride,
                         int32_t mode, void* stream);

int gm_proto_loss_spt(const gm_batch_t* b, const float* logits, int32_t n_out, const int32_t* y, int32_t n_support,
                      float* loss, float* acc, float* protos, float* dlogits, void* stream);
int gm_proto_loss_qry(const gm_batch_t* b, const float* logits, int32_t n_out, const int32_t* y, const float* protos,
                      int32_t c_task, float* loss, float* acc, float* dlogits, float* dprotos, void* stream);
void gm_set_ragged_classes(int32_t on);
int32_t gm_get_ragged_classes(void);
int gm_dense_head_loss(const gm_batch_t* b, const float* H, int32_t Hd, int32_t nc, int32_t compact, int32_t C, const float* params,
                       int64_t param_stride, int64_t wl_off, int64_t bl_off, const int32_t* centre_local, const int32_t* y, int32_t mode,
                       int32_t n_support, const float* protos, int32_t c_task, const int32_t* spt_labels, const int32_t* spt_counts, float* logits,
                       float* dlogits, float* dprotos, float* protos_out, float* loss, float* acc, int32_t bwd, float* dparams,
                       int64_t dparam_stride, float* dQ, float* Gc, const float* sgd_cur, float* sgd_next, int64_t sgd_stride, float sgd_lr,
                       uint32_t* dq_amax, int32_t path, int32_t* launched, void* stream);

#define GM_READOUT_CENTRE 0
#define GM_READOUT_MEAN 1
void gm_set_readout(int32_t mode);
int32_t gm_get_readout(void);

int64_t gm_meta_ws_bytes(const gm_batch_t* spt, const gm_batch_t* qry, const gm_model_t* m, const gm_hparams_t* hp);
int64_t gm_meta_out_floats(const gm_batch_t* spt, const gm_model_t* m, const gm_hparams_t* hp);
int gm_meta_step(const gm_batch_t* spt, const gm_batch_t* qry, const int32_t* y_spt, const int32_t* y_qry,
                 const gm_model_t* m, const gm_hparams_t* hp, const float* theta, float* out, int64_t out_floats,
                 void* ws, int64_t ws_bytes, void* stream);

int64_t gm_adapt_ws_bytes(const gm_batch_t* spt, const gm_model_t* m, const gm_hparams_t* hp);
int gm_meta_adapt(const gm_batch_t* spt, const int32_t* y_spt, const gm_model_t* m, const gm_hparams_t* hp, const float* theta, float* fw_out,
                  int64_t fw_stride, float* protos_out, int32_t c_task, void* ws, int64_t ws_bytes, void* stream);
int64_t gm_predict_ws_bytes(const gm_batch_t* qry, const gm_model_t* m, const gm_hparams_t* hp);
int gm_proto_predict(const gm_batch_t* qry, const gm_model_t* m, const gm_hparams_t* hp, const float* params, int64_t param_stride,
                     const float* protos, const int32_t* n_classes, int32_t c_task, float* logits_out, float* logp_out, int32_t* pred_out,
                     void* ws, int64_t ws_bytes, void* stream);

int gm_meta_finish(const float* head, int64_t P, int32_t K1, float* grad, float* found_inf, void* stream);
int gm_meta_finish_adam(const float* head, int64_t P, int32_t K1, float* theta, float* exp_avg, float* exp_avg_sq, float* grad, float* steps, int32_t n_steps,
                        float lr, float beta1, float beta2, float eps, float* found_inf, uint32_t* ticket, void* stream);

void gm_set_gemm_mode(int32_t mode);
int32_t gm_get_gemm_mode(void);
void gm_set_split_pieces(int32_t pieces);
int32_t gm_get_split_pieces(void);
int gm_set_tuning(const char* name, int32_t value);
int32_t gm_get_tuning(const char* name);
int32_t gm_tuning_epoch(void);

void gm_set_fuse_agg(int32_t on);
int32_t gm_get_fuse_agg(void);

void gm_profile_enable(int32_t on);
int gm_profile_aggregate(double* total_ms, int64_t* launches, int64_t* algorithmic_bytes);
int gm_profile_read(int32_t category, double* total_ms, int64_t* launches, int64_t* work);
int gm_profile_read_launches(int32_t category, double* ms, int64_t* work, int32_t cap);

#ifdef __cplusplus
}
#endif
#endif
```

Before: 1919.

## Aggregate only observable rows via precomputed compacted row lists

During batch setup, the code builds compacted row lists (plus hub schedules) of the rows whose outputs are actually observed: centre rows, e1 rows, and transposed e1 rows. The forward and backward aggregations then launch over these lists, reading the list length from device memory, and skip the launch entirely when a list is empty. The aim is to stop aggregating rows whose results are masked out anyway. In exchange, batch construction does extra compaction and scheduling work and the device-side bounds add complexity. A knob (on by default) and a new export for inspecting the lists are included.

New measurement: 1941, median of 6. 1.01x the previous value.

```diff
diff --git a/g-meta_amd/_lib.py b/g-meta_amd/_lib.py
--- a/g-meta_amd/_lib.py
+++ b/g-meta_amd/_lib.py
@@ -91,6 +91,7 @@
     'gm_dense_wgrad_fused': (C.c_int, [vp, i32, vp, i64, i32, vp, i64, vp, i64, i32, vp, vp, vp, i64, vp, i64, i32, vp]),
     'gm_dense_aggregate': (C.c_int, [vp, i32, i32, vp, i64, i32, i32, vp, vp, i32, vp, i64, i32, vp, vp, vp, i32, vp, i64, i32, i32, i32, i32, i32, vp, vp, vp]),
     'gm_dense_agg_info': (C.c_int, [vp, i32, vp]),
+    'gm_dense_obs_lists': (C.c_int, [vp, vp, vp]),
     'gm_dense_fuse_counts': (C.c_int, [vp, vp]),
     'gm_dense_agg_table': (C.c_int, [vp, i32, i32, vp, i64, vp]),
     'gm_dense_dz_centre': (C.c_int, [vp, vp, i32, vp, i64, i32, vp, vp]),
@@ -135,6 +136,8 @@
     'gm_head_loss_debug': (C.c_int, [i32, vp]),
 }
 
+LATER_EXPORTS = {'gm_dense_obs_lists'}
+
 _lib = None
 
 
@@ -146,6 +149,8 @@
                                '(hipcc --offload-arch=gfx950).  There is no CPU fallback.' % LIB_PATH)
         l = C.CDLL(LIB_PATH)
         for name, (res, args) in PROTOTYPES.items():
+            if name in LATER_EXPORTS and os.environ.get('GMETA_HIP_LIB') and not hasattr(l, name):
+                continue
             fn = getattr(l, name)
             fn.restype, fn.argtypes = res, args
         for name, (res, args) in PROBE_PROTOTYPES.items():
diff --git a/g-meta_amd/csrc/agg.hip b/g-meta_amd/csrc/agg.hip
--- a/g-meta_amd/csrc/agg.hip
+++ b/g-meta_amd/csrc/agg.hip
@@ -20,6 +20,7 @@
     int skip_lo, skip_hi;
     const int32_t* rowlist; int64_t n_list;
     int keep_signed;
+    const int32_t* n_list_dev;
 };
 __host__ __device__ __forceinline__ int agg_xcd_first(const int nb, const int x) {
     const int q = nb / GM_NXCD, r = nb % GM_NXCD;
@@ -242,7 +243,7 @@
     const int lane = threadIdx.x & 63, wave = threadIdx.x >> 6;
     const int g = lane / LPR, l = lane % LPR;
     const int64_t R0 = ((int64_t)lb * (AGG_BLOCK / GM_WAVE) + wave) * a.win;
-    const int64_t nrows_w = a.rowlist ? a.n_list : a.rows;
+    const int64_t nrows_w = a.rowlist ? (a.n_list_dev ? (int64_t)*a.n_list_dev : a.n_list) : a.rows;
     if (R0 >= nrows_w) return;
     const bool mine = lane < a.win && R0 + lane < nrows_w;
     const int64_t myrow = a.rowlist ? (mine ? (int64_t)a.rowlist[R0 + lane] : 0) : R0 + lane;
@@ -306,12 +307,12 @@
 }
 
 int gm_agg_schedule_flat(gm_batch* b, int64_t rows, int win, const int32_t* pos, int n_heavy, const std::vector<int32_t>& tab, int32_t** d_sched, int32_t* len_out,
-                         hipStream_t s, gm_stager* sg) {
+                         hipStream_t s, gm_stager* sg, const uint8_t* keep) {
     const bool split = !tab.empty();
     const int RPB = win * (AGG_BLOCK / GM_WAVE);
     const int nwb = std::max(1, (int)((rows + RPB - 1) / RPB));
     auto x_start = [&](int x) { return agg_xcd_first(nwb, x); };
-    auto n_entries = [&](int k) { return split ? tab[k + 1] - tab[k] : 1; };
+    auto n_entries = [&](int k) { return (keep && !keep[k]) ? 0 : split ? tab[k + 1] - tab[k] : 1; };
     int extra[GM_NXCD] = {}; int first[GM_NXCD + 1];
     {
         int hk = 0;
@@ -333,6 +334,7 @@
         int32_t* o = flat.data() + x * len; int32_t* const o_end = o + len;
         int wb = x_start(x); const int end = x_start(x + 1);
         for (int hk = first[x]; hk < first[x + 1]; ++hk) {
+            if (keep && !keep[hk]) continue;
             const int hb = pos[hk] / RPB;
             while (wb <= hb) *o++ = wb++;
             if (split) for (int g = tab[hk]; g < tab[hk + 1]; ++g) *o++ = -g - 2;
@@ -424,7 +426,7 @@
     a.hub = g.sched ? g.hub : nullptr; a.hub_scratch = g.sched ? g.hub_scratch : nullptr; a.hub_part = g.hub_part; a.hub_ld = GM_AGG_HUB_LD;
     a.e_w = g.e_w; a.x_idx = g.x_idx;
     a.skip_lo = g.skip_on ? g.skip_lo : 1; a.skip_hi = g.skip_on ? g.skip_hi : 0;
-    a.rowlist = g.rowlist; a.n_list = g.n_list;
+    a.rowlist = g.rowlist; a.n_list = g.n_list; a.n_list_dev = g.rowlist ? g.n_list_dev : nullptr;
     a.keep_signed = (g.keep_signed && g.s_out) ? 1 : 0;
     const bool vec4 = (g.width % 4 == 0) && (g.ldx % 4 == 0) && (((uintptr_t)g.x & 15) == 0) && (((uintptr_t)g.out & 15) == 0);
     const bool bias_ok = !g.bias || ((((uintptr_t)g.bias & 15) == 0) && (g.bias_stride % 4 == 0));
diff --git a/g-meta_amd/csrc/common.hip b/g-meta_amd/csrc/common.hip
--- a/g-meta_amd/csrc/common.hip
+++ b/g-meta_amd/csrc/common.hip
@@ -336,6 +336,7 @@
         k.query_streams = env("GM_QUERY_STREAMS", 0);
         k.agg_mid_list = env("GM_AGG_MID_LIST", 1);
         k.agg_mid_win = env("GM_AGG_MID_WIN", 0);
+        k.agg_obs_list = env("GM_AGG_OBS_LIST", 1);
         k.split_pieces = env("GM_SPLIT_PIECES", 3);
         k.split16_min_rows = env("GM_SPLIT16_MIN_ROWS", 65536);
         k.wgrad_split_min_chunks = env("GM_WGRAD_SPLIT_MIN_CHUNKS", -1);
@@ -366,7 +367,7 @@
     (void)gm_knob();
     static const struct { const char* name; int gm_knobs::*field; } tab[] = {
         {"GM_GEMM_SPLIT_MIN_TILES", &gm_knobs::gemm_split_min_tiles}, {"GM_CENTRE_STORE", &gm_knobs::centre_store}, {"GM_DEAD_ROWS", &gm_knobs::dead_rows},
-        {"GM_HEAD_STAGE", &gm_knobs::head_stage}, {"GM_HEAD_THREADS", &gm_knobs::head_threads}, {"GM_QUERY_STREAMS", &gm_knobs::query_streams}, {"GM_AGG_MID_LIST", &gm_knobs::agg_mid_list}, {"GM_AGG_MID_WIN", &gm_knobs::agg_mid_win}, {"GM_AGG_STREAM", &gm_knobs::agg_stream}, {"GM_AGG_STREAM_MIN_ROWS", &gm_knobs::agg_stream_min_rows},
+        {"GM_HEAD_STAGE", &gm_knobs::head_stage}, {"GM_HEAD_THREADS", &gm_knobs::head_threads}, {"GM_QUERY_STREAMS", &gm_knobs::query_streams}, {"GM_AGG_MID_LIST", &gm_knobs::agg_mid_list}, {"GM_AGG_MID_WIN", &gm_knobs::agg_mid_win}, {"GM_AGG_OBS_LIST", &gm_knobs::agg_obs_list}, {"GM_AGG_STREAM", &gm_knobs::agg_stream}, {"GM_AGG_STREAM_MIN_ROWS", &gm_knobs::agg_stream_min_rows},
         {"GM_SPLIT16_MIN_ROWS", &gm_knobs::split16_min_rows}, {"GM_WGRAD_SPLIT_MIN_CHUNKS", &gm_knobs::wgrad_split_min_chunks}, {"GM_TIMING", &gm_knobs::timing},
         {"GM_FUSE_DIFF", &gm_knobs::fuse_diff}, {"GM_EXTRACT_PREF16", &gm_knobs::extract_pref16},
         {"neg_round", &gm_knobs::neg_round}, {"GM_NEG_ROUND", &gm_knobs::neg_round},
diff --git a/g-meta_amd/csrc/dense_exports.hip b/g-meta_amd/csrc/dense_exports.hip
--- a/g-meta_amd/csrc/dense_exports.hip
+++ b/g-meta_amd/csrc/dense_exports.hip
@@ -326,6 +326,13 @@
                        "dense_aggregate: the list schedule goes with the batch's own list (%d rows, windows of %d) and its hub tables", b->n_mid, b->mid_win);
             a.sched = b->d_sched_mid; a.sched_len = b->sched_len_mid; a.sched_win = b->mid_win;
         } else { a.sched = nullptr; a.sched_len = 0; }
+    } else if (list_sched >= 2 && list_sched <= 4) {
+        const gm_batch::obs_list& ol = b->obs[list_sched - 2];
+        GM_REQUIRE(ol.rows && (list_sched == 4) == (transposed != 0), GM_EINVAL, "dense_aggregate: the batch holds no list %d of this orientation", list_sched - 2);
+        GM_REQUIRE(ol.cap >= 1 || ol.sched, GM_EINVAL, "dense_aggregate: list %d is empty and the orientation has no hub rows: nothing to launch", list_sched - 2);
+        GM_REQUIRE(b->n_heavy[o] == 0 || (hubs == 2 && ol.sched), GM_EINVAL, "dense_aggregate: list %d has no schedule for the orientation's hub rows", list_sched - 2);
+        a.rowlist = ol.rows; a.n_list = ol.cap; a.n_list_dev = ol.len; a.list_win = ol.win;
+        a.sched = ol.sched; a.sched_len = ol.sched ? ol.sched_len : 0; a.sched_win = ol.win;
     } else GM_REQUIRE(!list_sched, GM_EINVAL, "dense_aggregate: a list schedule without a row list");
     if (stream_ok && a.e_w && a.e_w == b->d_enorm[o]) GM_TRY(gm_agg_stream_args(a, b, o, gather, st));
     const int rc = gm_launch_aggregate(a, st);
@@ -341,13 +348,40 @@
     std::copy(v, v + 16, info);
     return GM_OK;
 }
+extern "C" int gm_dense_obs_lists(const gm_batch_t* b, int64_t* info, void* stream) {
+    GM_REQUIRE(b && info, GM_EINVAL, "dense_obs_lists: bad arguments");
+    for (int k = 0; k < 3; ++k) {
+        const gm_batch::obs_list& ol = b->obs[k];
+        if (ol.n < 0) {
+            int32_t h = 0;
+            if (ol.rows && ol.len) { GM_HIP(hipMemcpyAsync(&h, ol.len, 4, hipMemcpyDeviceToHost, (hipStream_t)stream)); GM_HIP(hipStreamSynchronize((hipStream_t)stream)); }
+            ol.n = h;
+        }
+        info[4 * k] = ol.n; info[4 * k + 1] = ol.cap; info[4 * k + 2] = ol.win; info[4 * k + 3] = ol.take + (ol.sched ? 4 : 0);
+    }
+    for (int k = 0; k < 2; ++k) {
+        int64_t w[3] = {-1, -1, -1};
+        if (b->d_obs[k] && b->rows > 0) GM_TRY(gm_batch_fwd_counts(b, k, (hipStream_t)stream, w));
+        info[12 + k] = w[0];
+    }
+    info[14] = gm_batch_e1_rows(b, (hipStream_t)stream); info[15] = 0;
+    gm_batch_mark_use(b, (hipStream_t)stream);
+    return GM_OK;
+}
 extern "C" int gm_dense_fuse_counts(const gm_batch_t* b, int64_t* counts) {
     GM_REQUIRE(b && counts, GM_EINVAL, "dense_fuse_counts: bad arguments");
     counts[0] = b->unfused_rows; counts[1] = b->unfused_edges;
     return GM_OK;
 }
 extern "C" int gm_dense_agg_table(const gm_batch_t* b, int32_t which, int32_t transposed, void* dst, int64_t n, void* stream) {
-    GM_REQUIRE(b && dst && n >= 0 && which >= 0 && which <= 9, GM_EINVAL, "dense_agg_table: bad arguments");
+    GM_REQUIRE(b && dst && n >= 0 && which >= 0 && which <= 12, GM_EINVAL, "dense_agg_table: bad arguments");
+    if (which >= 10) {
+        const gm_batch::obs_list& ol = b->obs[which - 10];
+        GM_REQUIRE(ol.rows && n <= ol.cap, GM_EINVAL, "dense_agg_table: table %d holds %lld entries", which, (long long)(ol.rows ? ol.cap : 0));
+        if (n) GM_HIP(hipMemcpyAsync(dst, ol.rows, 4 * (size_t)n, hipMemcpyDeviceToDevice, (hipStream_t)stream));
+        gm_batch_mark_use(b, (hipStream_t)stream);
+        return GM_OK;
+    }
     const int o = transposed ? 1 : 0;
     const void* src = which == 0 ? (const void*)b->d_enorm[o] : which == 1 ? (const void*)b->d_efeat : which == 2 ? (const void*)b->d_mid : which == 3 ? (const void*)b->d_heavy[o]
                     : which == 4 ? (const void*)b->d_fuse2 : which == 5 ? (const void*)b->d_fuse2_feat : which == 6 ? (const void*)b->d_dq_tab
diff --git a/g-meta_amd/csrc/extract.hip b/g-meta_amd/csrc/extract.hip
--- a/g-meta_amd/csrc/extract.hip
+++ b/g-meta_amd/csrc/extract.hip
@@ -610,20 +610,20 @@
     return ok ? (b->unfused_src = (int64_t)h) : fallback;
 }
 #define MID_BLOCK 1024
-__device__ __forceinline__ bool mid_row(const int32_t* indptr, int64_t r, int64_t rows, int lo, int hi) {
+__device__ __forceinline__ bool mid_row(const int32_t* indptr, const float* flag, int64_t r, int64_t rows, int lo, int hi) {
     if (r >= rows) return false;
     const int d = indptr[r + 1] - indptr[r];
-    return d >= lo && d <= hi;
-}
-__global__ __launch_bounds__(MID_BLOCK) void k_mid_count(const int32_t* indptr, int64_t rows, int lo, int hi, int32_t* bcnt) {
+    return d >= lo && d <= hi && !(flag && (__float_as_uint(flag[r]) >> 31));
+}
+__global__ __launch_bounds__(MID_BLOCK) void k_mid_count(const int32_t* indptr, const float* flag, int64_t rows, int lo, int hi, int32_t* bcnt) {
     __shared__ int wsum[MID_BLOCK / 64];
     const int64_t r = (int64_t)blockIdx.x * MID_BLOCK + threadIdx.x;
-    const unsigned long long m = __ballot(mid_row(indptr, r, rows, lo, hi));
+    const unsigned long long m = __ballot(mid_row(indptr, flag, r, rows, lo, hi));
     if ((threadIdx.x & 63) == 0) wsum[threadIdx.x >> 6] = __popcll(m);
     __syncthreads();
     if (threadIdx.x == 0) { int t = 0; for (int k = 0; k < MID_BLOCK / 64; ++k) t += wsum[k]; bcnt[blockIdx.x] = t; }
 }
-__global__ __launch_bounds__(1024) void k_mid_scan(int32_t* bcnt, int nb) {
+__global__ __launch_bounds__(1024) void k_mid_scan(int32_t* bcnt, int nb, int32_t* total, int cap) {
     __shared__ int part[1024];
     const int per = (nb + 1023) / 1024, a = threadIdx.x * per, b = min(nb, a + per);
     int t = 0;
@@ -634,11 +634,12 @@
     __syncthreads();
     int run = part[threadIdx.x];
     for (int k = a; k < b; ++k) { const int v = bcnt[k]; bcnt[k] = run; run += v; }
-}
-__global__ __launch_bounds__(MID_BLOCK) void k_mid_scatter(const int32_t* indptr, int64_t rows, int lo, int hi, const int32_t* boff, int32_t* list, int cap) {
+    if (total && threadIdx.x == 1023) *total = min(run, cap);
+}
+__global__ __launch_bounds__(MID_BLOCK) void k_mid_scatter(const int32_t* indptr, const float* flag, int64_t rows, int lo, int hi, const int32_t* boff, int32_t* list, int cap) {
     __shared__ int wsum[MID_BLOCK / 64];
     const int64_t r = (int64_t)blockIdx.x * MID_BLOCK + threadIdx.x;
-    const bool f = mid_row(indptr, r, rows, lo, hi);
+    const bool f = mid_row(indptr, flag, r, rows, lo, hi);
     const unsigned long long m = __ballot(f);
     const int lane = threadIdx.x & 63, wv = threadIdx.x >> 6;
     if (lane == 0) wsum[wv] = __popcll(m);
@@ -982,7 +983,8 @@
     }
     b->h_centre.assign(h_centre, h_centre + b->n_c);
     b->sched_win = gm_agg_window(b->rows, b->edges);
-    std::vector<int32_t> heavy0, tab0;
+    std::vector<int32_t> heavy_h[2], tab_h[2];
+    std::vector<int32_t>&heavy0 = heavy_h[0], &tab0 = tab_h[0];
     for (int o = 0; o < 2; ++o) {
         b->n_heavy[o] = std::min(h_cnt[o], cap);
         if (b->n_heavy[o] > 0) {
@@ -1001,7 +1003,7 @@
             gm_agg_sched sc;
             GM_TRY(gm_agg_schedule(b, b->rows, b->sched_win, h.data(), hd.data(), b->n_heavy[o], &sc, s, &sg));
             tm.lap("schedule");
-            if (o == 0) { heavy0 = h; tab0 = sc.tab; }
+            heavy_h[o] = h; tab_h[o] = sc.tab;
             {
                 gm_batch::stream_pending& sp = b->spend[o];
                 sp.pending = true; sp.has_tab = sc.d_hub != nullptr; sp.n_parts = sc.d_hub ? sc.parts : (int)nh;
@@ -1010,28 +1012,31 @@
             b->d_sched[o] = sc.d_sched; b->sched_len[o] = sc.len; b->d_hub[o] = sc.d_hub; b->d_hub_scratch[o] = sc.d_hub_scratch; b->hub_part[o] = sc.hub_part; b->hub_words[o] = sc.hub_words; b->hub_parts[o] = sc.parts;
         } else b->spend[o].pending = true;
     }
+    auto compact = [&](const int32_t* indptr, const float* flag, int lo, int hi, int32_t* list, int64_t n_cap, int32_t* total) {
+        const int nb = (int)((b->rows + MID_BLOCK - 1) / MID_BLOCK);
+        int32_t* d_bcnt = nullptr;
+        GM_TRY(gm_alloc(&d_bcnt, (size_t)nb, s));
+        hipLaunchKernelGGL(k_mid_count, dim3(nb), dim3(MID_BLOCK), 0, s, indptr, flag, (int64_t)b->rows, lo, hi, d_bcnt);
+        hipLaunchKernelGGL(k_mid_scan, dim3(1), dim3(1024), 0, s, d_bcnt, nb, total, (int)n_cap);
+        hipLaunchKernelGGL(k_mid_scatter, dim3(nb), dim3(MID_BLOCK), 0, s, indptr, flag, (int64_t)b->rows, lo, hi, d_bcnt, list, (int)n_cap);
+        GM_HIP(hipGetLastError());
+        gm_dev_free(d_bcnt, s);
+        return (int)GM_OK;
+    };
+    auto list_window = [](int64_t n) { int win = 64; while (win > 2 && n / win < 16384) win >>= 1; return gm_knob().agg_mid_win > 0 ? gm_knob().agg_mid_win : win; };
+    auto list_schedule = [&](int o, int64_t n, int win, int32_t** d_sched, int32_t* len, const uint8_t* keep = nullptr) {
+        std::vector<int32_t> pos(heavy_h[o].size());
+        for (size_t k = 0; k < pos.size(); ++k) pos[k] = (int32_t)std::min<int64_t>(std::max<int64_t>(n, 1) - 1, (int64_t)heavy_h[o][k] * n / b->rows);
+        return gm_agg_schedule_flat(b, n, win, pos.data(), (int)pos.size(), tab_h[o], d_sched, len, s, &sg, keep);
+    };
     if (b->d_fuse2 && gm_knob().agg_mid_list) {
         const int64_t n_mid = b->unfused_rows - (int64_t)b->n_heavy[0];
         if (n_mid > 0 && n_mid < b->rows && h_cnt[0] <= cap) {
-            const int nb = (int)((b->rows + MID_BLOCK - 1) / MID_BLOCK);
-            int32_t* d_bcnt = nullptr;
-            GM_TRY(gm_alloc(&d_bcnt, (size_t)nb, s));
             GM_TRY(gm_balloc(b, &b->d_mid, (size_t)n_mid, s));
-            hipLaunchKernelGGL(k_mid_count, dim3(nb), dim3(MID_BLOCK), 0, s, b->d_indptr, (int64_t)b->rows, GM_FUSE_MAXDEG + 1, b->heavy_deg, d_bcnt);
-            hipLaunchKernelGGL(k_mid_scan, dim3(1), dim3(1024), 0, s, d_bcnt, nb);
-            hipLaunchKernelGGL(k_mid_scatter, dim3(nb), dim3(MID_BLOCK), 0, s, b->d_indptr, (int64_t)b->rows, GM_FUSE_MAXDEG + 1, b->heavy_deg, d_bcnt, b->d_mid, (int)n_mid);
-            GM_HIP(hipGetLastError());
-            gm_dev_free(d_bcnt, s);
+            GM_TRY(compact(b->d_indptr, nullptr, GM_FUSE_MAXDEG + 1, b->heavy_deg, b->d_mid, n_mid, nullptr));
             b->n_mid = (int32_t)n_mid;
-            int win = 64;
-            while (win > 2 && n_mid / win < 16384) win >>= 1;
-            if (gm_knob().agg_mid_win > 0) win = gm_knob().agg_mid_win;
-            b->mid_win = win;
-            if (b->n_heavy[0] > 0 && b->d_sched[0]) {
-                std::vector<int32_t> pos(heavy0.size());
-                for (size_t k = 0; k < heavy0.size(); ++k) pos[k] = (int32_t)std::min<int64_t>(n_mid - 1, (int64_t)heavy0[k] * n_mid / b->rows);
-                GM_TRY(gm_agg_schedule_flat(b, n_mid, win, pos.data(), (int)heavy0.size(), tab0, &b->d_sched_mid, &b->sched_len_mid, s, &sg));
-            }
+            b->mid_win = list_window(n_mid);
+            if (b->n_heavy[0] > 0 && b->d_sched[0]) GM_TRY(list_schedule(0, n_mid, b->mid_win, &b->d_sched_mid, &b->sched_len_mid));
         }
     }
     tm.lap("mid-list");
@@ -1062,7 +1067,59 @@
             GM_HIP(hipGetLastError());
             b->d_fwd_tab[0] = tc; b->d_fwd_tab[1] = te; b->d_fwd_tab_feat = tf;
         }
-    }
+        if (gm_knob().agg_mid_list && h_cnt[0] <= cap && h_cnt[1] <= cap) {
+            const int64_t walked_fwd = b->d_mid ? b->n_mid : b->rows;
+            auto finish = [&](int k, int o, int64_t n, int64_t walked, const uint8_t* hub_keep) {
+                gm_batch::obs_list& ol = b->obs[k];
+                ol.cap = (int32_t)n; ol.win = list_window(n);
+                if (2 * n > walked || (b->n_heavy[o] > 0 && !b->d_sched[o])) return (int)GM_OK;
+                if (b->n_heavy[o] > 0) GM_TRY(list_schedule(o, n, ol.win, &ol.sched, &ol.sched_len, hub_keep));
+                ol.take = 1;
+                return (int)GM_OK;
+            };
+            if (b->d_obs[0]) {
+                std::vector<int32_t> lst, hubs_c;
+                for (int k = 0; k < b->n_c; ++k) {
+                    const int32_t row = b->h_sub_off[k / nc] + h_centre[k];
+                    if (h_cdeg[k] > b->heavy_deg) hubs_c.push_back(row); else if (h_cdeg[k] > GM_FUSE_MAXDEG) lst.push_back(row);
+                }
+                std::sort(lst.begin(), lst.end()); lst.erase(std::unique(lst.begin(), lst.end()), lst.end());
+                std::sort(hubs_c.begin(), hubs_c.end());
+                const bool hub_centre = !hubs_c.empty();
+                std::vector<uint8_t> hub_keep(heavy_h[0].size());
+                for (size_t k = 0; k < hub_keep.size(); ++k) hub_keep[k] = std::binary_search(hubs_c.begin(), hubs_c.end(), heavy_h[0][k]) ? 1 : 0;
+                gm_batch::obs_list& ol = b->obs[0];
+                ol.n = (int64_t)lst.size();
+                if (lst.empty() && !hub_centre) ol.take = 2;
+                else {
+                    GM_TRY(gm_balloc(b, &ol.rows, lst.size(), s));
+                    if (!lst.empty()) GM_TRY(sg.upload(ol.rows, lst));
+                    GM_TRY(finish(0, 0, (int64_t)lst.size(), walked_fwd, hub_keep.data()));
+                }
+            }
+            GM_TRY(gm_balloc(b, &b->obs[1].len, 2, s)); b->obs[2].len = b->obs[1].len + 1;
+            GM_HIP(hipMemsetAsync(b->obs[1].len, 0, 8, s));
+            if (b->d_obs[1]) {
+                const int64_t n_range = b->unfused_rows - (int64_t)b->n_heavy[0], bound = std::min<int64_t>(b->n_e1, n_range);
+                if (b->n_e1 == 0 || b->unfused_rows == 0) { b->obs[1].take = 2; b->obs[1].n = 0; }
+                else {
+                    GM_TRY(gm_balloc(b, &b->obs[1].rows, (size_t)bound, s));
+                    if (bound > 0) GM_TRY(compact(b->d_indptr, b->d_obs[1], GM_FUSE_MAXDEG + 1, b->heavy_deg, b->obs[1].rows, bound, b->obs[1].len));
+                    GM_TRY(finish(1, 0, bound, walked_fwd, nullptr));
+                }
+            }
+            {
+                const int64_t bound = std::min<int64_t>(b->n_e1, b->rows);
+                if (b->n_e1 == 0) { b->obs[2].take = 2; b->obs[2].n = 0; }
+                else {
+                    GM_TRY(gm_balloc(b, &b->obs[2].rows, (size_t)bound, s));
+                    GM_TRY(compact(b->d_indptr_t, b->d_norm_e1, 0, INT32_MAX, b->obs[2].rows, bound, b->obs[2].len));
+                    GM_TRY(finish(2, 1, bound, b->rows, nullptr));
+                }
+            }
+        }
+    }
+    tm.lap("obs-lists");
     std::vector<int32_t> ccoff, ecoff, c_set_off(b->sets + 1), e_set_off(b->sets + 1);
     for (int t = 0; t <= b->sets; ++t) { c_set_off[t] = b->h_set_sub_off[t] * nc; e_set_off[t] = eoff[b->h_set_sub_off[t] * nc]; }
     const std::vector<int32_t> ct = set_spans(c_set_off, GM_GEMM_BM), cc = set_spans(c_set_off, gm_wgrad_chunk_rows(c_set_off), &ccoff), ec = set_spans(e_set_off, gm_wgrad_chunk_rows(e_set_off), &ecoff);
diff --git a/g-meta_amd/csrc/gm_internal.h b/g-meta_amd/csrc/gm_internal.h
--- a/g-meta_amd/csrc/gm_internal.h
+++ b/g-meta_amd/csrc/gm_internal.h
@@ -157,6 +157,8 @@
     void* d_fwd_tab[2] = {nullptr, nullptr};
     void* d_fwd_tab_feat = nullptr;
     float* d_obs[2] = {nullptr, nullptr};
+    struct obs_list { int32_t* rows = nullptr; int32_t* len = nullptr; int32_t cap = 0, win = 0, take = 0; int32_t* sched = nullptr; int32_t sched_len = 0; mutable int64_t n = -1; };
+    obs_list obs[3];
     mutable int64_t fwd_cnt[2][3] = {{-1, -1, -1}, {-1, -1, -1}};
     float* d_e1_norm = nullptr;
     float* d_e1_coef = nullptr;
@@ -188,6 +190,7 @@
     int fuse_agg, head_stage;
     int fuse_diff;
     int agg_mid_win;
+    int agg_obs_list;
     int agg_mid_list;
     int query_streams;
     int head_threads;
@@ -396,6 +399,7 @@
     int sched_len, sched_win;
     const int32_t* hub; float* hub_scratch; int hub_part;
     const int32_t* rowlist; int64_t n_list; int list_win;
+    const int32_t* n_list_dev;
     const gm_batch* stream; int stream_o; int stream_feat; int64_t stream_xrows;
     int* launched;
 };
@@ -432,7 +436,8 @@
 }
 int gm_agg_window(int64_t rows, int64_t edges);
 struct gm_stager;
-int gm_agg_schedule_flat(gm_batch* b, int64_t rows, int win, const int32_t* pos, int n_heavy, const std::vector<int32_t>& tab, int32_t** d_sched, int32_t* len, hipStream_t s, gm_stager* sg);
+int gm_agg_schedule_flat(gm_batch* b, int64_t rows, int win, const int32_t* pos, int n_heavy, const std::vector<int32_t>& tab, int32_t** d_sched, int32_t* len, hipStream_t s, gm_stager* sg,
+                         const uint8_t* keep = nullptr);
 int gm_agg_schedule(gm_batch* b, int64_t rows, int win, const int32_t* heavy_host, const int32_t* heavy_deg_host, int n_heavy, gm_agg_sched* out, hipStream_t s, gm_stager* sg);
 int gm_heavy_deg();
 int gm_heavy_deg_for(int64_t rows, int64_t edges);
diff --git a/g-meta_amd/csrc/model.hip b/g-meta_amd/csrc/model.hip
--- a/g-meta_amd/csrc/model.hip
+++ b/g-meta_amd/csrc/model.hip
@@ -594,8 +594,8 @@
 enum PassKind { PASS_PLAIN = 0, PASS_FWD_ONLY = 1, PASS_DIFF = 2 };
 enum RowSet { ROWS_ALL, ROWS_SRC, ROWS_E1, ROWS_CENTRE };
 enum DqFill { DQ_MEMSET, DQ_ZEROED, DQ_CENTRE };
-struct LayerPlan { bool split, fuse; RowSet formed, stored; bool relu_bits; };
-struct PassPlan { PassKind kind; LayerPlan layer[GM_MAX_GCN]; DqFill dq; bool t_centre, dq_e1; };
+struct LayerPlan { bool split, fuse; RowSet formed, stored; bool relu_bits; const gm_batch::obs_list* list; };
+struct PassPlan { PassKind kind; LayerPlan layer[GM_MAX_GCN]; DqFill dq; bool t_centre, dq_e1; const gm_batch::obs_list* t_list; };
 
 struct GcnCtx {
     const gm_batch* b; gm_layout L;
@@ -868,7 +868,17 @@
     if (fwd3 || diff4) p.layer[last].formed = ROWS_CENTRE;
     if (below_ok && ((fwd3 && p.layer[Lg - 2].split) || (diff4 && p.dq_e1 && p.layer[0].fuse && c.M[0]))) {
         p.layer[Lg - 2].stored = ROWS_E1; if (p.layer[Lg - 2].fuse) p.layer[Lg - 2].formed = ROWS_E1; }
+    if (gm_knob().agg_obs_list && c.hub_set == 0) {
+        auto taken = [&](int k) { return b->obs[k].take ? &b->obs[k] : nullptr; };
+        for (int l = 0; l < Lg; ++l)
+            if (p.layer[l].fuse && p.layer[l].formed != ROWS_ALL) p.layer[l].list = taken(p.layer[l].formed == ROWS_CENTRE ? 0 : 1);
+        if (p.dq_e1) p.t_list = taken(2);
+    }
     *plan = p; return plan_check(c, p);
+}
+static void agg_take_list(gm_agg_args& a, const gm_batch::obs_list& ol) {
+    a.rowlist = ol.rows; a.n_list = ol.cap; a.n_list_dev = ol.len; a.list_win = ol.win;
+    a.sched = ol.sched; a.sched_len = ol.sched ? ol.sched_len : 0; a.sched_win = ol.win;
 }
 
 static int gcn_forward(GcnCtx& c, const float* params, int64_t pstride, float* logits, hipStream_t st, int reuse_z1, int skip_head = 0, PassKind kind = PASS_PLAIN) {
@@ -915,9 +925,12 @@
                         else { a.sched = nullptr; a.sched_len = 0; }
                     }
                     if (lp.formed != ROWS_ALL) { a.s_out = row_view(b, lp.formed, gather).sign; a.keep_signed = 1; }
-                    int64_t pb, pbs;
-                    GM_TRY(partial_agg_bytes(b, lp.formed, fi, gather, st, &pb, &pbs));
-                    GM_TRY(launch_agg(a, pb, pbs, st));
+                    if (lp.list && lp.list->take == 1) agg_take_list(a, *lp.list);
+                    if (!(lp.list && lp.list->take == 2)) {
+                        int64_t pb, pbs;
+                        GM_TRY(partial_agg_bytes(b, lp.formed, fi, gather, st, &pb, &pbs));
+                        GM_TRY(launch_agg(a, pb, pbs, st));
+                    }
                 } else {
                     if (a.e_w) GM_TRY(gm_agg_stream_args(a, b, 0, gather, st));
                     int64_t strict = gm_aggregate_bytes(b, fi);
@@ -1045,9 +1058,10 @@
                     a.x_idx = b->d_ect;
                     const RowSet out = dq_e1 ? ROWS_E1 : ROWS_ALL;
                     if (dq_e1) { a.s_out = row_view(b, out, false).keep; a.keep_signed = 1; }
+                    if (dq_e1 && plan.t_list && plan.t_list->take == 1) agg_take_list(a, *plan.t_list);
                     by = t_centre_agg_bytes(b, out, fi, maskbits != nullptr, st);
                 }
-                GM_TRY(launch_agg(a, by, by, st));
+                if (!(t_centre && l == Lg - 1 && dq_e1 && plan.t_list && plan.t_list->take == 2)) GM_TRY(launch_agg(a, by, by, st));
             }
         }
     }
diff --git a/include/gmeta_hip.h b/include/gmeta_hip.h
--- a/include/gmeta_hip.h
+++ b/include/gmeta_hip.h
@@ -175,6 +175,7 @@
                        uint8_t* relu_bits, const float* mask_h, const uint8_t* mask_b, int32_t hubs, const int32_t* rowlist, int64_t n_list,
                        int32_t list_win, int32_t list_sched, int32_t skip_lo, int32_t skip_hi, int32_t stream_ok, float* out, int32_t* launched,
                        void* stream);
+int gm_dense_obs_lists(const gm_batch_t* b, int64_t* info, void* stream);
 int gm_dense_agg_info(const gm_batch_t* b, int32_t transposed, int64_t* info);
 int gm_dense_fuse_counts(const gm_batch_t* b, int64_t* counts);
 int gm_dense_agg_table(const gm_batch_t* b, int32_t which, int32_t transposed, void* dst, int64_t n, void* stream);
```
